# gue-ni/raytracer.glsl

Hardware: AMD Instinct MI355X
Metric: Mpaths/s at 1920x1080, 8 bounces, 10k tris (higher is better)
Workload: dtype f32; 1 GPU; C2: 1920x1080, 8 bounces, 10000 triangles + 5 spheres, cube map 256^2, 1 spp/frame progressive, dof=1; parallelism=1 GPU(s), 8-row strips interleaved, gather to rank 0 every frame, frame_batch=1, kernel=4, wf_rays=4, wf_mode=1, wf_chunk=256, wf_early=0, wf_packed=0, mf_sets=4, mf_group_quads=32, mf_chunk_quads=32

## Files before the change

### raytracer.glsl_amd/csrc/rt_scan.hpp

```cpp
#pragma once
#include <type_traits>
#include "rt_mfma.hpp"

#pragma clang fp contract(off)

namespace rt {

typedef uint32_t u32x4 __attribute__((ext_vector_type(4)));
typedef float f32x6 __attribute__((ext_vector_type(6)));

template <bool kMax> __device__ __forceinline__ float half_reduce(float x)
{
    auto op = [](float a, float b) { return kMax ? __builtin_fmaxf(a, b) : __builtin_fminf(a, b); };
    auto dpp = [](float v, auto ctrl) { return __builtin_bit_cast(float, __builtin_amdgcn_update_dpp(0, __builtin_bit_cast(int, v), decltype(ctrl)::value, 0xf, 0xf, false)); };
    x = op(x, dpp(x, std::integral_constant<int, 0xB1>{}));
    x = op(x, dpp(x, std::integral_constant<int, 0x4E>{}));
    x = op(x, dpp(x, std::integral_constant<int, 0x141>{}));
    x = op(x, dpp(x, std::integral_constant<int, 0x140>{}));
    const float r0 = __builtin_bit_cast(float, __builtin_amdgcn_readlane(__builtin_bit_cast(int, x), 0));
    const float r1 = __builtin_bit_cast(float, __builtin_amdgcn_readlane(__builtin_bit_cast(int, x), 16));
    return op(r0, r1);
}
__device__ __forceinline__ float half_max(float x) { return half_reduce<true>(x); }
__device__ __forceinline__ float half_min(float x) { return half_reduce<false>(x); }
// ... 7 lines not shown
    x = op(x, dpp(x, std::integral_constant<int, 0x140>{}));
    auto rl = [&](int l) { return __builtin_bit_cast(float, __builtin_amdgcn_readlane(__builtin_bit_cast(int, x), l)); };
    return op(op(rl(0), rl(16)), op(rl(32), rl(48)));
}

constexpr uint32_t kCullRowWords = 128;
__device__ __forceinline__ void wave_lds_sync() { __builtin_amdgcn_fence(__ATOMIC_ACQ_REL, "wavefront"); __builtin_amdgcn_wave_barrier(); }
__device__ __forceinline__ bool cull_lane(const MfCull &c, bool have, const MfPacket &pk)
{
    bool skip = false, open = false;
    f3 W = mk(0.0f, 0.0f, 0.0f); float L = 0.0f, nz = 0.0f, Wn = 0.0f;
    if (have && c.Nmin > 0.0f) {
        const f3 gq = pk.O - mk(c.cx, c.cy, c.cz);
        L = __builtin_amdgcn_sqrtf(dot3(gq, gq)) * 1.0001f;
        nz = 9.5367431640625e-07f * __builtin_fmaf(c.lmax, pk.On, c.Pw) * 1.01f;
        W = cross3(pk.D, gq);
        Wn = __builtin_amdgcn_sqrtf(dot3(W, W));
        skip = mf_certified_ka(c, pk, gq, L, nz, Wn);
        open = !skip;
    }
    if (__any(open)) { if (open) skip = mf_certified_b(c, pk, W, L, nz, Wn); }
    return skip;
}

__global__ void __launch_bounds__(256) __attribute__((amdgpu_waves_per_eu(5))) packet_cull_kernel(WaveBuffers wb, const MfCull *__restrict__ cull, uint32_t n_tiles, uint32_t bounce, float ro_add, float sigma_add,
                                                          const MfCull *__restrict__ node, uint32_t node_shift, uint32_t gather)
{
    __shared__ uint32_t s_row[4][kCullRowWords];
    __shared__ uint32_t s_open[4][64];
    const uint32_t n_rays = wb.counts[bounce];
    const RayQueue qin = (bounce & 1u) ? wb.q[1] : wb.q[0];
    const uint32_t lane = threadIdx.x & 63u, n_gran = (n_rays + 127u) / 128u;
    const float inf = __builtin_inff();
    for (uint32_t g = blockIdx.x * 4u + (threadIdx.x >> 6); g < n_gran; g += gridDim.x * 4u) {
        f3 o[2], dh[2]; bool valid[2]; bool usable = true;
        f3 olo = mk(inf, inf, inf), ohi = mk(-inf, -inf, -inf), dlo = olo, dhi = ohi;
#pragma unroll
        for (int k = 0; k < 2; ++k) {
            const uint32_t slot = g * 128u + (uint32_t)k * 64u + lane;
            valid[k] = slot < n_rays;
            o[k] = mk(0.0f, 0.0f, 0.0f); dh[k] = o[k];
            if (valid[k]) {
                float4 a, b;
                const uint32_t from = gather ? wb.sort_src[slot] : n_rays;
                if (from < n_rays) {
                    const float4 *const rec = wb.stage + 4u * from;
                    a = rec[0]; b = rec[1];
                    const float4 c = rec[2];
                    const uint4 r = *reinterpret_cast<const uint4 *>(rec + 3);
                    const uint32_t px = wb.stage_pixel[from];
                    store_through(qin.a + slot, a.x, a.y, a.z, a.w);
                    store_through(qin.b + slot, b.x, b.y, b.z, b.w);
                    store_through(qin.c + slot, c.x, c.y, c.z, c.w);
                    store_through(qin.rng + slot, r.x, r.y, r.z, r.w);
                    store_through(qin.pixel + slot, px);
                } else { a = qin.a[slot]; b = qin.b[slot]; }
                o[k] = mk(a.x, a.y, a.z);
                const f3 d = mk(a.w, b.x, b.y);
                const float dd = dot3(d, d), il = __builtin_amdgcn_rsqf(dd), dl = dd * il;
                dh[k] = mk(d.x * il, d.y * il, d.z * il);
                usable &= (dl > 0.0f) && (dl < inf) && (fabsf(o[k].x) < 1e18f) && (fabsf(o[k].y) < 1e18f) && (fabsf(o[k].z) < 1e18f);
                olo = mk(fminf(olo.x, o[k].x), fminf(olo.y, o[k].y), fminf(olo.z, o[k].z)); ohi = mk(fmaxf(ohi.x, o[k].x), fmaxf(ohi.y, o[k].y), fmaxf(ohi.z, o[k].z));
                dlo = mk(fminf(dlo.x, dh[k].x), fminf(dlo.y, dh[k].y), fminf(dlo.z, dh[k].z)); dhi = mk(fmaxf(dhi.x, dh[k].x), fmaxf(dhi.y, dh[k].y), fmaxf(dhi.z, dh[k].z));
            }
        }
        olo = mk(full_reduce<false>(olo.x), full_reduce<false>(olo.y), full_reduce<false>(olo.z)); ohi = mk(full_reduce<true>(ohi.x), full_reduce<true>(ohi.y), full_reduce<true>(ohi.z));
        dlo = mk(full_reduce<false>(dlo.x), full_reduce<false>(dlo.y), full_reduce<false>(dlo.z)); dhi = mk(full_reduce<true>(dhi.x), full_reduce<true>(dhi.y), full_reduce<true>(dhi.z));
        MfPacket pk;
        pk.O = mk(0.5f * olo.x + 0.5f * ohi.x, 0.5f * olo.y + 0.5f * ohi.y, 0.5f * olo.z + 0.5f * ohi.z);
        f3 D = mk(0.5f * dlo.x + 0.5f * dhi.x, 0.5f * dlo.y + 0.5f * dhi.y, 0.5f * dlo.z + 0.5f * dhi.z);
        const float DD = dot3(D, D), iDl = __builtin_amdgcn_rsqf(DD), Dl = DD * iDl;
        pk.D = mk(D.x * iDl, D.y * iDl, D.z * iDl);
        float ro = 0.0f, sigma = 0.0f;
#pragma unroll
        for (int k = 0; k < 2; ++k)
            if (valid[k]) {
                const f3 eo = o[k] - pk.O, ed = dh[k] - pk.D;
                ro = fmaxf(ro, __builtin_amdgcn_sqrtf(dot3(eo, eo))); sigma = fmaxf(sigma, __builtin_amdgcn_sqrtf(dot3(ed, ed)));
            }
        pk.ro = full_reduce<true>(ro) * 1.0001f + 1e-30f + ro_add; pk.sigma = full_reduce<true>(sigma) * 1.0001f + 2e-6f + sigma_add;
        usable = !__any(!usable) && (Dl > 0.25f);
        pk.On = __builtin_amdgcn_sqrtf(dot3(pk.O, pk.O)) * 1.0001f + pk.ro;
        uint32_t *const row = wb.keep + (size_t)g * wb.keep_words;
        if (node_shift) {
            const uint32_t wv = threadIdx.x >> 6, S = 1u << node_shift, n_nodes = (n_tiles + S - 1u) >> node_shift;
            const uint32_t batch_nodes = (kCullRowWords * 32u) >> node_shift;
            const uint32_t grp = min(S, 32u);
            for (uint32_t b0 = 0; b0 < n_nodes; b0 += batch_nodes) {
                const uint32_t tile0 = b0 << node_shift, w0 = tile0 >> 5;
                s_row[wv][lane] = 0u; s_row[wv][lane + 64u] = 0u;
                wave_lds_sync();
                for (uint32_t n0 = b0; n0 < min(b0 + batch_nodes, n_nodes); n0 += 64u) {
                    const bool have_node = usable && n0 + lane < n_nodes;
                    MfCull c = {};
                    if (have_node) c = node[n0 + lane];
                    const bool closed = cull_lane(c, have_node, pk);
                    const unsigned long long open_nodes = __builtin_amdgcn_ballot_w64(n0 + lane < n_nodes && !closed);
                    if (n0 + lane < n_nodes && !closed)
                        s_open[wv][__builtin_amdgcn_mbcnt_hi((uint32_t)(open_nodes >> 32), __builtin_amdgcn_mbcnt_lo((uint32_t)open_nodes, 0u))] = n0 + lane;
                    wave_lds_sync();
                    const uint32_t n_items = (uint32_t)__builtin_popcountll(open_nodes) << node_shift;
                    for (uint32_t i0 = 0; i0 < n_items; i0 += 64u) {
                        const uint32_t j = i0 + lane;
                        const uint32_t t = j < n_items ? (s_open[wv][j >> node_shift] << node_shift) + (j & (S - 1u)) : n_tiles;
                        const bool have_tile = t < n_tiles;
                        MfCull ct = {};
                        if (usable && have_tile) ct = cull[t];
                        const bool skip = cull_lane(ct, usable && have_tile, pk);
                        const unsigned long long keep = __builtin_amdgcn_ballot_w64(have_tile && !skip);
                        if (j < n_items && (lane & (grp - 1u)) == 0u) {
                            const uint32_t bits = (uint32_t)(keep >> lane) & (uint32_t)((1ull << grp) - 1ull);
                            if (bits) atomicOr(&s_row[wv][(t >> 5) - w0], bits << (t & 31u));
                        }
                    }
                    wave_lds_sync();
                }
                for (uint32_t k = lane; k < kCullRowWords && w0 + k < wb.keep_words; k += 64u)
                    store_through(row + w0 + k, s_row[wv][k]);
                wave_lds_sync();
            }
            continue;
        }
        MfCull c_next = {};
        bool have_next = usable && lane < n_tiles;
        if (have_next) c_next = cull[lane];
        for (uint32_t t0 = 0; t0 < n_tiles; t0 += 64u) {
            const MfCull c = c_next;
            const bool have_this = have_next;
            have_next = usable && t0 + 64u + lane < n_tiles;
            if (have_next) c_next = cull[t0 + 64u + lane];
            const bool skip = cull_lane(c, have_this, pk);
            const unsigned long long have = (n_tiles - t0 >= 64u) ? ~0ull : ((1ull << (n_tiles - t0)) - 1ull);
            const unsigned long long keep = ~(unsigned long long)__builtin_amdgcn_ballot_w64(skip) & have;
            if (lane == 0u) {
                store_through(row + (t0 >> 5), (uint32_t)keep);
                if ((t0 >> 5) + 1u < wb.keep_words) store_through(row + ((t0 >> 5) + 1u), (uint32_t)(keep >> 32));
            }
        }
    }
}

__device__ __forceinline__ void exact_and_merge_at(const MfView &mf, const RayQueue &qin, unsigned long long *best, uint32_t slot, uint32_t pos)
{
    const float4 a = qin.a[slot], b = qin.b[slot];
    const uint32_t v = mf.order[pos];
    TriRay tr; tr.o = mk(a.x, a.y, a.z); tr.d = mk(a.w, b.x, b.y); tr.cv = cross3(tr.d, tr.o); tr.ncv = tr.nd = 0.0f;
    const float t = tri_exact(mf.edges_s[pos], mf.planes_s[pos], tr);
    if (kEps < t && t < kInf) atomicMin(&best[slot], ((unsigned long long)__float_as_uint(t) << 32) | v);
}

constexpr int kDrainFly = 4;
typedef float drain_f4 __attribute__((ext_vector_type(4)));
static_assert(sizeof(TriEdges) == 80 && sizeof(TriPlane) == 32 && alignof(TriEdges) == 16 && alignof(TriPlane) == 16, "drain_region reads these as rows of 16 bytes");
__device__ __forceinline__ void drain_region(const SceneView &sc, const MfView &mf, const RayQueue &qin, unsigned long long *best,
                                             const unsigned long long *recs, uint32_t n_rec, uint32_t lane)
{
    constexpr int K = kDrainFly;
    const uint32_t last_tri = sc.n_tri_visits - 1u;
    for (uint32_t i0 = 0; i0 < n_rec; i0 += 64u * (uint32_t)K) {
        unsigned long long rec[K];
#pragma unroll
        for (int j = 0; j < K; ++j) rec[j] = __hip_atomic_load(recs + min(i0 + (uint32_t)j * 64u + lane, n_rec - 1u), __ATOMIC_RELAXED, __HIP_MEMORY_SCOPE_AGENT);
        uint32_t slot[K], pos5[K], um[K];
#pragma unroll
        for (int j = 0; j < K; ++j) {
            const uint32_t hi = (uint32_t)(rec[j] >> 32);
            slot[j] = (uint32_t)rec[j]; pos5[j] = hi >> 5;
            um[j] = i0 + (uint32_t)j * 64u + lane < n_rec ? hi & 31u : 0u;
        }
        float4 a[K], b[K];
#pragma unroll
        for (int j = 0; j < K; ++j) a[j] = qin.a[slot[j]];
#pragma unroll
        for (int j = 0; j < K; ++j) b[j] = qin.b[slot[j]];
        TriRay tr[K];
#pragma unroll
        for (int j = 0; j < K; ++j) { tr[j].o = mk(a[j].x, a[j].y, a[j].z); tr[j].d = mk(a[j].w, b[j].x, b[j].y); tr[j].cv = cross3(tr[j].d, tr[j].o); tr[j].ncv = tr[j].nd = 0.0f; }
        while ((um[0] | um[1] | um[2] | um[3]) != 0u) {
            static_assert(K == 4, "the loop condition names the masks");
            bool on[K]; uint32_t p[K], v[K]; drain_f4 e[K][5], pl[K][2];
#pragma unroll
            for (int j = 0; j < K; ++j) {
                const uint32_t pos = pos5[j] + (um[j] ? (uint32_t)__builtin_ctz(um[j]) : 0u);
                on[j] = um[j] != 0u && pos < sc.n_tri_visits;
                um[j] &= um[j] - 1u;
                p[j] = min(pos, last_tri);
            }
#pragma unroll
            for (int j = 0; j < K; ++j) {
                const drain_f4 *const ep = reinterpret_cast<const drain_f4 *>(mf.edges_s + p[j]), *const pp = reinterpret_cast<const drain_f4 *>(mf.planes_s + p[j]);
#pragma unroll
                for (int k = 0; k < 5; ++k) e[j][k] = ep[k];
                pl[j][0] = pp[0]; pl[j][1] = pp[1]; v[j] = mf.order[p[j]];
            }
#pragma unroll
            for (int j = 0; j < K; ++j) {
#pragma unroll
                for (int k = 0; k < 5; ++k) asm volatile("" : "+v"(e[j][k]));
                asm volatile("" : "+v"(pl[j][0]), "+v"(pl[j][1]), "+v"(v[j]));
            }
#pragma unroll
            for (int j = 0; j < K; ++j) {
                TriEdges T; TriPlane P;
                T.e0x = e[j][0].x; T.e0y = e[j][0].y; T.e0z = e[j][0].z; T.e1x = e[j][0].w; T.e1y = e[j][1].x; T.e1z = e[j][1].y; T.e2x = e[j][1].z; T.e2y = e[j][1].w; T.e2z = e[j][2].x;
                T.m0x = e[j][2].y; T.m0y = e[j][2].z; T.m0z = e[j][2].w; T.m1x = e[j][3].x; T.m1y = e[j][3].y; T.m1z = e[j][3].z; T.m2x = e[j][3].w; T.m2y = e[j][4].x; T.m2z = e[j][4].y;
                T.bound_e = e[j][4].z; T.bound_m = e[j][4].w;
                P.nx = pl[j][0].x; P.ny = pl[j][0].y; P.nz = pl[j][0].z; P.v0x = pl[j][0].w; P.v0y = pl[j][1].x; P.v0z = pl[j][1].y; P.material = 0; P.pad = 0;
                const float t = tri_exact(T, P, tr[j]);
                if (on[j] && kEps < t && t < kInf) atomicMin(&best[slot[j]], ((unsigned long long)__float_as_uint(t) << 32) | v[j]);
            }
        }
    }
}

constexpr int kSoloSets = 4;
struct SoloCfg {
    static constexpr uint32_t kStepMax = 2u * 64u;
    static constexpr uint32_t kDrain = 192u;
    static constexpr uint32_t kQueue = kStepMax + kDrain + 1u;
    static constexpr uint32_t kRaysPerWave = (uint32_t)kSoloSets * 32u;
};

#define RT_HEAD "s_nop 1\n\t"
#define RT_EXAM(PL, ML, KL, TH) \
    "v_min3_f32 v[" #ML "+0], v[" #PL "+0], v[" #PL "+1], v[" #PL "+2]\n\t" \
    "v_min3_f32 v[" #ML "+1], v[" #PL "+3], v[" #PL "+4], v[" #PL "+5]\n\t" \
    "v_min3_f32 v[" #ML "+2], v[" #PL "+6], v[" #PL "+7], v[" #PL "+8]\n\t" \
    "v_min3_f32 v[" #ML "+3], v[" #PL "+9], v[" #PL "+10], v[" #PL "+11]\n\t" \
    "v_min3_f32 v[" #ML "+4], v[" #PL "+12], v[" #PL "+13], v[" #PL "+14]\n\t" \
    "v_max3_f32 v[" #ML "+5], v[" #ML "+0], v[" #ML "+1], v[" #ML "+2]\n\t" \
    "v_max3_f32 v[" #ML "+5], v[" #ML "+5], v[" #ML "+3], v[" #ML "+4]\n\t" \
    "v_cmp_nle_f32_e64 s[" #KL ":" #KL "+1], v[" #ML "+5], " TH "\n\t"
#define RT_MFMA(NL, AOP, B) "v_mfma_f32_32x32x16_bf16 v[" #NL ":" #NL "+15], " AOP ", " B ", 0\n\t"
#define RT_FOLD(ANY, KL) "s_or_b64 " ANY ", s[" #KL ":" #KL "+1], s[" #KL "+2:" #KL "+3]\n\ts_or_b64 " ANY ", " ANY ", s[" #KL "+4:" #KL "+5]\n\ts_or_b64 " ANY ", " ANY ", s[" #KL "+6:" #KL "+7]\n\t"
#define RT_STAGE_Y_TEXT(AOP) RT_MFMA(192, AOP, "%[b0]") RT_EXAM(128, 96, 36, "%[t0]") RT_MFMA(208, AOP, "%[b1]") RT_EXAM(144, 104, 38, "%[t1]") \
                             RT_MFMA(224, AOP, "%[b2]") RT_EXAM(160, 112, 40, "%[t2]") RT_MFMA(240, AOP, "%[b3]") RT_EXAM(176, 120, 42, "%[t3]")
#define RT_STAGE_X_TEXT(AOP) RT_MFMA(128, AOP, "%[b0]") RT_EXAM(192, 64, 44, "%[t0]") RT_MFMA(144, AOP, "%[b1]") RT_EXAM(208, 72, 46, "%[t1]") \
                             RT_MFMA(160, AOP, "%[b2]") RT_EXAM(224, 80, 48, "%[t2]") RT_MFMA(176, AOP, "%[b3]") RT_EXAM(240, 88, 50, "%[t3]")
#define RT_K_CLOBBERS "s36", "s37", "s38", "s39", "s40", "s41", "s42", "s43", "s44", "s45", "s46", "s47", "s48", "s49", "s50", "s51"
#define RT_TRIP(AY, AX) \
    asm volatile(RT_HEAD RT_STAGE_Y_TEXT("%[ay]") RT_STAGE_X_TEXT("%[ax]") RT_FOLD("%[anya]", 36) RT_FOLD("%[anyb]", 44) \
                 : "+{v[128:143]}"(X0), "+{v[144:159]}"(X1), "+{v[160:175]}"(X2), "+{v[176:191]}"(X3), \
                   "=&{v[192:207]}"(Y0), "=&{v[208:223]}"(Y1), "=&{v[224:239]}"(Y2), "=&{v[240:255]}"(Y3), \
                   "=&{v[96:101]}"(MA0), "=&{v[104:109]}"(MA1), "=&{v[112:117]}"(MA2), "=&{v[120:125]}"(MA3), \
                   "=&{v[64:69]}"(MB0), "=&{v[72:77]}"(MB1), "=&{v[80:85]}"(MB2), "=&{v[88:93]}"(MB3), [anya] "=&s"(any_a), [anyb] "=&s"(any_b) \
                 : [ay] "v"(AY), [ax] "v"(AX), [b0] "v"(B0), [b1] "v"(B1), [b2] "v"(B2), [b3] "v"(B3), [t0] "v"(th0), [t1] "v"(th1), [t2] "v"(th2), [t3] "v"(th3) \
                 : RT_K_CLOBBERS)
#define RT_TRIP_L(AY, AX, NY, NX, ADDR) \
    asm volatile(RT_HEAD RT_MFMA(192, "%[ay]", "%[b0]") "ds_read_b128 %[ny], %[addr]\n\tds_read_b128 %[nx], %[addr] offset:1024\n\tv_add_u32_e32 %[addr], 0x800, %[addr]\n\t" \
                 RT_EXAM(128, 96, 36, "%[t0]") RT_MFMA(208, "%[ay]", "%[b1]") RT_EXAM(144, 104, 38, "%[t1]") \
                 RT_MFMA(224, "%[ay]", "%[b2]") RT_EXAM(160, 112, 40, "%[t2]") RT_MFMA(240, "%[ay]", "%[b3]") RT_EXAM(176, 120, 42, "%[t3]") \
                 RT_STAGE_X_TEXT("%[ax]") "s_waitcnt lgkmcnt(0)\n\t" RT_FOLD("%[anya]", 36) RT_FOLD("%[anyb]", 44) \
                 : "+{v[128:143]}"(X0), "+{v[144:159]}"(X1), "+{v[160:175]}"(X2), "+{v[176:191]}"(X3), \
                   "=&{v[192:207]}"(Y0), "=&{v[208:223]}"(Y1), "=&{v[224:239]}"(Y2), "=&{v[240:255]}"(Y3), \
                   "=&{v[96:101]}"(MA0), "=&{v[104:109]}"(MA1), "=&{v[112:117]}"(MA2), "=&{v[120:125]}"(MA3), \
                   "=&{v[64:69]}"(MB0), "=&{v[72:77]}"(MB1), "=&{v[80:85]}"(MB2), "=&{v[88:93]}"(MB3), [anya] "=&s"(any_a), [anyb] "=&s"(any_b), \
                   [ny] "=&v"(NY), [nx] "=&v"(NX), [addr] "+v"(ADDR) \
                 : [ay] "v"(AY), [ax] "v"(AX), [b0] "v"(B0), [b1] "v"(B1), [b2] "v"(B2), [b3] "v"(B3), [t0] "v"(th0), [t1] "v"(th1), [t2] "v"(th2), [t3] "v"(th3) \
                 : RT_K_CLOBBERS, "memory")
#define RT_TRIP_G(AY, AX, NY, NX, ADDRY, ADDRX) \
    asm volatile(RT_HEAD RT_MFMA(192, "%[ay]", "%[b0]") "ds_read_b128 %[ny], %[addry]\n\tds_read_b128 %[nx], %[addrx]\n\t" \
                 RT_EXAM(128, 96, 36, "%[t0]") RT_MFMA(208, "%[ay]", "%[b1]") RT_EXAM(144, 104, 38, "%[t1]") \
                 RT_MFMA(224, "%[ay]", "%[b2]") RT_EXAM(160, 112, 40, "%[t2]") RT_MFMA(240, "%[ay]", "%[b3]") RT_EXAM(176, 120, 42, "%[t3]") \
                 RT_STAGE_X_TEXT("%[ax]") "s_waitcnt lgkmcnt(0)\n\t" RT_FOLD("%[anya]", 36) RT_FOLD("%[anyb]", 44) \
                 : "+{v[128:143]}"(X0), "+{v[144:159]}"(X1), "+{v[160:175]}"(X2), "+{v[176:191]}"(X3), \
                   "=&{v[192:207]}"(Y0), "=&{v[208:223]}"(Y1), "=&{v[224:239]}"(Y2), "=&{v[240:255]}"(Y3), \
                   "=&{v[96:101]}"(MA0), "=&{v[104:109]}"(MA1), "=&{v[112:117]}"(MA2), "=&{v[120:125]}"(MA3), \
                   "=&{v[64:69]}"(MB0), "=&{v[72:77]}"(MB1), "=&{v[80:85]}"(MB2), "=&{v[88:93]}"(MB3), [anya] "=&s"(any_a), [anyb] "=&s"(any_b), \
                   [ny] "=&v"(NY), [nx] "=&v"(NX) \
                 : [ay] "v"(AY), [ax] "v"(AX), [b0] "v"(B0), [b1] "v"(B1), [b2] "v"(B2), [b3] "v"(B3), [t0] "v"(th0), [t1] "v"(th1), [t2] "v"(th2), [t3] "v"(th3), \
                   [addry] "v"(ADDRY), [addrx] "v"(ADDRX) \
                 : RT_K_CLOBBERS, "memory")
#define RT_STAGE_Y(AY) \
    asm volatile(RT_HEAD RT_STAGE_Y_TEXT("%[ay]") RT_FOLD("%[anya]", 36) \
                 : "=&{v[192:207]}"(Y0), "=&{v[208:223]}"(Y1), "=&{v[224:239]}"(Y2), "=&{v[240:255]}"(Y3), \
                   "=&{v[96:101]}"(MA0), "=&{v[104:109]}"(MA1), "=&{v[112:117]}"(MA2), "=&{v[120:125]}"(MA3), [anya] "=&s"(any_a) \
                 : "{v[128:143]}"(X0), "{v[144:159]}"(X1), "{v[160:175]}"(X2), "{v[176:191]}"(X3), \
                   [ay] "v"(AY), [b0] "v"(B0), [b1] "v"(B1), [b2] "v"(B2), [b3] "v"(B3), [t0] "v"(th0), [t1] "v"(th1), [t2] "v"(th2), [t3] "v"(th3) \
                 : RT_K_CLOBBERS)
#define RT_PRODUCTS_X(AOP) \
    asm volatile(RT_HEAD RT_MFMA(128, "%[a]", "%[b0]") RT_MFMA(144, "%[a]", "%[b1]") RT_MFMA(160, "%[a]", "%[b2]") RT_MFMA(176, "%[a]", "%[b3]") "s_nop 15" \
                 : "=&{v[128:143]}"(X0), "=&{v[144:159]}"(X1), "=&{v[160:175]}"(X2), "=&{v[176:191]}"(X3) \
                 : [a] "v"(AOP), [b0] "v"(B0), [b1] "v"(B1), [b2] "v"(B2), [b3] "v"(B3))
#define RT_EXAMINE_X() \
    asm volatile("s_nop 15\n\t" RT_EXAM(128, 96, 36, "%[t0]") RT_EXAM(144, 104, 38, "%[t1]") RT_EXAM(160, 112, 40, "%[t2]") RT_EXAM(176, 120, 42, "%[t3]") "s_nop 7\n\t" RT_FOLD("%[anya]", 36) \
                 : "=&{v[96:101]}"(MA0), "=&{v[104:109]}"(MA1), "=&{v[112:117]}"(MA2), "=&{v[120:125]}"(MA3), [anya] "=&s"(any_a) \
                 : "{v[128:143]}"(X0), "{v[144:159]}"(X1), "{v[160:175]}"(X2), "{v[176:191]}"(X3), [t0] "v"(th0), [t1] "v"(th1), [t2] "v"(th2), [t3] "v"(th3) \
                 : RT_K_CLOBBERS)
#define RT_EXAMINE_Y() \
    asm volatile("s_nop 15\n\t" RT_EXAM(192, 64, 44, "%[t0]") RT_EXAM(208, 72, 46, "%[t1]") RT_EXAM(224, 80, 48, "%[t2]") RT_EXAM(240, 88, 50, "%[t3]") "s_nop 7\n\t" RT_FOLD("%[anyb]", 44) \
                 : "=&{v[64:69]}"(MB0), "=&{v[72:77]}"(MB1), "=&{v[80:85]}"(MB2), "=&{v[88:93]}"(MB3), [anyb] "=&s"(any_b) \
                 : "{v[192:207]}"(Y0), "{v[208:223]}"(Y1), "{v[224:239]}"(Y2), "{v[240:255]}"(Y3), [t0] "v"(th0), [t1] "v"(th1), [t2] "v"(th2), [t3] "v"(th3) \
                 : RT_K_CLOBBERS)

#define RT_MASK_BIT(ML, U, TH) "v_cmp_nle_f32_e32 vcc, v[" #ML "+" #U "], " TH "\n\tv_addc_co_u32_e32 %[m], vcc, %[m], %[m], vcc\n\t"
#define RT_MASK_SET(ML, TH) RT_MASK_BIT(ML, 4, TH) RT_MASK_BIT(ML, 3, TH) RT_MASK_BIT(ML, 2, TH) RT_MASK_BIT(ML, 1, TH) RT_MASK_BIT(ML, 0, TH)
#define RT_MASK_A(MASK) \
    asm volatile("v_mov_b32_e32 %[m], 0\n\t" RT_MASK_SET(120, "%[t3]") RT_MASK_SET(112, "%[t2]") RT_MASK_SET(104, "%[t1]") RT_MASK_SET(96, "%[t0]") \
                 : [m] "=&v"(MASK) : "{v[96:101]}"(MA0), "{v[104:109]}"(MA1), "{v[112:117]}"(MA2), "{v[120:125]}"(MA3), \
                   [t0] "v"(th0), [t1] "v"(th1), [t2] "v"(th2), [t3] "v"(th3) : "vcc")
#define RT_MASK_B(MASK) \
    asm volatile("v_mov_b32_e32 %[m], 0\n\t" RT_MASK_SET(88, "%[t3]") RT_MASK_SET(80, "%[t2]") RT_MASK_SET(72, "%[t1]") RT_MASK_SET(64, "%[t0]") \
                 : [m] "=&v"(MASK) : "{v[64:69]}"(MB0), "{v[72:77]}"(MB1), "{v[80:85]}"(MB2), "{v[88:93]}"(MB3), \
                   [t0] "v"(th0), [t1] "v"(th1), [t2] "v"(th2), [t3] "v"(th3) : "vcc")

#if defined(RT_SOLO_STAMPS) && RT_SOLO_STAMPS == 3
#define RT_STAMP(var) const unsigned long long var = 0
#define RT_STAMP_ADD(acc, from, to)
#define RT_STAMP_NOW() __builtin_amdgcn_s_memtime()
#elif defined(RT_SOLO_STAMPS) && RT_SOLO_STAMPS == 2
#define RT_STAMP(var) const unsigned long long var = 0
#define RT_STAMP_ADD(acc, from, to)
#define RT_STAMP_NOW() __builtin_amdgcn_s_memrealtime()
#elif defined(RT_SOLO_STAMPS)
#define RT_STAMP(var) const unsigned long long var = __builtin_amdgcn_s_memtime()
#define RT_STAMP_ADD(acc, from, to) acc += (to) - (from)
#define RT_STAMP_NOW() __builtin_amdgcn_s_memtime()
#else
#define RT_STAMP(var)
#define RT_STAMP_ADD(acc, from, to)
#endif

struct Mask128 { unsigned long long lo, hi; };
__device__ __forceinline__ Mask128 m128_shr(Mask128 m, uint32_t s)
{
    Mask128 r;
    if (s >= 128u) { r.lo = 0ull; r.hi = 0ull; }
    else if (s >= 64u) { r.lo = m.hi >> (s - 64u); r.hi = 0ull; }
    else if (s == 0u) r = m;
    else { r.lo = (m.lo >> s) | (m.hi << (64u - s)); r.hi = m.hi >> s; }
    return r;
}
__device__ __forceinline__ Mask128 m128_low(uint32_t n)
{
    Mask128 r;
    r.lo = n >= 64u ? ~0ull : ((1ull << n) - 1ull);
    r.hi = n >= 128u ? ~0ull : (n > 64u ? ((1ull << (n - 64u)) - 1ull) : 0ull);
    return r;
}
__device__ __forceinline__ Mask128 m128_and(Mask128 a, Mask128 b) { Mask128 r; r.lo = a.lo & b.lo; r.hi = a.hi & b.hi; return r; }
__device__ __forceinline__ bool m128_any(Mask128 m) { return (m.lo | m.hi) != 0ull; }
__device__ __forceinline__ uint32_t m128_popc(Mask128 m) { return (uint32_t)__builtin_popcountll(m.lo) + (uint32_t)__builtin_popcountll(m.hi); }
__device__ __forceinline__ uint32_t m128_ctz(Mask128 m)
{
    return m.lo ? (uint32_t)__builtin_ctzll(m.lo) : (m.hi ? 64u + (uint32_t)__builtin_ctzll(m.hi) : 128u);
}
__device__ __forceinline__ uint32_t m128_cto(Mask128 m)
{
    Mask128 n; n.lo = ~m.lo; n.hi = ~m.hi;
    return m128_ctz(n);
}
template <typename Words>
__device__ __forceinline__ Mask128 chunk_keep_bits(Words row, uint32_t tile_begin, uint32_t n_tiles)
{
    const Words w = row + (tile_begin >> 5);
    const uint32_t sh = tile_begin & 31u;
    const unsigned long long w01 = (unsigned long long)w[0] | ((unsigned long long)w[1] << 32), w23 = (unsigned long long)w[2] | ((unsigned long long)w[3] << 32), w4 = w[4];
    Mask128 m;
    m.lo = sh ? (w01 >> sh) | (w23 << (64u - sh)) : w01;
    m.hi = sh ? (w23 >> sh) | (w4 << (64u - sh)) : w23;
    return m128_and(m, m128_low(n_tiles));
}

template <bool kCount>
__global__ void __launch_bounds__(256) cull_items_kernel(WaveBuffers wb, uint32_t bounce, uint32_t chunk_quads, uint32_t n_quads, Counters *__restrict__ counters)
{
    const uint32_t n_rays = wb.counts[bounce], n_gran = (n_rays + 127u) >> 7;
    const uint32_t c = blockIdx.y, q_begin = c * chunk_quads, q_end = min(q_begin + chunk_quads, n_quads);
    const uint32_t lane = threadIdx.x & 63u;
    if (q_begin >= q_end) return;
    const uint32_t n_tiles = (q_end - q_begin) * kMfQuadTiles;
    unsigned long long culled = 0;
    for (uint32_t g0 = blockIdx.x * 256u + (threadIdx.x & ~63u); g0 < n_gran; g0 += gridDim.x * 256u) {
        const uint32_t g = g0 + lane;
        bool any = false;
        if (g < n_gran) {
            const Mask128 bits = chunk_keep_bits(wb.keep + (size_t)g * wb.keep_words, q_begin * kMfQuadTiles, n_tiles);
            any = m128_any(bits);
            if (kCount) culled += (unsigned long long)(n_tiles - m128_popc(bits)) * kMfTileTris * min(128u, n_rays - g * 128u);
        }
        const unsigned long long m = __builtin_amdgcn_ballot_w64(any);
        if (m == 0ull) continue;
        uint32_t at = 0u;
        if (lane == 0u) at = atomicAdd(wb.item_counts + c, (uint32_t)__popcll(m));
        at = __builtin_amdgcn_readfirstlane(at) + __builtin_amdgcn_mbcnt_hi((uint32_t)(m >> 32), __builtin_amdgcn_mbcnt_lo((uint32_t)m, 0u));
        if (any) store_through(wb.items + ((size_t)c * wb.items_stride + at), g);
    }
    if (kCount && culled) atomicAdd(&counters->culled_tests, culled);
}

constexpr uint32_t kPlanItemFixed = 6u;
template <bool kCount>
__global__ void __launch_bounds__(256) scan_plan_kernel(WaveBuffers wb, uint32_t bounce, uint32_t chunk_quads, uint32_t n_quads, Counters *__restrict__ counters)
{
    __shared__ uint32_t wsum[4];
    __shared__ uint32_t carry;
    const uint32_t n_rays = wb.counts[bounce], n_gran = (n_rays + 127u) >> 7;
    const uint32_t c = blockIdx.x, q_begin = c * chunk_quads, q_end = min(q_begin + chunk_quads, n_quads);
    const uint32_t lane = threadIdx.x & 63u, wave = threadIdx.x >> 6;
    const uint32_t n_tiles = q_begin < q_end ? (q_end - q_begin) * kMfQuadTiles : 0u;
    uint32_t *const P = wb.plan_prefix + (size_t)c * wb.plan_stride;
    unsigned long long culled = 0;
    if (threadIdx.x == 0) carry = 0u;
    __syncthreads();
    for (uint32_t g0 = 0; g0 < n_gran; g0 += 256u) {
        const uint32_t g = g0 + threadIdx.x;
        uint32_t cost = 0u;
        if (g < n_gran && n_tiles) {
            const uint32_t kept = m128_popc(chunk_keep_bits(wb.keep + (size_t)g * wb.keep_words, q_begin * kMfQuadTiles, n_tiles));
            cost = kept ? 4u * (kept + kPlanItemFixed) : 1u;
            if (kCount) culled += (unsigned long long)(n_tiles - kept) * kMfTileTris * min(128u, n_rays - g * 128u);
        }
        uint32_t inc = cost;
        for (int off = 1; off < 64; off <<= 1) { const uint32_t t = __shfl_up(inc, off); if (lane >= (uint32_t)off) inc += t; }
        if (lane == 63u) wsum[wave] = inc;
        __syncthreads();
        uint32_t base = carry;
        for (uint32_t w = 0; w < wave; ++w) base += wsum[w];
        if (g < n_gran) store_through(P + g, base + inc);
        __syncthreads();
        if (threadIdx.x == 255u) carry = base + inc;
        __syncthreads();
    }
    if (threadIdx.x == 0) store_through(wb.plan_total + c, carry);
    if (kCount && culled) atomicAdd(&counters->culled_tests, culled);
}
__global__ void __launch_bounds__(64) scan_plan_base_kernel(WaveBuffers wb, uint32_t n_chunks)
{
    const uint32_t lane = threadIdx.x;
    unsigned long long run = 0ull;
    for (uint32_t c0 = 0; c0 < n_chunks; c0 += 64u) {
        const uint32_t c = c0 + lane;
        const unsigned long long t = c < n_chunks ? (unsigned long long)wb.plan_total[c] : 0ull;
        unsigned long long inc = t;
        for (int off = 1; off < 64; off <<= 1) { const unsigned long long u = __shfl_up(inc, off); if (lane >= (uint32_t)off) inc += u; }
        if (c < n_chunks) store_through(wb.plan_base + c, run + inc - t);
        run += __shfl(inc, 63);
    }
    if (lane == 0) store_through(wb.plan_base + n_chunks, run);
}

template <bool kCount, uint32_t kWaves>
__device__ __forceinline__ unsigned long long *solo_cand_words()
{
    if constexpr (kCount) { __shared__ unsigned long long words[kWaves]; return words; }
    else return nullptr;
}
template <bool kCount, int W, int kDist>
__global__ void __launch_bounds__(256 * W) __attribute__((amdgpu_waves_per_eu(W, W)))
scan_solo_kernel(SceneView sc, WaveBuffers wb, MfView mf, uint32_t bounce, uint32_t chunk_quads, uint32_t n_chunks, Counters *__restrict__ counters, int debug_skip_exact, int cull, int narrow_fused)
{
    using Cfg = SoloCfg;
    constexpr bool dynamic = kDist == 1, planned = kDist == 2, hybrid = kDist == 3;
    constexpr int S = kSoloSets;
    constexpr uint32_t kWaves = 4u * (uint32_t)W, kThreads = 256u * (uint32_t)W;
    extern __shared__ uint4 lds_tiles[];
    __shared__ uint2 lds_queue[kWaves * Cfg::kQueue];
    __shared__ uint32_t lds_pick;
    unsigned long long *const lds_cand = solo_cand_words<kCount, kWaves>();
    __shared__ uint32_t lds_ring[kWaves * 16u];
#ifdef RT_SOLO_STAMPS
#if RT_SOLO_STAMPS == 3
    const unsigned long long tr_wave_begin = __builtin_amdgcn_s_memrealtime();
#endif
    const unsigned long long ts_wave_begin = RT_STAMP_NOW();
    unsigned long long tt_stage = 0, tt_rays = 0, tt_group = 0, tt_steady = 0, tt_park = 0, tt_flush = 0, tt_iters = 0, tt_culled = 0, tt_culled_n = 0, tt_tiles = 0;
#endif
    if constexpr (W == 1) asm volatile("" ::: "a255");
    const uint32_t n_rays = wb.counts[bounce], n_gran = (n_rays + 127u) >> 7;
    const RayQueue qin = (bounce & 1u) ? wb.q[1] : wb.q[0];
    unsigned long long *best = (bounce & 1u) ? wb.best[1] : wb.best[0];
    const int lane = threadIdx.x & 63, wave = __builtin_amdgcn_readfirstlane((int)(threadIdx.x >> 6)), col = lane & 31, half = lane >> 5;
    const uint32_t real_quads = min(mf.n_quads, (sc.n_tri_visits + kMfQuadTris - 1u) / kMfQuadTris);
    const uint32_t region = blockIdx.x * kWaves + (uint32_t)wave;
    uint2 *const cand = wb.cand + (size_t)region * wb.cand_region;
    unsigned long long appended = 0;
    uint32_t *const sched = wb.sched + (size_t)bounce * wb.sched_stride;
    uint32_t opaque_zero = 0u;
    asm volatile("" : "+v"(opaque_zero));
    const uint32_t group_shift = (uint32_t)__builtin_ctz(mf.group_quads);
    constexpr uint32_t kQuadBytes = kMfQuadTiles * 1024;
    uint2 *queue = lds_queue + wave * Cfg::kQueue;
    if (kCount && lane == 0) lds_cand[wave] = 0ull;
    unsigned long long c_culled = 0;
    typedef const float __attribute__((address_space(4))) *ConstFloats;
    typedef const uint32_t __attribute__((address_space(4))) *ConstWords;
    typedef float f32x4 __attribute__((ext_vector_type(4)));
    typedef const volatile f32x4 __attribute__((address_space(4))) *ConstGroupHalf;
    const ConstFloats groups_k = (ConstFloats)(uintptr_t)mf.groups;
    const uint32_t l_lane = (uint32_t)half * 32u + (uint32_t)col;

    constexpr bool kSplit = W == 2;
    constexpr int H = kSplit ? S / 2 : S;
    static_assert(S == 4, "a granule is four sets of 32 rays");
    constexpr uint32_t kRayStride = kSplit ? 64u : 32u;
    const uint32_t ray_lane = kSplit ? (uint32_t)lane : (uint32_t)col;
    float4 nxt_a[H], nxt_b[H];
    auto fetch_rays = [&](uint32_t g, float4 (&da)[H], float4 (&db)[H]) {
        if (g * 128u + 128u <= n_rays) {
            const uint32_t slot0 = g * 128u + ray_lane;
#pragma unroll
            for (int j = 0; j < H; ++j) da[j] = qin.a[slot0 + (uint32_t)j * kRayStride];
#pragma unroll
            for (int j = 0; j < H; ++j) db[j] = qin.b[slot0 + (uint32_t)j * kRayStride];
            return;
        }
#pragma unroll
        for (int j = 0; j < H; ++j) {
            const uint32_t slot = g * 128u + (uint32_t)j * kRayStride + ray_lane;
            da[j] = make_float4(0.0f, 0.0f, 0.0f, 0.0f); db[j] = da[j];
            if (slot < n_rays) { da[j] = qin.a[slot]; db[j] = qin.b[slot]; }
        }
    };
    auto prepare_ray = [&](MfRay &r, const float4 &a, const float4 &b, bool valid) {
        r.valid = valid;
        r.o = mk(a.x, a.y, a.z); r.d = mk(a.w, b.x, b.y);
        r.wd = __builtin_amdgcn_sqrtf(dot3(r.d, r.d)) * 1.001f;
        r.wod = (__builtin_amdgcn_sqrtf(dot3(r.o, r.o)) * 1.001f) * r.wd;
        const uint32_t dxy = pack_bf16(r.d.x, r.d.y);
        r.dyz = pack_bf16(r.d.y, r.d.z);
        r.dx_hi = dxy << 16;
        const f3 dl = mk(r.d.x - __uint_as_float(dxy << 16), r.d.y - __uint_as_float(dxy & 0xffff0000u), r.d.z - __uint_as_float(r.dyz & 0xffff0000u));
        if constexpr (kSplit) { r.tail = pack_bf16(1.0f, dl.x); r.tail_hi = pack_bf16(dl.y, dl.z); }
        else { r.tail = half ? pack_bf16(dl.y, dl.z) : pack_bf16(1.0f, dl.x); r.tail_hi = r.tail; }
    };

    constexpr uint32_t kXcds = 8;
    const bool by_xcd = gridDim.x >= kXcds * n_chunks;
    const uint32_t c_first = by_xcd ? (blockIdx.x / kXcds) % n_chunks : blockIdx.x % n_chunks;
    typedef const unsigned long long __attribute__((address_space(4))) *ConstU64;
    const ConstU64 pbase_k = (ConstU64)(uintptr_t)wb.plan_base;
    auto chunk_base = [&](uint32_t cc) -> unsigned long long { return cull ? pbase_k[cc] : (unsigned long long)cc * n_gran; };
    unsigned long long p_lo = 0ull, p_hi = 0ull;
    uint32_t p_next = 0u;
    if constexpr (planned) {
        const unsigned long long total = chunk_base(n_chunks);
        p_lo = (unsigned long long)(((unsigned __int128)total * blockIdx.x) / gridDim.x);
        p_hi = (unsigned long long)(((unsigned __int128)total * (blockIdx.x + 1u)) / gridDim.x);
        uint32_t lo = 0u, hi = n_chunks;
        while (hi - lo > 1u) { const uint32_t mid = (lo + hi) >> 1; if (chunk_base(mid) <= p_lo) lo = mid; else hi = mid; }
        p_next = lo;
    }
    bool first_chunk = true;
    for (uint32_t c_from = c_first;;) {
        RT_STAMP(ts_pick);
        uint32_t c = c_from;
        if constexpr (planned) {
            while (p_next < n_chunks && chunk_base(p_next + 1u) <= p_lo) ++p_next;
            if (p_lo == p_hi || p_next >= n_chunks || chunk_base(p_next) >= p_hi) break;
            c = p_next++;
            if (!first_chunk) __syncthreads();
            first_chunk = false;
        }
        if (dynamic) {
            __syncthreads();
            if (wave == 0) {
                uint32_t dist = 0xFFFFFFFFu;
                for (uint32_t cc = (uint32_t)lane; cc < n_chunks; cc += 64u) {
                    const uint32_t have = cull ? wb.item_counts[cc] : n_gran;
                    if (__hip_atomic_load(sched + cc, __ATOMIC_RELAXED, __HIP_MEMORY_SCOPE_AGENT) < have) dist = min(dist, (cc + n_chunks - c_from) % n_chunks);
                }
                for (int off = 32; off > 0; off >>= 1) dist = min(dist, (uint32_t)__shfl_xor((int)dist, off));
                if (lane == 0) lds_pick = dist == 0xFFFFFFFFu ? 0xFFFFFFFFu : (c_from + dist) % n_chunks;
            }
            __syncthreads();
            c = __builtin_amdgcn_readfirstlane(lds_pick);
            if (c == 0xFFFFFFFFu) break;
        }
        c_from = (c + 1u) % n_chunks;
        const uint32_t q_begin = c * chunk_quads, q_end = min(q_begin + chunk_quads, real_quads);
        const uint32_t v_chunk_begin = q_begin * kMfQuadTris, v_chunk_end = min(q_end * (uint32_t)kMfQuadTris, sc.n_tri_visits);
        const uint32_t n_tiles = (q_end - q_begin) * kMfQuadTiles, tile_begin = q_begin * kMfQuadTiles;
        const Mask128 keep_all = m128_low(n_tiles);
        {
            const uint32_t n16 = (q_end - q_begin) * (kQuadBytes / 16u);
            const uint4 *src = mf.A + (size_t)q_begin * (kQuadBytes / 16u);
            for (uint32_t i0 = threadIdx.x; i0 < n16; i0 += 8u * kThreads) {
                uint4 v[8];
#pragma unroll
                for (int k = 0; k < 8; ++k) { const uint32_t i = i0 + (uint32_t)k * kThreads; v[k] = src[min(i, n16 - 1u)]; }
#pragma unroll
                for (int k = 0; k < 8; ++k) { const uint32_t i = i0 + (uint32_t)k * kThreads; if (i < n16) lds_tiles[i] = v[k]; }
            }
            __syncthreads();
        }
        RT_STAMP(ts_staged);
        RT_STAMP_ADD(tt_stage, ts_pick, ts_staged);

        uint32_t *const counter = sched + c;
        const uint32_t n_items = __builtin_amdgcn_readfirstlane((cull && dynamic) ? wb.item_counts[c] : n_gran);
        const ConstWords items_k = (ConstWords)(uintptr_t)(wb.items + (size_t)c * wb.items_stride);
        uint32_t blocks_here, rank_here;
        if (by_xcd) {
            const uint32_t rest = gridDim.x % (kXcds * n_chunks);
            blocks_here = (gridDim.x / (kXcds * n_chunks)) * kXcds + min(kXcds, rest > kXcds * c ? rest - kXcds * c : 0u);
            rank_here = (blockIdx.x / (kXcds * n_chunks)) * kXcds + blockIdx.x % kXcds;
        } else { blocks_here = (gridDim.x - c + n_chunks - 1u) / n_chunks; rank_here = blockIdx.x / n_chunks; }
        constexpr uint32_t kNone = 0xFFFFFFFFu;
        const uint32_t hdiv = max(wb.hybrid_div, 1u), hturn = max(hdiv - 1u, 1u);
        const uint32_t n_tail = hybrid ? n_gran / hdiv : 0u, n_turns = n_gran - n_tail;
        const uint32_t n_claimable = hybrid ? n_tail : n_items;
        auto claim = [&](uint32_t seen, uint32_t &lo, uint32_t &end) {
            const uint32_t rem = n_claimable > seen ? n_claimable - seen : 0u;
            const uint32_t n = hybrid ? min(max(rem / (2u * max(blocks_here, 1u) * kWaves), 1u), 4u) : min(max(rem / (4u * max(blocks_here, 1u) * kWaves), 1u), 16u);
            uint32_t v = 0u;
            if (lane == 0) v = atomicAdd(counter + opaque_zero, n);
            const uint32_t at = __builtin_amdgcn_readfirstlane(v);
            lo = min(at, n_claimable); end = min(at + n, n_claimable);
        };
        bool tail = false;
        const ConstWords keep_k = (ConstWords)(uintptr_t)wb.keep;
        auto item_of = [&](uint32_t k, uint32_t &g, Mask128 &bits) {
            g = hybrid ? (tail ? hdiv * k + (hdiv - 1u) : (k / hturn) * hdiv + k % hturn) : k; bits = keep_all;
            if (cull) {
                if (dynamic) g = items_k[k];
                bits = chunk_keep_bits(keep_k + (size_t)g * wb.keep_words, tile_begin, n_tiles);
            }
        };
        uint32_t k, hi, step;
        if (dynamic) { step = 1u; claim(0u, k, hi); }
        else if (planned) {
            const unsigned long long cb = chunk_base(c), ce = chunk_base(c + 1u);
            const uint32_t a = (uint32_t)((p_lo > cb ? p_lo : cb) - cb), e = (uint32_t)((p_hi < ce ? p_hi : ce) - cb);
            const uint32_t w_lo = a + (uint32_t)(((unsigned long long)(e - a) * (uint32_t)wave) / kWaves), w_hi = a + (uint32_t)(((unsigned long long)(e - a) * ((uint32_t)wave + 1u)) / kWaves);
            const ConstWords P = (ConstWords)(uintptr_t)(wb.plan_prefix + (size_t)c * wb.plan_stride);
            auto first_above = [&](uint32_t x) -> uint32_t {
                if (!cull) return min(x, n_gran);
                uint32_t lo = 0u, up = n_gran;
                while (lo < up) { const uint32_t mid = (lo + up) >> 1; if (P[mid] > x) up = mid; else lo = mid + 1u; }
                return lo;
            };
            step = 1u; k = first_above(w_lo); hi = first_above(w_hi);
        }
        else {
            step = blocks_here * kWaves; k = rank_here * kWaves + (uint32_t)wave; hi = hybrid ? n_turns : n_items;
            if (hybrid && k >= hi) { tail = true; step = 1u; claim(0u, k, hi); }
        }
        uint32_t rec_k = kNone, rec_g = 0u;
        Mask128 rec_keep = {0ull, 0ull};
        uint32_t ray_k = kNone;
        auto advance = [&]() {
            k += step;
            if (dynamic && k >= hi) claim(hi, k, hi);
            if (hybrid && k >= hi) { if (tail) claim(hi, k, hi); else { tail = true; step = 1u; claim(0u, k, hi); } }
        };
        uint32_t qn = 0, seq = 0, seq_flushed = 0;
        uint32_t *const ring = lds_ring + wave * 16;
        auto flush = [&]() __attribute__((always_inline)) {
            for (uint32_t i0 = 0; i0 < qn; i0 += 64u) {
                const uint32_t i = i0 + (uint32_t)lane;
                const uint2 e = i < qn ? queue[i] : make_uint2(0u, 0u);
                const uint32_t ln = e.x & 63u, pos5 = v_chunk_begin + ((e.x >> 8) & 127u) * kMfTileTris + 5u * (ln >> 5);
                const uint32_t slot0 = ring[(e.x >> 16) & 15u] * 128u;
                if (kCount) {
                    uint32_t pairs = 0u;
#pragma unroll
                    for (int b = 0; b < 5 * S; ++b) pairs += (uint32_t)__popcll(__builtin_amdgcn_ballot_w64(((e.y >> b) & 1u) != 0u));
                    if (lane == 0) lds_cand[wave] += (unsigned long long)pairs;
                }
                const uint32_t bits = (debug_skip_exact == 0 || debug_skip_exact == 3) ? e.y : 0u;
#pragma unroll
                for (int s = 0; s < S; ++s) {
                    uint32_t um = (bits >> (5 * s)) & 31u;
                    const unsigned long long m = __builtin_amdgcn_ballot_w64(um != 0u);
                    const unsigned long long at = appended + __builtin_amdgcn_mbcnt_hi((uint32_t)(m >> 32), __builtin_amdgcn_mbcnt_lo((uint32_t)m, 0u));
                    const uint32_t slot = slot0 + (uint32_t)(s * 32) + (ln & 31u);
                    if (um != 0u) {
                        if (at < (unsigned long long)wb.cand_region) store_through(reinterpret_cast<unsigned long long *>(cand + at), (unsigned long long)slot | ((unsigned long long)((pos5 << 5) | um) << 32));
                        else
                            while (um) {
                                const uint32_t pos = pos5 + (uint32_t)__builtin_ctz(um);
                                um &= um - 1u;
                                if (pos < v_chunk_end) exact_and_merge_at(mf, qin, best, slot, pos);
                            }
                    }
                    appended += (unsigned long long)__popcll(m);
                }
            }
            qn = 0; seq_flushed = seq;
        };
        while (k < hi) {
            RT_STAMP(ts_iter);
            uint32_t g; Mask128 keep;
            if (rec_k == k) { g = rec_g; keep = rec_keep; } else item_of(k, g, keep);
            const uint32_t wave_slot0 = g * 128u;
            const uint32_t succ = k + step < hi ? k + step : kNone;
            if (succ != kNone) { item_of(succ, rec_g, rec_keep); rec_k = succ; }
            if (kCount && cull && !dynamic && !planned)
                c_culled += (unsigned long long)(n_tiles - m128_popc(keep)) * kMfTileTris * min(128u, n_rays - wave_slot0);
            if (!m128_any(keep)) {
                if constexpr (W == 1) { if (succ != kNone && m128_any(rec_keep)) { fetch_rays(rec_g, nxt_a, nxt_b); ray_k = succ; } }
                advance();
                continue;
            }
            if (seq - seq_flushed >= 15u) flush();
            if (lane == 0) ring[seq & 15u] = g;
            const uint32_t item_tag = (seq & 15u) << 16;
            ++seq;
            MfRay ray[H];
            if constexpr (W == 1) {
                if (ray_k != k) fetch_rays(g, nxt_a, nxt_b);
#pragma unroll
                for (int j = 0; j < H; ++j) prepare_ray(ray[j], nxt_a[j], nxt_b[j], wave_slot0 + (uint32_t)j * kRayStride + ray_lane < n_rays);
                if (succ != kNone && m128_any(rec_keep)) { fetch_rays(rec_g, nxt_a, nxt_b); ray_k = succ; }
            }

            u32x4 B0, B1, B2, B3;
            float th0, th1, th2, th3;
            f32x16 X0, X1, X2, X3, Y0, Y1, Y2, Y3;
            f32x6 MA0, MA1, MA2, MA3, MB0, MB1, MB2, MB3;
            unsigned long long any_a, any_b;
            auto append = [&](uint32_t tile, uint32_t mask) __attribute__((always_inline)) {
                const unsigned long long m = __builtin_amdgcn_ballot_w64(mask != 0u);
                uint32_t pre = __builtin_amdgcn_mbcnt_hi((uint32_t)(m >> 32), __builtin_amdgcn_mbcnt_lo((uint32_t)m, 0u));
                asm volatile("" : "+v"(pre));
                queue[mask ? qn + pre : Cfg::kQueue - 1u] = make_uint2((uint32_t)lane | (tile << 8) | item_tag, mask);
                qn += (uint32_t)__popcll(m);
                if (qn >= Cfg::kDrain) flush();
            };
            auto park_a = [&](uint32_t tile) { RT_STAMP(ts_p0); uint32_t mask; RT_MASK_A(mask); append(tile, mask); RT_STAMP(ts_p1); RT_STAMP_ADD(tt_park, ts_p0, ts_p1); };
            auto park_b = [&](uint32_t tile) { RT_STAMP(ts_p0); uint32_t mask; RT_MASK_B(mask); append(tile, mask); RT_STAMP(ts_p1); RT_STAMP_ADD(tt_park, ts_p0, ts_p1); };
            RT_STAMP(ts_rays);
            RT_STAMP_ADD(tt_rays, ts_iter, ts_rays);

            for (uint32_t ts0 = 0; ts0 < n_tiles;) {
                RT_STAMP(ts_g0);
                const uint32_t q = q_begin + ts0 / kMfQuadTiles;
                const uint32_t grp = q >> group_shift;
                const uint32_t ts1 = min(n_tiles, (((grp + 1u) << group_shift) - q_begin) * kMfQuadTiles);
                Mask128 seg = m128_and(m128_shr(keep, ts0), m128_low(ts1 - ts0));
                if (!m128_any(seg)) { ts0 = ts1; continue; }
                const ConstGroupHalf gp = (ConstGroupHalf)(groups_k + (size_t)grp * (sizeof(MfGroup) / 4));
                const f32x4 g_lo = gp[0], g_hi = gp[1];
                MfGroup G;
                G.cx = g_lo.x; G.cy = g_lo.y; G.cz = g_lo.z; G.E = g_lo.w; G.Ml = g_hi.x; G.Pw = g_hi.y; G.P = g_hi.z; G.pad1 = 0.0f;
                if constexpr (W == 2) {
                    fetch_rays(g, nxt_a, nxt_b);
#pragma unroll
                    for (int j = 0; j < H; ++j) prepare_ray(ray[j], nxt_a[j], nxt_b[j], wave_slot0 + (uint32_t)j * kRayStride + ray_lane < n_rays);
                }
                u32x4 Bs[S]; float ths[S];
#pragma unroll
                for (int j = 0; j < H; ++j) {
                    const MfRay &r = ray[j];
                    const f3 ol = r.o - mk(G.cx, G.cy, G.cz);
                    const f3 cvl = cross3(r.d, ol);
                    const float ncv = __builtin_amdgcn_sqrtf(dot3(cvl, cvl)) * 1.001f, no = __builtin_amdgcn_sqrtf(dot3(ol, ol)) * 1.001f;
                    const float margin = mf_margin(G, ncv, no, r);
                    const float th = (!r.valid || debug_skip_exact == 2) ? __builtin_inff() : (margin < 1.0e30f ? -margin : __builtin_nanf(""));
                    const uint32_t bx = pack_bf16(cvl.x, cvl.y), by = (pack_bf16(cvl.z, 0.0f) & 0xffffu) | r.dx_hi;
                    if constexpr (!kSplit) {
                        Bs[j].x = bx; Bs[j].y = by; Bs[j].z = r.dyz; Bs[j].w = r.tail; ths[j] = th;
                    } else {
                        const auto px = __builtin_amdgcn_permlane32_swap(bx, bx, false, false);
                        const auto py = __builtin_amdgcn_permlane32_swap(by, by, false, false);
                        const auto pz = __builtin_amdgcn_permlane32_swap(r.dyz, r.dyz, false, false);
                        const auto pw = __builtin_amdgcn_permlane32_swap(r.tail, r.tail_hi, false, false);
                        const auto pt = __builtin_amdgcn_permlane32_swap(__float_as_uint(th), __float_as_uint(th), false, false);
                        const int s0 = 2 * j, s1 = 2 * j + 1;
                        Bs[s0].x = px[0]; Bs[s0].y = py[0]; Bs[s0].z = pz[0]; Bs[s0].w = pw[0]; ths[s0] = __uint_as_float(pt[0]);
                        Bs[s1].x = px[1]; Bs[s1].y = py[1]; Bs[s1].z = pz[1]; Bs[s1].w = pw[1]; ths[s1] = __uint_as_float(pt[1]);
                    }
                }
                B0 = Bs[0]; B1 = Bs[1]; B2 = Bs[2]; B3 = Bs[3];
                th0 = ths[0]; th1 = ths[1]; th2 = ths[2]; th3 = ths[3];
#if defined(RT_SOLO_STAMPS) && RT_SOLO_STAMPS == 1
                asm volatile("" : "+v"(B0), "+v"(B1), "+v"(B2), "+v"(B3), "+v"(th0), "+v"(th1), "+v"(th2), "+v"(th3));
#endif
                RT_STAMP(ts_g1);
                RT_STAMP_ADD(tt_group, ts_g0, ts_g1);
                typedef const uint4 __attribute__((address_space(3))) *LdsRow;
                const uint32_t n_kept = m128_popc(seg);
                if (n_kept == ts1 - ts0 && debug_skip_exact != 3) {
                    const uint32_t t0 = ts0, t1 = ts1;
                    const uint4 *row = lds_tiles + (size_t)t0 * 64u + l_lane;
                    auto tile_row = [&]() { const uint4 r = *row; row += 64; return u32x4{r.x, r.y, r.z, r.w}; };
                    u32x4 ap = tile_row(), ay = tile_row(), ax = tile_row(), by, bx;
                    uint32_t addr = (uint32_t)(uintptr_t)(LdsRow)row;
                    RT_PRODUCTS_X(ap);
                    uint32_t t = t0 + 1u;
                    for (; t + 3u < t1; t += 4u) {
                        RT_TRIP_L(ay, ax, by, bx, addr);
                        if (__builtin_expect((any_a | any_b) != 0ull, 0)) {
                            if (any_a) park_a(t - 1u);
                            if (any_b) park_b(t);
                        }
                        RT_TRIP_L(by, bx, ay, ax, addr);
                        if (__builtin_expect((any_a | any_b) != 0ull, 0)) {
                            if (any_a) park_a(t + 1u);
                            if (any_b) park_b(t + 2u);
                        }
                    }
                    if (t + 1u < t1) {
                        RT_TRIP_L(ay, ax, by, bx, addr);
                        if ((any_a | any_b) != 0ull) {
                            if (any_a) park_a(t - 1u);
                            if (any_b) park_b(t);
                        }
                        ay = by; t += 2u;
                    }
                    if (t < t1) {
                        RT_STAGE_Y(ay);
                        if (any_a) park_a(t - 1u);
                        RT_EXAMINE_Y();
                        if (any_b) park_b(t);
                    } else {
                        RT_EXAMINE_X();
                        if (any_a) park_a(t - 1u);
                    }
                } else {
                    unsigned long long cur = seg.lo, nxt = seg.hi;
                    uint32_t base = ts0;
                    auto next_tile = [&]() -> uint32_t {
                        if (cur == 0ull) { cur = nxt; nxt = 0ull; base += 64u; }
                        const uint32_t bit = (uint32_t)__builtin_ctzll(cur);
                        cur &= ~(1ull << bit);
                        return base + bit;
                    };
                    const uint32_t lds_lane = (uint32_t)(uintptr_t)(LdsRow)(lds_tiles + l_lane);
                    auto row_addr = [&](uint32_t tile) { return lds_lane + tile * 1024u; };
                    auto load_row = [&](uint32_t tile) { const uint4 r = lds_tiles[(size_t)tile * 64u + l_lane]; return u32x4{r.x, r.y, r.z, r.w}; };
                    uint32_t left = n_kept;
                    uint32_t t_x = next_tile(); --left;
                    u32x4 ap = load_row(t_x), ay, ax, by, bx;
                    uint32_t t_y = t_x, t_n = t_x;
                    if (left > 0u) t_y = next_tile();
                    if (left > 1u) t_n = next_tile();
                    ay = load_row(t_y); ax = load_row(t_n);
                    RT_PRODUCTS_X(ap);
#define RT_LIST_TRIP(AY, AX, NY, NX) do { \
                        left -= 2u; \
                        const uint32_t u_y = left > 0u ? next_tile() : t_x, u_n = left > 1u ? next_tile() : t_x; \
                        const uint32_t a_y = row_addr(u_y), a_n = row_addr(u_n); \
                        RT_TRIP_G(AY, AX, NY, NX, a_y, a_n); \
                        if (__builtin_expect((any_a | any_b) != 0ull, 0)) { \
                            if (any_a) park_a(t_x); \
                            if (any_b) park_b(t_y); \
                        } \
                        t_x = t_n; t_y = u_y; t_n = u_n; \
                    } while (0)
                    while (left >= 4u) { RT_LIST_TRIP(ay, ax, by, bx); RT_LIST_TRIP(by, bx, ay, ax); }
                    if (left >= 2u) { RT_LIST_TRIP(ay, ax, by, bx); ay = by; }
#undef RT_LIST_TRIP
                    if (left == 1u) {
                        RT_STAGE_Y(ay);
                        if (any_a) park_a(t_x);
                        RT_EXAMINE_Y();
                        if (any_b) park_b(t_y);
                    } else {
                        RT_EXAMINE_X();
                        if (any_a) park_a(t_x);
                    }
                }
                ts0 = ts1;
                RT_STAMP(ts_g2);
                RT_STAMP_ADD(tt_steady, ts_g0, ts_g2);
            }
            RT_STAMP(ts_f0);
            advance();
            RT_STAMP(ts_f1);
            RT_STAMP_ADD(tt_flush, ts_f0, ts_f1);
#ifdef RT_SOLO_STAMPS
            tt_iters++; tt_tiles += m128_popc(keep);
#endif
        }
        flush();
        if (!dynamic && !planned) break;
    }
    if (narrow_fused) {
        const uint32_t n_rec = (uint32_t)(appended < (unsigned long long)wb.cand_region ? appended : (unsigned long long)wb.cand_region);
        if (n_rec) {
            asm volatile("s_waitcnt vmcnt(0)" ::: "memory");
            drain_region(sc, mf, qin, best, reinterpret_cast<const unsigned long long *>(cand), n_rec, (uint32_t)lane);
        }
    }
#ifdef RT_SOLO_STAMPS
    if (lane == 0 && mf.dbg_log) {
        unsigned long long *d = reinterpret_cast<unsigned long long *>(mf.dbg_log) + 16ull * bounce;
        const unsigned long long ts_end = RT_STAMP_NOW();
#if RT_SOLO_STAMPS == 3
        const unsigned long long tr_end = __builtin_amdgcn_s_memrealtime();
#endif
        atomicAdd(d + 0, ts_end - ts_wave_begin); atomicAdd(d + 1, tt_stage); atomicAdd(d + 2, tt_rays); atomicAdd(d + 3, tt_group);
        atomicAdd(d + 4, tt_steady); atomicAdd(d + 5, tt_park); atomicAdd(d + 6, tt_flush); atomicAdd(d + 7, tt_iters); atomicAdd(d + 8, 1ull);
        atomicAdd(d + 9, tt_tiles);
        if (blockIdx.x == 0 && wave == 0) d[15] = (unsigned long long)gridDim.x * kWaves;
        atomicMax(d + 10, ts_end - ts_wave_begin);
        if (kDist == 0 && bounce < 16u) {
            unsigned long long *pc = reinterpret_cast<unsigned long long *>(mf.dbg_log) + 2048ull + (16ull * bounce) * 64ull * 2ull + 2ull * (c_first % 512u);
            atomicAdd(pc, ts_end - ts_wave_begin); atomicAdd(pc + 1, 1ull);
        }
        atomicAdd(d + 11, tt_culled); atomicAdd(d + 12, tt_culled_n);
#if RT_SOLO_STAMPS == 3
        atomicAdd(d + 14, tr_end - tr_wave_begin);
#endif
    }
#endif
    if (lane == 0) store_through(wb.cand_counts + region, (uint32_t)(appended < (unsigned long long)wb.cand_region ? appended : (unsigned long long)wb.cand_region));
    if (lane == 0 && appended > (unsigned long long)*wb.cand_peak) atomicMax(wb.cand_peak, (uint32_t)(appended < 0xFFFFFFF0ull ? appended : 0xFFFFFFF0ull));
    if (kCount) {
        if (lane == 0 && lds_cand[wave]) atomicAdd(&counters->candidates, lds_cand[wave]);
        if (lane == 0 && c_culled) atomicAdd(&counters->culled_tests, c_culled);
        if (blockIdx.x == 0 && threadIdx.x == 0) atomicAdd(&counters->tri_tests, (unsigned long long)n_rays * sc.n_tri_visits);
    }
}

constexpr uint32_t kNarrowSplit = 4;
__global__ void __launch_bounds__(256) narrow_phase_kernel(SceneView sc, WaveBuffers wb, MfView mf, uint32_t bounce, uint32_t n_regions)
{
#ifdef RT_SOLO_STAMPS
    if (blockIdx.x == 0 && blockIdx.y == 0 && threadIdx.x == 0 && mf.dbg_log) {
        unsigned long long *d = reinterpret_cast<unsigned long long *>(mf.dbg_log) + 16ull * bounce;
        d[13] += d[10]; d[10] = 0ull;
    }
#endif
    const RayQueue qin = (bounce & 1u) ? wb.q[1] : wb.q[0];
// ... 21 lines not shown
```

### raytracer.glsl_amd/csrc/rtgl_amd.hip

```cpp
#include <hip/hip_runtime.h>
#include <algorithm>
#include <cmath>
#include <cstdio>
#include <cstring>
#include <string>
#include <vector>
#include <map>
#include <mutex>
#include <thread>
#include <condition_variable>
#include <memory>

#include "../../include/rtgl_amd.h"
#include "rt_device.hpp"
#include "rt_wavefront.hpp"
#include "rt_mfma.hpp"
#include "rt_scan.hpp"
#include "rt_denoise.hpp"
#include "rt_temporal.hpp"
#include "rt_temporal_clip.hpp"
#include "rt_tonemap.hpp"
#include "rt_error.hpp"
#include "rt_adaptive.hpp"
#include "rt_adaptive_plan.hpp"
#include "rt_robust.hpp"
#include "rt_robust_plan.hpp"
#include "rt_spread.hpp"
#include "rt_spread_plan.hpp"
#include "rt_node_walk.hpp"
#include "rt_mesh_visits.hpp"
#include "rt_buffers.hpp"
#include "rt_scan_launch.hpp"
#include "rt_shade_launch.hpp"
#include "rt_camera_keep.hpp"

#pragma clang fp contract(off)

using namespace rt;


__global__ void __launch_bounds__(256) prepare_triangles_kernel(const float4 *__restrict__ vertices,
                                                                const uint32_t *__restrict__ visit_tri, uint32_t n_visits,
                                                                TriEdges *__restrict__ edges, TriPlane *__restrict__ planes)
{
    uint32_t k = blockIdx.x * blockDim.x + threadIdx.x;
    if (k >= n_visits) return;
    uint32_t tri = visit_tri[k];
    float4 a = vertices[3 * (size_t)tri + 0], b = vertices[3 * (size_t)tri + 1], c = vertices[3 * (size_t)tri + 2];
    f3 v0 = mk(a.x, a.y, a.z), v1 = mk(b.x, b.y, b.z), v2 = mk(c.x, c.y, c.z);
    f3 e0 = v1 - v0, e1 = v2 - v1, e2 = v0 - v2;
    f3 m0 = cross3(v1, v0), m1 = cross3(v2, v1), m2 = cross3(v0, v2);
    f3 n = normalize3(cross3(v1 - v0, v2 - v0));
    TriEdges E;
    E.e0x = e0.x; E.e0y = e0.y; E.e0z = e0.z; E.e1x = e1.x; E.e1y = e1.y; E.e1z = e1.z; E.e2x = e2.x; E.e2y = e2.y; E.e2z = e2.z;
    E.m0x = m0.x; E.m0y = m0.y; E.m0z = m0.z; E.m1x = m1.x; E.m1y = m1.y; E.m1z = m1.z; E.m2x = m2.x; E.m2y = m2.y; E.m2z = m2.z;
    float be = fmaxf(fmaxf(dot3(e0, e0), dot3(e1, e1)), dot3(e2, e2));
    float bm = fmaxf(fmaxf(dot3(m0, m0), dot3(m1, m1)), dot3(m2, m2));
    E.bound_e = __builtin_sqrtf(be) * 1.0001f;
    E.bound_m = __builtin_sqrtf(bm) * 1.0001f;
    edges[k] = E;
    TriPlane P;
    P.nx = n.x; P.ny = n.y; P.nz = n.z; P.v0x = v0.x; P.v0y = v0.y; P.v0z = v0.z;
    float w = a.w;
    P.material = (w > -2147483648.0f && w < 2147483648.0f) ? (int32_t)w : -1;
    P.pad = 0;
    planes[k] = P;
}

template <bool kCount, bool kAov>
__global__ void __launch_bounds__(256) pathtrace_mega_kernel(SceneView sc, FrameParams P, ImageView im, uint4 *rng_out, Counters *counters, AovView aov)
{
    const int lane = threadIdx.x & 63, wave = threadIdx.x >> 6;
    const int px = (blockIdx.x * 4 + wave) * 8 + (lane & 7);
    const int lrow = blockIdx.y * 8 + (lane >> 3);
    if (px >= im.disp_w || lrow >= im.local_rows) return;
    const int py = local_to_global_row(im, lrow);
    if (py >= im.disp_h) return;

    Rng rng; rng.x = (uint32_t)px; rng.y = (uint32_t)py; rng.z = (uint32_t)P.random;
    rng.w = (uint32_t)px + (uint32_t)py + (uint32_t)P.random;
    float4 *pix = im.pixels + (size_t)lrow * im.width + px;
    f3 prev = mk(0.0f, 0.0f, 0.0f);
    if (!P.reset_flag) { float4 q = *pix; prev = mk(q.x, q.y, q.z); }
    f3 origin, dir;
    camera_ray(P, px, py, im.width, im.height, rng, origin, dir);

    unsigned long long c_seg = 0, c_tests = 0, c_cand = 0, c_env = 0;
    f3 color = mk(0.0f, 0.0f, 0.0f);
    for (uint32_t s = 0; s < P.samples; ++s) {
        f3 o = origin, d = dir;
        f3 radiance = mk(0.0f, 0.0f, 0.0f), thr = mk(1.0f, 1.0f, 1.0f);
        for (uint32_t bounce = 0; bounce < P.max_bounce; ++bounce) {
            if (kCount) c_seg++;
            Hit h1; h1.t = kInf; h1.material = 0; h1.point = h1.normal = mk(0.0f, 0.0f, 0.0f);
            uint32_t sphere_id = kNoSphere;
            bool hit_sphere = kAov ? sphere_pass_id(sc, o, d, h1, sphere_id) : sphere_pass(sc, o, d, h1);
            TriRay tr = make_tri_ray(o, d);
            float best_t = kInf; uint32_t best_v = 0xFFFFFFFFu;
            for (uint32_t v = 0; v < sc.n_tri_visits; ++v) {
                const TriEdges &T = sc.tri_edges[v];
                if (tri_filter(T, tr)) {
                    if (kCount) c_cand++;
                    float t = tri_exact(T, sc.tri_planes[v], tr);
                    if (kEps < t && t < best_t) { best_t = t; best_v = v; }
                }
            }
            if (kCount) c_tests += sc.n_tri_visits;
            bool hit_mesh = best_v != 0xFFFFFFFFu;
            if (!hit_sphere && !hit_mesh) {
                f3 bg;
                if (P.use_envmap) { bg = env_lookup(sc, d); if (kCount) c_env++; }
                else bg = mk(P.background[0], P.background[1], P.background[2]);
                if (kAov && s == 0u && bounce == 0u) aov_write(sc, aov, (uint32_t)(lrow * im.width + px), kAovMiss, h1, 0u, bg);
                radiance = radiance + bg * thr;
                break;
            }
            Hit h = h1;
            if (!(h1.t < best_t)) {
                const TriPlane &pl = sc.tri_planes[best_v];
                h.t = best_t; h.point = o + d * best_t; h.normal = mk(pl.nx, pl.ny, pl.nz); h.material = pl.material;
            }
            if (kAov && s == 0u && bounce == 0u)
                aov_write(sc, aov, (uint32_t)(lrow * im.width + px), !(h1.t < best_t) ? kAovTriangle : kAovSphere, h, !(h1.t < best_t) ? best_v : sphere_id, mk(0.0f, 0.0f, 0.0f));
            if (!shade_hit(sc, h, rng, o, d, thr, radiance)) break;
        }
        color = color + radiance;
    }
    if (kAov && P.max_bounce == 0u) {
        Hit none; none.t = kInf; none.material = 0; none.point = none.normal = mk(0.0f, 0.0f, 0.0f);
        aov_write(sc, aov, (uint32_t)(lrow * im.width + px), kAovMiss, none, 0u, mk(0.0f, 0.0f, 0.0f));
    }
    { const float4 v = accumulate_pixel(P, color, prev); store_through(pix, v.x, v.y, v.z, v.w); }
    if (rng_out) rng_out[(size_t)lrow * im.width + px] = make_uint4(rng.x, rng.y, rng.z, rng.w);
    if (kCount) {
        atomicAdd(&counters->paths, (unsigned long long)P.samples);
        atomicAdd(&counters->segments, c_seg);
        atomicAdd(&counters->tri_tests, c_tests);
        atomicAdd(&counters->candidates, c_cand);
        atomicAdd(&counters->env_lookups, c_env);
    }
}

__global__ void __launch_bounds__(256) image_to_u8_kernel(const float4 *__restrict__ src, uchar4 *__restrict__ dst, int width, int rows, int flip)
{
    int i = blockIdx.x * blockDim.x + threadIdx.x;
    if (i >= width * rows) return;
    int y = i / width, x = i - y * width;
    float4 p = src[i];
    auto q = [](float v) -> unsigned char {
        v = v < 0.0f ? 0.0f : (v > 1.0f ? 1.0f : v);
        if (!(v == v)) v = 0.0f;
        return (unsigned char)__builtin_rintf(v * 255.0f);
    };
    int oy = flip ? rows - 1 - y : y;
    dst[(size_t)oy * width + x] = make_uchar4(q(p.x), q(p.y), q(p.z), q(p.w));
}


static thread_local std::string g_create_error;

struct PartWorker {
    std::thread th;
    std::mutex m;
    std::condition_variable cv;
    enum { kIdle, kJob, kDone, kQuit } state = kIdle;
    int rc = 0;
    rtgl_context *part = nullptr;
};

static int device_alloc(void **p, size_t bytes) { return (int)hipMalloc(p, bytes); }
static int device_free(void *p) { return (int)hipFree(p); }

struct rtgl_context {
    int device = 0;
    int width = 0, height = 0;
    int rank = 0, world = 1, strip_rows = 8, local_rows = 0;
    hipStream_t own_stream = nullptr, stream = nullptr; bool own_stream_shared = false;
    hipEvent_t ev0 = nullptr, ev1 = nullptr;
    bool timed = false;
    std::vector<hipEvent_t> kev;
    uint32_t kev_used = 0;
    std::vector<uint32_t> kev_frame_start;
    std::string error;

    std::vector<uint8_t> h_meshes, h_nodes, h_vertices;
    uint32_t n_meshes = 0, n_nodes = 0, n_vec4 = 0;

    rt_buffers::Ledger buffers{device_alloc, device_free};
    SphereRec *d_spheres = nullptr; uint32_t n_spheres = 0;
    MaterialRec *d_materials = nullptr; uint32_t n_materials = 0;
    float4 *d_vertices = nullptr;
    uint32_t *d_sphere_visits = nullptr; uint32_t n_sphere_visits = 0;
    TriEdges *d_edges = nullptr; TriPlane *d_planes = nullptr; uint32_t n_tri_visits = 0;
    TriEdges *d_edges_s = nullptr; TriPlane *d_planes_s = nullptr;
    uint8_t *d_env = nullptr; int env_w = 0, env_h = 0, env_c = 0, env_faces = 0;
    float4 *d_image_own = nullptr, *d_image = nullptr;
    uint4 *d_rng = nullptr;
    Counters *d_counters = nullptr;
    uchar4 *d_u8 = nullptr;

    float2 *d_group_bounds = nullptr;
    MfGroup *d_mf_groups = nullptr; MfCull *d_mf_cull = nullptr; MfCull *d_mf_cull_node = nullptr; uint32_t cull_node_shift = 0; uint4 *d_mf_A = nullptr; uint32_t *d_mf_order = nullptr; uint32_t n_mf_groups = 0, mf_group_quads = 32; uint32_t *d_dbg_log = nullptr;
    void *d_wave = nullptr; size_t wave_capacity = 0; bool wave_multi = false;
    uint32_t *d_counts = nullptr; uint32_t counts_capacity = 0;
    uint32_t *h_counts = nullptr;
    hipEvent_t counts_ev = nullptr; bool counts_pending = false, counts_valid = false;
    bool timing_this_frame = false; uint32_t timing_frame_counter = 0;
    int kernel_in_use = -1;
    int n_cus = 256;
    uint2 *d_items = nullptr; size_t items_capacity = 0;
    uint32_t *d_sched = nullptr; size_t sched_capacity = 0;
    uint32_t *d_keep = nullptr; size_t keep_capacity = 0;
    uint32_t *d_keep0 = nullptr; size_t keep0_capacity = 0; bool keep0_valid = false; rt_camera_keep::Camera keep0_camera{}; uint32_t keep0_n0 = 0, keep0_words = 0; uint64_t keep0_scene = 0;
    int opt_camera_lean = 1;
    uint32_t camera_lean_frames = 0;
    int opt_shade_pass = 1;
    uint32_t shade_pass_launches = 0;
    uint64_t scene_version = 0;
    void *d_plan = nullptr; size_t plan_capacity = 0;
    void *d_stage = nullptr; size_t stage_capacity = 0;
    uint32_t *d_sort_hist = nullptr; uint32_t sort_bits_alloc = 0;
    int sort_set = 0; uint32_t sort_set_bits = 0; bool sort_sets_clean = false;
    int opt_narrow_fused = 1;
    int opt_sort_move = 1;
    float mesh_lo[3] = {0.0f, 0.0f, 0.0f}, mesh_hi[3] = {0.0f, 0.0f, 0.0f}, mesh_ext = 0.0f;
    uint2 *d_cand = nullptr; uint32_t cand_regions = 0, cand_region_pairs = 0, cand_region_target = 0; bool cand_fixed = false;
    bool solo_attr_set = false;
    bool group_explicit = false;
    bool kernel_explicit = false;
    uint32_t counts_n0 = 0, counts_len = 0;
    std::vector<uint32_t> est_counts;
    WaveBuffers wb{};

    std::vector<rtgl_context *> parts;
    std::vector<hipEvent_t> part_done;
    hipEvent_t gather_done = nullptr;
    std::vector<std::unique_ptr<PartWorker>> workers;
    bool gathered = false, peer_copy = true;

    std::vector<FrameParams> pending;
    float4 *d_batch_rad = nullptr; size_t batch_capacity = 0;
    uint32_t last_batch_frames = 1;
    bool tris_dirty = false, visits_dirty = false;
    float4 *d_aov[3] = {nullptr, nullptr, nullptr}; uint4 *d_aov_ids = nullptr;
    uint32_t aov_n = 0; bool aov_restart = true;
    std::vector<uint32_t> h_visit_mesh, h_visit_tri;
    uint32_t *d_visit_mesh = nullptr, *d_visit_tri = nullptr; bool visit_ids_dirty = true;
    uint32_t *d_visit_scratch = nullptr;
    float4 *d_dn_scratch[2] = {nullptr, nullptr}, *d_denoised = nullptr; bool has_denoised = false;
    float4 *d_dn_variance = nullptr; uint32_t *d_dn_near = nullptr; bool has_dn_variance = false;
    float4 *d_tm_hist[2] = {nullptr, nullptr}, *d_tm_normal[2] = {nullptr, nullptr}, *d_tm_position[2] = {nullptr, nullptr};
    int tm_cur = 0; bool has_temporal = false, tm_valid = false, tm_has_normal = false;
    TemporalCamera tm_camera{};
    float4 *d_tm_moments[2] = {nullptr, nullptr}; int tm_moments = 0;
    uchar4 *d_display = nullptr; uint32_t *d_tone_state = nullptr;
    bool has_display = false, tone_prev = false, tone_auto = false; int tone_set = 0, tone_hist_set = -1; float tone_exposure = 1.0f;
    float *d_err_snapshot = nullptr; uint4 *d_err_tiles = nullptr; uint32_t *d_err_summary = nullptr;
    uint64_t err_epoch = 1, err_snap_epoch = 0; int32_t err_fm = 0, err_first = 0, err_fn = 0; bool err_rendered = false, has_error = false;
    float4 *d_ad_samples = nullptr; float *d_ad_snapshot = nullptr; uint4 *d_ad_records = nullptr; uint32_t *d_ad_counts = nullptr, *d_ad_lists = nullptr;
    bool ad_active = false, has_adaptive = false; rtgl_adaptive_params ad_params{};
    std::vector<uint8_t> ad_mask; std::vector<uint32_t> ad_blocks, ad_tiles;
    float4 *d_rb_buckets = nullptr, *d_rb_out = nullptr;
    uint32_t rb_K = 0, rb_N = 0; bool rb_active = false, rb_resolved = false;
    uint4 *d_rbe_tiles = nullptr; uint32_t *d_rbe_summary = nullptr; bool has_rb_error = false;
    FrameParams params{};
    bool have_params = false;
    int opt_kernel = RTGL_KERNEL_WAVEFRONT_MFMA_SOLO, opt_rng_state = 0, opt_counters = 0, opt_kernel_timing = 0, opt_wf_rays = 4, opt_wf_mode = kLds, opt_wf_chunk = 256, opt_wf_early = 0, opt_wf_packed = 0, opt_mf_chunk_quads = 32, opt_mf_group_quads = 32, opt_cull = 3, opt_sort_min_rays = 131072, opt_scan_waves = 0, opt_scan_dynamic = 0, opt_debug_skip_exact = 0, opt_frame_batch = 1, opt_aov = 0, opt_denoise_source = 0, opt_temporal_moments = 0, opt_denoise_variance = 0;
};

static int fail(rtgl_context *ctx, int code, const std::string &msg)
{
    if (ctx) ctx->error = msg; else g_create_error = msg;
    return code;
}
#define HIPCHK(ctx, expr) do { hipError_t e_ = (expr); if (e_ != hipSuccess) \
    return fail(ctx, RTGL_ERR_DEVICE, std::string(#expr) + ": " + hipGetErrorString(e_)); } while (0)

#define RCCHK(expr) do { const int rc_ = (expr); if (rc_) return rc_; } while (0)

static int buf_rc(rtgl_context *ctx, const char *what, int e) { return e ? fail(ctx, RTGL_ERR_DEVICE, std::string(what) + ": " + hipGetErrorString((hipError_t)e)) : RTGL_OK; }
template <typename T> static int buf_alloc(rtgl_context *ctx, T *&p, size_t bytes) { return buf_rc(ctx, "device allocation", ctx->buffers.allocate((void **)&p, bytes)); }
template <typename T> static int buf_ensure(rtgl_context *ctx, T *&p, size_t bytes) { return buf_rc(ctx, "device allocation", ctx->buffers.ensure((void **)&p, bytes)); }
template <typename T, typename C> static int buf_grow(rtgl_context *ctx, T *&p, C &capacity, size_t need, size_t bytes) { return buf_rc(ctx, "device allocation", ctx->buffers.grow((void **)&p, capacity, (C)need, bytes)); }
template <typename... T> static int buf_release(rtgl_context *ctx, T *&...p)
{
    int e = 0;
    ((e = e ? e : ctx->buffers.release((void **)&p)), ...);
    return buf_rc(ctx, "device free", e);
}

static size_t local_px(const rtgl_context *ctx) { return (size_t)std::max(ctx->local_rows, 1) * ctx->width; }

static int read_rows(rtgl_context *ctx, void *dst, const void *src, size_t px_bytes)
{
    HIPCHK(ctx, hipMemcpyAsync(dst, src, (size_t)ctx->local_rows * ctx->width * px_bytes, hipMemcpyDeviceToHost, ctx->stream));
    HIPCHK(ctx, hipStreamSynchronize(ctx->stream));
    return RTGL_OK;
}

template <typename T>
static int realloc_upload(rtgl_context *ctx, T *&dptr, const void *src, size_t bytes)
{
    if (bytes == 0) return buf_release(ctx, dptr);
    RCCHK(buf_alloc(ctx, dptr, bytes));
    if (src) HIPCHK(ctx, hipMemcpyAsync(dptr, src, bytes, hipMemcpyHostToDevice, ctx->stream));
    HIPCHK(ctx, hipStreamSynchronize(ctx->stream));
    return RTGL_OK;
}

static int local_rows_for(int height, int rank, int world, int strip_rows)
{
    int n_strips = (height + strip_rows - 1) / strip_rows, rows = 0;
    for (int s = rank; s < n_strips; s += world) rows += std::min(strip_rows, height - s * strip_rows);
    return rows;
}

static std::mutex g_stream_mutex;
static std::map<int, std::pair<hipStream_t, int>> g_device_streams;
static hipError_t acquire_device_stream(int device, hipStream_t *out, bool *shared)
{
    const char *priv = getenv("RTGL_AMD_PRIVATE_STREAMS");
    if (priv && atoi(priv) != 0) { *shared = false; return hipStreamCreateWithFlags(out, hipStreamNonBlocking); }
    std::lock_guard<std::mutex> lock(g_stream_mutex);
    auto it = g_device_streams.find(device);
    if (it == g_device_streams.end()) {
        hipStream_t st = nullptr;
        const hipError_t e = hipStreamCreateWithFlags(&st, hipStreamNonBlocking);
        if (e != hipSuccess) return e;
        it = g_device_streams.emplace(device, std::make_pair(st, 0)).first;
    }
    it->second.second++;
    *out = it->second.first; *shared = true;
    return hipSuccess;
}
static std::map<const rtgl_context *, std::pair<int, hipStream_t>> g_ctx_streams;
static void register_ctx_stream(const rtgl_context *ctx, int device, hipStream_t st)
{
    std::lock_guard<std::mutex> lock(g_stream_mutex);
    g_ctx_streams[ctx] = std::make_pair(device, st);
}
static void unregister_ctx_stream(const rtgl_context *ctx)
{
    std::lock_guard<std::mutex> lock(g_stream_mutex);
    g_ctx_streams.erase(ctx);
}
static bool other_stream_in_use(const rtgl_context *ctx, int device, hipStream_t st)
{
    std::lock_guard<std::mutex> lock(g_stream_mutex);
    for (const auto &kv : g_ctx_streams) if (kv.first != ctx && kv.second.first == device && kv.second.second != st) return true;
    return false;
}
static bool concurrent_pipelines_allowed()
{
    const char *a = getenv("RTGL_AMD_ALLOW_CONCURRENT_PIPELINES"), *p = getenv("RTGL_AMD_PRIVATE_STREAMS");
    return (a && atoi(a) != 0) || (p && atoi(p) != 0);
}

static void release_device_stream(int device, hipStream_t st, bool shared)
{
    if (!shared) { (void)hipStreamDestroy(st); return; }
    std::lock_guard<std::mutex> lock(g_stream_mutex);
    auto it = g_device_streams.find(device);
    if (it != g_device_streams.end() && --it->second.second == 0) { (void)hipStreamDestroy(it->second.first); g_device_streams.erase(it); }
}

extern "C" int rtgl_create_tiled(rtgl_context **out, int width, int height, int device, int rank, int world, int strip_rows)
{
    if (!out) return fail(nullptr, RTGL_ERR_INVALID, "out is NULL");
    *out = nullptr;
    if (width <= 0 || height <= 0 || world < 1 || rank < 0 || rank >= world || strip_rows <= 0 || (strip_rows % 8) != 0)
        return fail(nullptr, RTGL_ERR_INVALID, "rtgl_create: bad size / tiling arguments");
    int ndev = 0;
    if (hipGetDeviceCount(&ndev) != hipSuccess || ndev <= 0)
        return fail(nullptr, RTGL_ERR_NO_DEVICE, "no HIP device visible (this library has no CPU path)");
    if (device < 0 || device >= ndev) return fail(nullptr, RTGL_ERR_INVALID, "device ordinal out of range");
    rtgl_context *ctx = new rtgl_context();
    ctx->device = device; ctx->width = width; ctx->height = height;
    ctx->rank = rank; ctx->world = world; ctx->strip_rows = strip_rows;
    ctx->local_rows = local_rows_for(height, rank, world, strip_rows);
    auto bail = [&](int code) { g_create_error = ctx->error; rtgl_destroy(ctx); return code; };
#define CCHK(expr) do { hipError_t e_ = (expr); if (e_ != hipSuccess) { \
    ctx->error = std::string(#expr) + ": " + hipGetErrorString(e_); return bail(RTGL_ERR_DEVICE); } } while (0)
    CCHK(hipSetDevice(device));
    { hipDeviceProp_t prop; if (hipGetDeviceProperties(&prop, device) == hipSuccess && prop.multiProcessorCount > 0) ctx->n_cus = prop.multiProcessorCount; }
    CCHK(acquire_device_stream(device, &ctx->own_stream, &ctx->own_stream_shared));
    ctx->stream = ctx->own_stream;
    register_ctx_stream(ctx, device, ctx->stream);
    CCHK(hipEventCreate(&ctx->ev0));
    CCHK(hipEventCreate(&ctx->ev1));
    size_t img_bytes = local_px(ctx) * sizeof(float4);
    if (buf_alloc(ctx, ctx->d_image_own, img_bytes)) return bail(RTGL_ERR_DEVICE);
    CCHK(hipMemsetAsync(ctx->d_image_own, 0, img_bytes, ctx->stream));
    ctx->d_image = ctx->d_image_own;
    if (buf_alloc(ctx, ctx->d_counters, 64)) return bail(RTGL_ERR_DEVICE);
    CCHK(hipMemsetAsync(ctx->d_counters, 0, 64, ctx->stream));
    CCHK(hipStreamSynchronize(ctx->stream));
#undef CCHK
    if (const char *k = getenv("RTGL_AMD_KERNEL")) { const int v = atoi(k); if (v >= RTGL_KERNEL_MEGA && v <= RTGL_KERNEL_WAVEFRONT_MFMA_SOLO && v != RTGL_KERNEL_REMOVED_3) { ctx->opt_kernel = v; ctx->kernel_explicit = true; } }
    if (const char *k = getenv("RTGL_AMD_SCAN_WAVES")) { const int v = atoi(k); if (v >= 0 && v <= 2) ctx->opt_scan_waves = v; }
    if (const char *k = getenv("RTGL_AMD_FRAME_BATCH")) { const int v = atoi(k); if (v >= 1 && v <= (int)kBatchMax) ctx->opt_frame_batch = v; }
    if (const char *k = getenv("RTGL_AMD_SCAN_DYNAMIC")) { const int v = atoi(k); if (v >= 0 && v <= 4) ctx->opt_scan_dynamic = v; }
    if (const char *k = getenv("RTGL_AMD_NARROW_FUSED")) { const int v = atoi(k); if (v == 0 || v == 1) ctx->opt_narrow_fused = v; }
    if (const char *k = getenv("RTGL_AMD_SORT_MOVE")) { const int v = atoi(k); if (v == 0 || v == 1) ctx->opt_sort_move = v; }
    if (const char *k = getenv("RTGL_AMD_CAMERA_LEAN")) { const int v = atoi(k); if (v == 0 || v == 1) ctx->opt_camera_lean = v; }
    if (const char *k = getenv("RTGL_AMD_SHADE_PASS")) { const int v = atoi(k); if (v == 0 || v == 1) ctx->opt_shade_pass = v; }
    *out = ctx;
    return RTGL_OK;
}

static int flush_pending(rtgl_context *ctx);
extern "C" int rtgl_create(rtgl_context **out, int width, int height, int device)
{
    return rtgl_create_tiled(out, width, height, device, 0, 1, 8);
}

extern "C" void rtgl_destroy(rtgl_context *ctx)
{
    if (!ctx) return;
    if (!ctx->pending.empty() && hipSetDevice(ctx->device) == hipSuccess && flush_pending(ctx) != RTGL_OK)
        fprintf(stderr, "rtgl_destroy: %zu batched frame(s) could not be submitted: %s\n", ctx->pending.size(), ctx->error.c_str());
    unregister_ctx_stream(ctx);
    for (auto &w : ctx->workers) {
        { std::lock_guard<std::mutex> lk(w->m); w->state = PartWorker::kQuit; }
        w->cv.notify_all();
        if (w->th.joinable()) w->th.join();
    }
    ctx->workers.clear();
    for (rtgl_context *part : ctx->parts) rtgl_destroy(part);
    ctx->parts.clear();
    (void)hipSetDevice(ctx->device);
    for (hipEvent_t e : ctx->part_done) (void)hipEventDestroy(e);
    if (ctx->gather_done) (void)hipEventDestroy(ctx->gather_done);
    if (ctx->stream) (void)hipStreamSynchronize(ctx->stream);
#ifdef RT_SOLO_STAMPS
    if (ctx->d_dbg_log) {
        unsigned long long h[16 * 64];
        if (hipMemcpy(h, ctx->d_dbg_log, sizeof h, hipMemcpyDeviceToHost) == hipSuccess)
            for (int b = 0; b < 64 && h[16 * b + 8]; ++b) {
                const unsigned long long *d = h + 16 * b; const double tot = (double)d[0];
                fprintf(stderr, "rtgl stamps bounce %2d: waves %llu iters %llu  cycles/wave %.0f  staging %.1f%% rays %.1f%% segments %.1f%% (of the wave: set-up %.1f%%, park %.1f%%) flush %.1f%%  cycles per tile-stage in steady %.1f  slowest wave of a launch (mean over launches) %.0f  culled items %llu at %.0f cycles\n",
                        b, d[8], d[7], tot / d[8], 100.0 * d[1] / tot, 100.0 * d[2] / tot, 100.0 * d[4] / tot, 100.0 * d[3] / tot, 100.0 * d[5] / tot, 100.0 * d[6] / tot,
                        d[9] ? (double)d[4] / (double)d[9] : 0.0, (double)d[13] * (double)d[15] / (double)d[8], d[12], d[12] ? (double)d[11] / (double)d[12] : 0.0);
            }
#if RT_SOLO_STAMPS == 3
        if (hipMemcpy(h, ctx->d_dbg_log, sizeof h, hipMemcpyDeviceToHost) == hipSuccess) {
            double cyc = 0, ticks = 0;
            for (int b = 0; b < 64 && h[16 * b + 8]; ++b) {
                const unsigned long long *d = h + 16 * b;
                fprintf(stderr, "rtgl clock bounce %2d: %llu waves, %.0f shader cycles per wave over %.0f ticks of 10 ns: %.3f GHz\n", b, d[8], (double)d[0] / d[8], (double)d[14] / d[8], d[14] ? (double)d[0] / (double)d[14] * 0.1 : 0.0);
                cyc += (double)d[0]; ticks += (double)d[14];
            }
            if (ticks > 0) fprintf(stderr, "rtgl clock: in-kernel shader clock of scan_solo_kernel, wave-time weighted over all launches: %.3f GHz\n", cyc / ticks * 0.1);
        }
#endif
        std::vector<unsigned long long> pc(16 * 64 * 2 * 16);
        if (hipMemcpy(pc.data(), reinterpret_cast<unsigned long long *>(ctx->d_dbg_log) + 2048, pc.size() * 8, hipMemcpyDeviceToHost) == hipSuccess)
            for (int b = 0; b < 8; ++b) {
                double tot = 0, cnt = 0; int nch = 0;
                for (int c = 0; c < 64; ++c) { const unsigned long long *e = pc.data() + ((size_t)16 * b * 64 + c) * 2; if (e[1]) { tot += (double)e[0]; cnt += (double)e[1]; nch = c + 1; } }
                if (cnt == 0) continue;
                fprintf(stderr, "rtgl stamps bounce %2d: mean wave time per chunk / bounce mean:", b);
                for (int c = 0; c < nch; ++c) { const unsigned long long *e = pc.data() + ((size_t)16 * b * 64 + c) * 2; fprintf(stderr, " %.2f", e[1] ? ((double)e[0] / (double)e[1]) / (tot / cnt) : 0.0); }
                fprintf(stderr, "\n");
            }
    }
#endif
    ctx->buffers.release_all();
    for (hipEvent_t e : ctx->kev) (void)hipEventDestroy(e);
    if (ctx->h_counts) (void)hipHostFree(ctx->h_counts);
    if (ctx->counts_ev) (void)hipEventDestroy(ctx->counts_ev);
    if (ctx->ev0) (void)hipEventDestroy(ctx->ev0);
    if (ctx->ev1) (void)hipEventDestroy(ctx->ev1);
    if (ctx->own_stream) release_device_stream(ctx->device, ctx->own_stream, ctx->own_stream_shared);
    delete ctx;
}

extern "C" const char *rtgl_last_error(const rtgl_context *ctx) { return ctx ? ctx->error.c_str() : g_create_error.c_str(); }

#define ENTER_NOFLUSH(ctx) do { if (!(ctx)) return RTGL_ERR_INVALID; HIPCHK(ctx, hipSetDevice((ctx)->device)); } while (0)
#define ENTER(ctx) do { ENTER_NOFLUSH(ctx); if (!(ctx)->pending.empty()) { const int rcf_ = flush_pending(ctx); if (rcf_) return rcf_; } } while (0)
#define FANOUT(ctx, call) do { if (!(ctx)->parts.empty()) { (ctx)->gathered = false; \
    for (rtgl_context *part : (ctx)->parts) { const int rc_ = (call); if (rc_) return fail(ctx, rc_, std::string("device ") + std::to_string(part->device) + ": " + part->error); } \
    return RTGL_OK; } } while (0)

extern "C" int rtgl_create_multi(rtgl_context **out, int width, int height, const int *devices, int n_devices, int strip_rows)
{
    if (!out) return fail(nullptr, RTGL_ERR_INVALID, "out is NULL");
    *out = nullptr;
    if (!devices || n_devices < 1 || n_devices > 64) return fail(nullptr, RTGL_ERR_INVALID, "rtgl_create_multi: need 1..64 device ordinals");
    rtgl_context *ctx = nullptr;
    int rc = rtgl_create_tiled(&ctx, width, height, devices[0], 0, 1, strip_rows);
    if (rc) return rc;
    for (int i = 0; i < n_devices; ++i) {
        rtgl_context *part = nullptr;
        rc = rtgl_create_tiled(&part, width, height, devices[i], i, n_devices, strip_rows);
        if (rc) { const std::string msg = g_create_error; rtgl_destroy(ctx); g_create_error = msg; return rc; }
        ctx->parts.push_back(part);
        hipEvent_t ev = nullptr;
        (void)hipSetDevice(devices[i]);
        if (hipEventCreateWithFlags(&ev, hipEventDisableTiming) != hipSuccess) { rtgl_destroy(ctx); return fail(nullptr, RTGL_ERR_DEVICE, "hipEventCreate failed"); }
        ctx->part_done.push_back(ev);
        if (devices[i] != devices[0]) {
            int can = 0;
            (void)hipSetDevice(devices[0]);
            if (hipDeviceCanAccessPeer(&can, devices[0], devices[i]) != hipSuccess || !can) ctx->peer_copy = false;
            else { hipError_t e = hipDeviceEnablePeerAccess(devices[i], 0); if (e != hipSuccess && e != hipErrorPeerAccessAlreadyEnabled) ctx->peer_copy = false; }
            (void)hipGetLastError();
        }
    }
    const char *mt = getenv("RTGL_AMD_MULTI_THREADS");
    if (n_devices > 1 && !(mt && atoi(mt) == 0)) try {
        for (rtgl_context *part : ctx->parts) {
            ctx->workers.emplace_back(new PartWorker);
            PartWorker *w = ctx->workers.back().get();
            w->part = part;
            w->th = std::thread([w] {
                std::unique_lock<std::mutex> lk(w->m);
                for (;;) {
                    w->cv.wait(lk, [w] { return w->state == PartWorker::kJob || w->state == PartWorker::kQuit; });
                    if (w->state == PartWorker::kQuit) return;
                    lk.unlock();
                    const int rc = rtgl_render_frame(w->part);
                    lk.lock();
                    w->rc = rc; w->state = PartWorker::kDone;
                    w->cv.notify_all();
                }
            });
        }
    } catch (const std::exception &) {
        for (auto &w : ctx->workers) {
            { std::lock_guard<std::mutex> lk(w->m); w->state = PartWorker::kQuit; }
            w->cv.notify_all();
            if (w->th.joinable()) w->th.join();
        }
        ctx->workers.clear();
    }
    *out = ctx;
    return RTGL_OK;
}

extern "C" int rtgl_device_count(const rtgl_context *ctx) { return ctx ? (ctx->parts.empty() ? 1 : (int)ctx->parts.size()) : RTGL_ERR_INVALID; }

static int multi_gather(rtgl_context *ctx)
{
    if (ctx->gathered) return RTGL_OK;
    const int world = (int)ctx->parts.size(), sr = ctx->strip_rows;
    const size_t row_bytes = (size_t)ctx->width * 16, strip_bytes = row_bytes * sr;
    std::vector<float> host;
    for (int i = 0; i < world; ++i) {
        rtgl_context *part = ctx->parts[i];
        if (!part->pending.empty()) { HIPCHK(ctx, hipSetDevice(part->device)); const int rc = flush_pending(part); if (rc) return fail(ctx, rc, part->error); }
        const int full = part->local_rows / sr, tail_rows = part->local_rows - full * sr;
        uint8_t *dst = reinterpret_cast<uint8_t *>(ctx->d_image) + (size_t)i * strip_bytes;
        const uint8_t *src = reinterpret_cast<const uint8_t *>(part->d_image);
        if (ctx->peer_copy) {
            HIPCHK(ctx, hipSetDevice(part->device));
            HIPCHK(ctx, hipEventRecord(ctx->part_done[i], part->stream));
            HIPCHK(ctx, hipSetDevice(ctx->device));
            HIPCHK(ctx, hipStreamWaitEvent(ctx->stream, ctx->part_done[i], 0));
            if (full) HIPCHK(ctx, hipMemcpy2DAsync(dst, (size_t)world * strip_bytes, src, strip_bytes, strip_bytes, (size_t)full, hipMemcpyDeviceToDevice, ctx->stream));
            if (tail_rows) HIPCHK(ctx, hipMemcpyAsync(dst + (size_t)full * world * strip_bytes, src + (size_t)full * strip_bytes, row_bytes * tail_rows, hipMemcpyDeviceToDevice, ctx->stream));
        } else {
            host.resize((size_t)part->local_rows * ctx->width * 4);
            int rc = rtgl_read_image_f32(part, host.data());
            if (rc) return fail(ctx, rc, part->error);
            HIPCHK(ctx, hipSetDevice(ctx->device));
            if (full) HIPCHK(ctx, hipMemcpy2DAsync(dst, (size_t)world * strip_bytes, host.data(), strip_bytes, strip_bytes, (size_t)full, hipMemcpyHostToDevice, ctx->stream));
            if (tail_rows) HIPCHK(ctx, hipMemcpyAsync(dst + (size_t)full * world * strip_bytes, reinterpret_cast<const uint8_t *>(host.data()) + (size_t)full * strip_bytes, row_bytes * tail_rows, hipMemcpyHostToDevice, ctx->stream));
            HIPCHK(ctx, hipStreamSynchronize(ctx->stream));
        }
    }
    HIPCHK(ctx, hipSetDevice(ctx->device));
    if (ctx->peer_copy) {
        if (!ctx->gather_done) HIPCHK(ctx, hipEventCreateWithFlags(&ctx->gather_done, hipEventDisableTiming));
        HIPCHK(ctx, hipEventRecord(ctx->gather_done, ctx->stream));
        for (rtgl_context *part : ctx->parts)
            if (part->stream != ctx->stream) {
                HIPCHK(ctx, hipSetDevice(part->device));
                HIPCHK(ctx, hipStreamWaitEvent(part->stream, ctx->gather_done, 0));
            }
        HIPCHK(ctx, hipSetDevice(ctx->device));
    }
    ctx->gathered = true;
    return RTGL_OK;
}

extern "C" int rtgl_gather_tiles(rtgl_context *ctx)
{
    ENTER(ctx);
    if (ctx->parts.empty()) return RTGL_OK;
    return multi_gather(ctx);
}

extern "C" int rtgl_upload_spheres(rtgl_context *ctx, const void *data, uint32_t count)
{
    ENTER(ctx);
    FANOUT(ctx, rtgl_upload_spheres(part, data, count));
    if (count && !data) return fail(ctx, RTGL_ERR_INVALID, "spheres is NULL");
    static_assert(sizeof(SphereRec) == 32, "Sphere stride (shaders/raytracer.glsl:11-15, std140)");
    int rc = realloc_upload(ctx, ctx->d_spheres, data, (size_t)count * 32);
    if (rc) return rc;
    ctx->n_spheres = count; ctx->visits_dirty = true;
    return RTGL_OK;
}

extern "C" int rtgl_upload_materials(rtgl_context *ctx, const void *data, uint32_t count)
{
    ENTER(ctx);
    FANOUT(ctx, rtgl_upload_materials(part, data, count));
    if (count && !data) return fail(ctx, RTGL_ERR_INVALID, "materials is NULL");
    static_assert(sizeof(MaterialRec) == 32, "Material stride (shaders/raytracer.glsl:17-21, std140)");
    int rc = realloc_upload(ctx, ctx->d_materials, data, (size_t)count * 32);
    if (rc) return rc;
    ctx->n_materials = count;
    return RTGL_OK;
}

extern "C" int rtgl_upload_meshes(rtgl_context *ctx, const void *data, uint32_t count)
{
    ENTER(ctx);
    FANOUT(ctx, rtgl_upload_meshes(part, data, count));
    if (count && !data) return fail(ctx, RTGL_ERR_INVALID, "meshes is NULL");
// ... 281 lines not shown
        const size_t px = local_px(ctx), q_bytes = (size_t)n0 * (68 + 8), bytes = 2 * q_bytes + 1024 + (multi_sample ? px * 64 : 0);
        RCCHK(buf_grow(ctx, ctx->d_wave, ctx->wave_capacity, n0, bytes));
        ctx->wave_multi = multi_sample;
        uint8_t *p = (uint8_t *)ctx->d_wave;
        for (int q = 0; q < 2; ++q) {
            ctx->wb.q[q].a = (float4 *)p; p += (size_t)n0 * 16;
            ctx->wb.q[q].b = (float4 *)p; p += (size_t)n0 * 16;
            ctx->wb.q[q].c = (float4 *)p; p += (size_t)n0 * 16;
            ctx->wb.q[q].rng = (uint4 *)p; p += (size_t)n0 * 16;
        }
        for (int q = 0; q < 2; ++q) { ctx->wb.best[q] = (unsigned long long *)p; p += (size_t)n0 * 8; }
        for (int q = 0; q < 2; ++q) { ctx->wb.q[q].pixel = (uint32_t *)p; p += (size_t)n0 * 4; }
        p = (uint8_t *)(((uintptr_t)p + 255) & ~(uintptr_t)255);
        if (multi_sample) {
            ctx->wb.sums = (float4 *)p; p += px * 16;
            ctx->wb.cam_a = (float4 *)p; p += px * 16;
            ctx->wb.cam_b = (float4 *)p; p += px * 16;
            ctx->wb.pix_rng = (uint4 *)p; p += px * 16;
        } else ctx->wb.sums = ctx->wb.cam_a = ctx->wb.cam_b = nullptr, ctx->wb.pix_rng = nullptr;
    }
    ctx->wb.counts = ctx->d_counts;
    ctx->wb.cand_peak = ctx->d_counts + ctx->counts_capacity;
    ctx->wb.group_bounds = ctx->d_group_bounds;
    return RTGL_OK;
}

template <int R, int MODE>
static void launch_bounce(rtgl_context *ctx, const SceneView &sc, const FrameParams &P, const ImageView &im, uint32_t n0, uint32_t bounce, uint4 *rng_out, const AovView *aov)
{
    dim3 grid((n0 + 256u * R - 1) / (256u * R));
    if (aov) {
        if (ctx->opt_counters) hipLaunchKernelGGL((bounce_kernel<R, MODE, true, true>), grid, dim3(256), 0, ctx->stream, sc, P, im, ctx->wb, bounce, rng_out, ctx->d_counters, *aov);
        else hipLaunchKernelGGL((bounce_kernel<R, MODE, false, true>), grid, dim3(256), 0, ctx->stream, sc, P, im, ctx->wb, bounce, rng_out, ctx->d_counters, *aov);
    } else if (ctx->opt_counters)
        hipLaunchKernelGGL((bounce_kernel<R, MODE, true, false>), grid, dim3(256), 0, ctx->stream, sc, P, im, ctx->wb, bounce, rng_out, ctx->d_counters, AovView{});
    else
        hipLaunchKernelGGL((bounce_kernel<R, MODE, false, false>), grid, dim3(256), 0, ctx->stream, sc, P, im, ctx->wb, bounce, rng_out, ctx->d_counters, AovView{});
}

template <bool kSort>
static void launch_shade(rtgl_context *ctx, const rt_shade_launch::Launch &L, const SceneView &sc, const FrameParams &P, const ImageView &im, uint32_t bounce, uint4 *rng_out, const AovView *aov)
{
    using ShadeKernel = decltype(&shade_kernel<false, kSort, false>);
    static const ShadeKernel kKernels[2][2][2] = {
        {{shade_stride_kernel<false, kSort, false>, shade_stride_kernel<false, kSort, true>}, {shade_stride_kernel<true, kSort, false>, shade_stride_kernel<true, kSort, true>}},
        {{shade_kernel<false, kSort, false>, shade_kernel<false, kSort, true>}, {shade_kernel<true, kSort, false>, shade_kernel<true, kSort, true>}}};
    if (L.one_pass) ctx->shade_pass_launches++;
    hipLaunchKernelGGL(kKernels[L.one_pass][ctx->opt_counters != 0][aov != nullptr], dim3(L.blocks), dim3(256), 0, ctx->stream, sc, P, im, ctx->wb, bounce, rng_out, ctx->d_counters, aov ? *aov : AovView{});
}

template <bool kSort>
static void launch_shade_camera(rtgl_context *ctx, uint32_t n0, const SceneView &sc, const FrameParams &P, const ImageView &im, uint4 *rng_out)
{
    const dim3 grid((n0 + 255u) / 256u);
    if (ctx->opt_counters) hipLaunchKernelGGL((shade_camera_kernel<true, kSort>), grid, dim3(256), 0, ctx->stream, sc, P, im, ctx->wb, rng_out, ctx->d_counters);
    else hipLaunchKernelGGL((shade_camera_kernel<false, kSort>), grid, dim3(256), 0, ctx->stream, sc, P, im, ctx->wb, rng_out, ctx->d_counters);
}

static uint32_t estimate_rays(const rtgl_context *ctx, uint32_t n0, uint32_t bounce)
{
    if (bounce == 0 || bounce >= ctx->est_counts.size()) return n0;
    uint64_t e = (uint64_t)ctx->est_counts[bounce] + ctx->est_counts[bounce] / 10 + 2048;
    return (uint32_t)std::min<uint64_t>(e, n0);
}

template <int R, int MODE>
static void launch_intersect(rtgl_context *ctx, const SceneView &sc, uint32_t n0, uint32_t bounce)
{
    const uint32_t chunk = (uint32_t)ctx->opt_wf_chunk;
    const uint32_t est = estimate_rays(ctx, n0, bounce);
    dim3 grid((est + 256u * R - 1) / (256u * R), (sc.n_tri_visits + chunk - 1) / chunk);
    const bool early = bounce < (uint32_t)ctx->opt_wf_early;
#define RTGL_LAUNCH_ISECT(E, P, C) hipLaunchKernelGGL((intersect_kernel<R, MODE, E, P, C>), grid, dim3(256), 0, ctx->stream, sc, ctx->wb, bounce, chunk, ctx->d_counters)
    if (early) { if (ctx->opt_counters) RTGL_LAUNCH_ISECT(true, false, true); else RTGL_LAUNCH_ISECT(true, false, false); }
    else if (ctx->opt_wf_packed) { if (ctx->opt_counters) RTGL_LAUNCH_ISECT(false, true, true); else RTGL_LAUNCH_ISECT(false, true, false); }
    else { if (ctx->opt_counters) RTGL_LAUNCH_ISECT(false, false, true); else RTGL_LAUNCH_ISECT(false, false, false); }
#undef RTGL_LAUNCH_ISECT
}

using CameraKeep = rt_camera_keep::Decision;
static rt_camera_keep::Camera keep_camera(const FrameParams &P)
{
    rt_camera_keep::Camera c{};
    c.use_dof = P.use_dof; c.fov = P.cam_fov; c.aperture = P.cam_aperture; c.focal = P.cam_focal;
    memcpy(c.pos, P.cam_pos, sizeof c.pos); memcpy(c.forward, P.cam_forward, sizeof c.forward); memcpy(c.up, P.cam_up, sizeof c.up); memcpy(c.right, P.cam_right, sizeof c.right);
    return c;
}
static int camera_keep_decide(rtgl_context *ctx, uint32_t n0, const FrameParams *cam, CameraKeep *ck)
{
    const rt_scan_launch::Setup setup = scan_setup(ctx);
    rt_camera_keep::Frame f{};
    f.culled = rt_scan_launch::culls(setup, 0u, false); f.single = cam != nullptr; f.enabled = !getenv("RTGL_AMD_NO_CAMERA_KEEP");
    f.n0 = n0; f.words = ctx->wb.keep_words; f.scene = ctx->scene_version;
    if (cam) f.camera = keep_camera(*cam);
    const size_t need = rt_scan_launch::capacity(setup).keep_count(n0);
    f.room = ctx->keep0_capacity >= need;
    const rt_camera_keep::Key key{ctx->keep0_valid, ctx->keep0_n0, ctx->keep0_words, ctx->keep0_scene, ctx->keep0_camera};
    *ck = rt_camera_keep::decide(key, f);
    if (!ck->cached) return RTGL_OK;
    if (!ck->have_bits) ctx->keep0_valid = false;
    return buf_grow(ctx, ctx->d_keep0, ctx->keep0_capacity, need, need * sizeof(uint32_t));
}

using ScanKernel = decltype(&scan_solo_kernel<false, 1, 0>);
#define RTGL_SCAN_DISTS(C, WW) {scan_solo_kernel<C, WW, 0>, scan_solo_kernel<C, WW, 1>, scan_solo_kernel<C, WW, 2>, scan_solo_kernel<C, WW, 3>}
static const ScanKernel kScanKernels[2][2][4] = {{RTGL_SCAN_DISTS(false, 1), RTGL_SCAN_DISTS(false, 2)}, {RTGL_SCAN_DISTS(true, 1), RTGL_SCAN_DISTS(true, 2)}};
#undef RTGL_SCAN_DISTS

static int launch_intersect_solo(rtgl_context *ctx, const SceneView &sc, uint32_t n0, uint32_t bounce, bool binned, const CameraKeep *ck, const FrameParams *cam)
{
    const rt_scan_launch::Setup setup = scan_setup(ctx);
    const uint64_t items_per_wave = getenv("RTGL_AMD_ITEMS_PER_WAVE") ? (uint64_t)std::max(1, atoi(getenv("RTGL_AMD_ITEMS_PER_WAVE"))) : 3ull;
    const rt_scan_launch::Launch L = rt_scan_launch::launch(setup, items_per_wave, n0, estimate_rays(ctx, n0, bounce), bounce, binned);

#ifdef RT_SOLO_STAMPS
    if (!ctx->d_dbg_log) { RCCHK(buf_alloc(ctx, ctx->d_dbg_log, (size_t)(2 + (2u << 22)) * 4)); HIPCHK(ctx, hipMemsetAsync(ctx->d_dbg_log, 0, 2048 * 8 + 16 * 64 * 2 * 16 * 8, ctx->stream)); }
#endif
    MfView mf{ctx->d_mf_groups, ctx->n_mf_groups, ctx->mf_group_quads, ctx->n_mf_groups * ctx->mf_group_quads, ctx->d_mf_A, ctx->d_dbg_log, ctx->d_mf_cull, ctx->d_edges_s, ctx->d_planes_s, ctx->d_mf_order};
    if (!ctx->solo_attr_set) {
        for (const auto &by_w : kScanKernels) for (const auto &by_dist : by_w) for (const ScanKernel k : by_dist) {
            const void *fn = reinterpret_cast<const void *>(k);
            hipFuncAttributes fattr;
            HIPCHK(ctx, hipFuncGetAttributes(&fattr, fn));
            HIPCHK(ctx, hipFuncSetAttribute(fn, hipFuncAttributeMaxDynamicSharedMemorySize, (int)(160 * 1024 - fattr.sharedSizeBytes)));
        }
        ctx->solo_attr_set = true;
    }
    float ro_add = 0.0f, sigma_add = 0.0f; bool have_bits = false;
    const bool cached = L.cull && bounce == 0 && ck && cam && ck->cached;
    if (L.cull) {
        if (cached) { ctx->wb.keep = ctx->d_keep0; have_bits = ck->have_bits; ro_add = ck->ro_add; sigma_add = ck->sigma_add; }
        else ctx->wb.keep = ctx->d_keep;
        if (L.dist == 2) {
            RCCHK(buf_grow(ctx, ctx->d_plan, ctx->plan_capacity, L.plan_need, L.plan_need));
            ctx->wb.plan_prefix = reinterpret_cast<uint32_t *>(ctx->d_plan); ctx->wb.plan_stride = L.stride;
            ctx->wb.plan_total = reinterpret_cast<uint32_t *>(reinterpret_cast<uint8_t *>(ctx->d_plan) + L.plan_off_tot);
            ctx->wb.plan_base = reinterpret_cast<unsigned long long *>(reinterpret_cast<uint8_t *>(ctx->d_plan) + L.plan_off_base);
        }
        if (L.dist == 1) {
            RCCHK(buf_grow(ctx, ctx->d_items, ctx->items_capacity, L.items_need, L.items_need));
            ctx->wb.item_counts = reinterpret_cast<uint32_t *>(ctx->d_items);
            ctx->wb.items = reinterpret_cast<uint32_t *>(reinterpret_cast<uint8_t *>(ctx->d_items) + L.items_head);
            ctx->wb.items_stride = L.stride;
        }
    }

    if (L.cull) {
        if (!have_bits) {
            hipLaunchKernelGGL(packet_cull_kernel, dim3(L.cull_blocks), dim3(256), 0, ctx->stream, ctx->wb, ctx->d_mf_cull, setup.real_quads * (uint32_t)kMfQuadTiles, bounce, ro_add, sigma_add,
                               ctx->d_mf_cull_node, ctx->d_mf_cull_node ? ctx->cull_node_shift : 0u, (uint32_t)(binned && ctx->opt_sort_move == 1));
            if (cached) {
                HIPCHK(ctx, hipGetLastError());
                ctx->keep0_valid = true; ctx->keep0_n0 = n0; ctx->keep0_words = ctx->wb.keep_words; ctx->keep0_scene = ctx->scene_version; ctx->keep0_camera = keep_camera(*cam);
            }
        }
        if (L.dist == 2) {
            hipLaunchKernelGGL(ctx->opt_counters ? scan_plan_kernel<true> : scan_plan_kernel<false>, dim3(L.chunks), dim3(256), 0, ctx->stream, ctx->wb, bounce, L.chunk_quads, setup.real_quads, ctx->d_counters);
            hipLaunchKernelGGL(scan_plan_base_kernel, dim3(1), dim3(64), 0, ctx->stream, ctx->wb, L.chunks);
        }
        if (L.dist == 1) {
            HIPCHK(ctx, hipMemsetAsync(ctx->wb.item_counts, 0, (size_t)L.chunks * sizeof(uint32_t), ctx->stream));
            hipLaunchKernelGGL(ctx->opt_counters ? cull_items_kernel<true> : cull_items_kernel<false>, dim3(L.items_grid_x, L.items_grid_y), dim3(256), 0, ctx->stream, ctx->wb, bounce, L.chunk_quads, setup.real_quads, ctx->d_counters);
        }
    }
#ifdef RT_SOLO_STAMPS
    const int fused = 0;
#else
    const int fused = ctx->opt_narrow_fused;
#endif
    hipLaunchKernelGGL(kScanKernels[ctx->opt_counters != 0][L.W - 1][L.dist], dim3(L.blocks), dim3(256 * L.W), L.lds, ctx->stream, sc, ctx->wb, mf, bounce, L.chunk_quads, L.chunks, ctx->d_counters, ctx->opt_debug_skip_exact, L.cull, fused);
    HIPCHK(ctx, hipGetLastError());
    if (!fused) hipLaunchKernelGGL(narrow_phase_kernel, dim3(L.blocks * L.waves, kNarrowSplit), dim3(256), 0, ctx->stream, sc, ctx->wb, mf, bounce, L.blocks * L.waves);
    return RTGL_OK;
}

static int launch_wavefront(rtgl_context *ctx, const SceneView &sc, const std::vector<FrameParams> &frames, const ImageView &im, uint32_t n0_frame, uint4 *rng_out,
                            const AovView *aov, const uint32_t *masked = nullptr)
{
    const FrameParams &P = frames[0];
    const uint32_t B = (uint32_t)frames.size(), n0 = n0_frame * B;
    const dim3 gen_grid((n0_frame + 255) / 256);
    if (ctx->counts_pending && hipEventQuery(ctx->counts_ev) == hipSuccess) {
        ctx->counts_pending = false;
        if (ctx->counts_n0 == n0) ctx->est_counts.assign(ctx->h_counts, ctx->h_counts + ctx->counts_len);
        else ctx->est_counts.clear();
        const uint32_t peak = ctx->h_counts[ctx->counts_capacity];
        if (!ctx->cand_fixed && peak > ctx->cand_region_pairs) ctx->cand_region_target = (uint32_t)std::min<uint64_t>((uint64_t)peak + peak / 4, 0xFFFFFFF0u);
    }
    CameraKeep ck{};
    const FrameParams *const cam = (B == 1 && P.samples == 1u && !masked) ? &P : nullptr;
    if (ctx->opt_kernel == RTGL_KERNEL_WAVEFRONT_MFMA_SOLO && sc.n_tri_visits > 0 && P.max_bounce > 0) RCCHK(camera_keep_decide(ctx, n0, cam, &ck));
    const bool lean = rt_camera_keep::lean(ck, ctx->opt_camera_lean, aov != nullptr);
    if (lean) ctx->camera_lean_frames++;
    for (uint32_t s = 0; s < P.samples; ++s) {
        const uint32_t n_counts = ctx->counts_capacity + 1u <= 256u ? ctx->counts_capacity + 1u : 0u;
        if (!n_counts) HIPCHK(ctx, hipMemsetAsync(ctx->d_counts, 0, counts_bytes(ctx->counts_capacity), ctx->stream));
        uint32_t n_sched = 0u;
        if (ctx->opt_kernel == RTGL_KERNEL_WAVEFRONT_MFMA_SOLO && ctx->d_sched && rt_scan_launch::uses_claim_counters(rt_scan_launch::mesh_dist(scan_setup(ctx)))) {
            const size_t words = (size_t)(P.max_bounce + 2) * ctx->wb.sched_stride;
            if (words <= (size_t)gen_grid.x * 256u && !getenv("RTGL_AMD_SCHED_FILL")) n_sched = (uint32_t)words;
            else HIPCHK(ctx, hipMemsetAsync(ctx->d_sched, 0, words * sizeof(uint32_t), ctx->stream));
        }
        if (masked)
            hipLaunchKernelGGL(generate_rays_masked_kernel, gen_grid, dim3(256), 0, ctx->stream, P, im, ctx->wb, masked, n0_frame, ctx->opt_counters ? ctx->d_counters : (Counters *)nullptr, n_counts, n_sched);
        else for (uint32_t f = 0; f < B; ++f)
            hipLaunchKernelGGL(generate_rays_kernel, gen_grid, dim3(256), 0, ctx->stream, frames[f], im, ctx->wb, s, n0_frame,
                               ctx->opt_counters ? ctx->d_counters : (Counters *)nullptr, f == 0 ? n_counts : 0u, f * n0_frame, B > 1 ? f << 28 : 0u, f == 0 ? n0 : 0u, f == 0 ? n_sched : 0u,
                               lean ? 1u : 0u);
        bool binned = false;
        for (uint32_t b = 0; b < P.max_bounce; ++b) {
            const int key = ctx->opt_wf_mode * 10 + ctx->opt_wf_rays;
            const AovView *aov_b = (s == 0u && b == 0u) ? aov : nullptr;
            if (ctx->opt_kernel == RTGL_KERNEL_WAVEFRONT_SPLIT || ctx->opt_kernel == RTGL_KERNEL_WAVEFRONT_MFMA_SOLO) {
                if (sc.n_tri_visits > 0 && ctx->opt_kernel == RTGL_KERNEL_WAVEFRONT_MFMA_SOLO) {
                    kev_mark(ctx);
                    { const int rc = launch_intersect_solo(ctx, sc, n0, b, binned, b == 0u ? &ck : nullptr, cam); if (rc) return rc; }
                    kev_mark(ctx);
                } else if (sc.n_tri_visits > 0) {
                    kev_mark(ctx);
                    switch (key) {
                    case 1: launch_intersect<1, kScalar>(ctx, sc, n0, b); break;
                    case 2: launch_intersect<2, kScalar>(ctx, sc, n0, b); break;
                    case 4: launch_intersect<4, kScalar>(ctx, sc, n0, b); break;
                    case 8: launch_intersect<8, kScalar>(ctx, sc, n0, b); break;
                    case 11: launch_intersect<1, kLds>(ctx, sc, n0, b); break;
                    case 12: launch_intersect<2, kLds>(ctx, sc, n0, b); break;
                    case 14: launch_intersect<4, kLds>(ctx, sc, n0, b); break;
                    case 18: launch_intersect<8, kLds>(ctx, sc, n0, b); break;
                    default: return fail(ctx, RTGL_ERR_STATE, "unsupported wf_mode / wf_rays combination");
                    }
                    kev_mark(ctx);
                }
                const uint32_t est_next = estimate_rays(ctx, n0, b + 1u);
                const bool bin_next = ctx->opt_kernel == RTGL_KERNEL_WAVEFRONT_MFMA_SOLO && ctx->opt_cull == 3 && sc.n_tri_visits > 0 && b + 1u < P.max_bounce
                                      && est_next >= (uint32_t)ctx->opt_sort_min_rays;
                const rt_shade_launch::Launch shade = rt_shade_launch::launch(ctx->opt_shade_pass, n0, estimate_rays(ctx, n0, b), bin_next);
                if (bin_next) {
                    const size_t bins = (size_t)1 << ctx->wb.sort_bits, set_words = bins + bins / kSortSeg;
                    if (!ctx->sort_sets_clean || ctx->sort_set_bits != ctx->wb.sort_bits) {
                        HIPCHK(ctx, hipMemsetAsync(ctx->d_sort_hist, 0, 2 * set_words * sizeof(uint32_t), ctx->stream));
                        ctx->sort_set = 0; ctx->sort_set_bits = ctx->wb.sort_bits;
                    }
                    ctx->sort_sets_clean = false;
                    if (getenv("RTGL_AMD_HIST_FILL")) HIPCHK(ctx, hipMemsetAsync(ctx->d_sort_hist + (size_t)ctx->sort_set * set_words, 0, bins * sizeof(uint32_t), ctx->stream));
                    ctx->wb.sort_hist = ctx->d_sort_hist + (size_t)ctx->sort_set * set_words;
                    ctx->wb.sort_hist_other = ctx->d_sort_hist + (size_t)(ctx->sort_set ^ 1) * set_words;
                    if (lean && b == 0u) launch_shade_camera<true>(ctx, n0, sc, P, im, rng_out);
                    else launch_shade<true>(ctx, shade, sc, P, im, b, rng_out, aov_b);
                    hipLaunchKernelGGL(sort_sums_kernel, dim3((unsigned)(bins / kSortSeg)), dim3(256), 0, ctx->stream, ctx->wb);
                    hipLaunchKernelGGL(sort_prefix_kernel, dim3((unsigned)(bins / kSortSeg)), dim3(256), 0, ctx->stream, ctx->wb);
                    if (ctx->opt_sort_move == 1) hipLaunchKernelGGL(sort_place_kernel, dim3(std::max(1u, std::min((est_next + 255u) / 256u, 16384u))), dim3(256), 0, ctx->stream, ctx->wb, b + 1u);
                    else hipLaunchKernelGGL(sort_scatter_kernel, dim3(std::max(1u, std::min((est_next + 255u) / 256u, 16384u))), dim3(256), 0, ctx->stream, ctx->wb, b + 1u);
                    HIPCHK(ctx, hipGetLastError());
                    ctx->sort_set ^= 1; ctx->sort_sets_clean = true;
                } else if (lean && b == 0u) launch_shade_camera<false>(ctx, n0, sc, P, im, rng_out);
                else launch_shade<false>(ctx, shade, sc, P, im, b, rng_out, aov_b);
                binned = bin_next;
                continue;
            }
            kev_mark(ctx);
            switch (key) {
            case 1: launch_bounce<1, kScalar>(ctx, sc, P, im, n0, b, rng_out, aov_b); break;
            case 2: launch_bounce<2, kScalar>(ctx, sc, P, im, n0, b, rng_out, aov_b); break;
            case 4: launch_bounce<4, kScalar>(ctx, sc, P, im, n0, b, rng_out, aov_b); break;
            case 11: launch_bounce<1, kLds>(ctx, sc, P, im, n0, b, rng_out, aov_b); break;
            case 12: launch_bounce<2, kLds>(ctx, sc, P, im, n0, b, rng_out, aov_b); break;
            case 14: launch_bounce<4, kLds>(ctx, sc, P, im, n0, b, rng_out, aov_b); break;
            default: return fail(ctx, RTGL_ERR_STATE, "unsupported wf_mode / wf_rays combination");
            }
            kev_mark(ctx);
        }
        HIPCHK(ctx, hipGetLastError());
    }
    if (P.samples > 1u) {
        hipLaunchKernelGGL(resolve_kernel, gen_grid, dim3(256), 0, ctx->stream, P, im, ctx->wb);
        HIPCHK(ctx, hipGetLastError());
    }
    if (B > 1) {
        BatchInfo bi{};
        bi.n = B;
        for (uint32_t f = 0; f < B; ++f) { bi.frames[f] = frames[f].frames; bi.reset[f] = frames[f].reset_flag; }
        hipLaunchKernelGGL(resolve_batch_kernel, gen_grid, dim3(256), 0, ctx->stream, im, ctx->wb, bi);
        HIPCHK(ctx, hipGetLastError());
    }
    if (!ctx->counts_pending) {
        ctx->counts_len = P.max_bounce + 1; ctx->counts_n0 = n0;
        HIPCHK(ctx, hipMemcpyAsync(ctx->h_counts, ctx->d_counts, counts_bytes(ctx->counts_capacity), hipMemcpyDeviceToHost, ctx->stream));
        HIPCHK(ctx, hipEventRecord(ctx->counts_ev, ctx->stream));
        ctx->counts_pending = true;
    }
    return RTGL_OK;
}

extern "C" int rtgl_set_frame_params(rtgl_context *ctx, const rtgl_frame_params *p)
{
    ENTER_NOFLUSH(ctx);
    FANOUT(ctx, rtgl_set_frame_params(part, p));
    if (!p) return fail(ctx, RTGL_ERR_INVALID, "params is NULL");
    static_assert(sizeof(FrameParams) == sizeof(rtgl_frame_params), "FrameParams mirrors rtgl_frame_params");
    memcpy(&ctx->params, p, sizeof(FrameParams));
    ctx->have_params = true;
    return RTGL_OK;
}

static int render_batch(rtgl_context *ctx, const std::vector<FrameParams> &batch);

static bool batch_compatible(const FrameParams &a, const FrameParams &b)
{
    return a.samples == b.samples && a.max_bounce == b.max_bounce && a.use_envmap == b.use_envmap && memcmp(a.background, b.background, sizeof a.background) == 0;
}

static int flush_pending(rtgl_context *ctx)
{
    if (ctx->pending.empty()) return RTGL_OK;
    std::vector<FrameParams> batch;
    batch.swap(ctx->pending);
    return render_batch(ctx, batch);
}

extern "C" int rtgl_render_frame(rtgl_context *ctx)
{
    ENTER_NOFLUSH(ctx);
    if (!ctx->workers.empty()) {
        ctx->gathered = false;
        for (auto &w : ctx->workers) { { std::lock_guard<std::mutex> lk(w->m); w->state = PartWorker::kJob; } w->cv.notify_all(); }
        int first = RTGL_OK; const rtgl_context *bad = nullptr;
        for (auto &w : ctx->workers) {
            std::unique_lock<std::mutex> lk(w->m);
            w->cv.wait(lk, [&w] { return w->state == PartWorker::kDone; });
            w->state = PartWorker::kIdle;
            if (w->rc && !first) { first = w->rc; bad = w->part; }
        }
        return first ? fail(ctx, first, std::string("device ") + std::to_string(bad->device) + ": " + bad->error) : RTGL_OK;
    }
    FANOUT(ctx, rtgl_render_frame(part));
    if (!ctx->have_params) return fail(ctx, RTGL_ERR_STATE, "rtgl_set_frame_params has not been called");
    if (ctx->params.samples == 0) return fail(ctx, RTGL_ERR_INVALID, "u_samples == 0 divides by zero in the reference; refused");
    ctx->ad_active = false;
    const bool batchable = ctx->opt_frame_batch > 1 && ctx->params.samples == 1 && ctx->params.max_bounce > 0 && !ctx->opt_counters && !ctx->opt_rng_state
                           && !ctx->opt_kernel_timing && !ctx->opt_aov && (ctx->n_tri_visits > 0 || ctx->tris_dirty || ctx->kernel_explicit) && ctx->opt_kernel != RTGL_KERNEL_MEGA;
    if (!ctx->pending.empty() && (!batchable || !batch_compatible(ctx->pending.front(), ctx->params))) { const int rc = flush_pending(ctx); if (rc) return rc; }
    if (batchable) {
        ctx->pending.push_back(ctx->params);
        return (int)ctx->pending.size() >= ctx->opt_frame_batch ? flush_pending(ctx) : RTGL_OK;
    }
    return render_batch(ctx, std::vector<FrameParams>(1, ctx->params));
}

static SceneView scene_view(const rtgl_context *ctx)
{
    SceneView sc{};
    sc.spheres = ctx->d_spheres; sc.n_spheres = ctx->n_spheres;
    sc.sphere_visits = ctx->d_sphere_visits; sc.n_sphere_visits = ctx->n_sphere_visits;
    sc.materials = ctx->d_materials; sc.n_materials = ctx->n_materials;
    sc.tri_edges = ctx->d_edges; sc.tri_planes = ctx->d_planes; sc.n_tri_visits = ctx->n_tri_visits;
    sc.env = ctx->d_env; sc.env_w = ctx->env_w; sc.env_h = ctx->env_h; sc.env_c = ctx->env_c; sc.env_faces = ctx->env_faces;
    return sc;
}

static int render_batch(rtgl_context *ctx, const std::vector<FrameParams> &batch)
{
    const uint32_t B = (uint32_t)batch.size();
    for (const FrameParams &f : batch) {
        if (f.reset_flag) ++ctx->err_epoch;
        ctx->err_fn = f.frames; ctx->err_rendered = true;
    }
    if (ctx->visits_dirty) { int rc = rebuild_sphere_visits(ctx); if (rc) return rc; }
    if (ctx->tris_dirty) { int rc = rebuild_triangles(ctx); if (rc) return rc; }
    if (ctx->opt_rng_state) RCCHK(buf_ensure(ctx, ctx->d_rng, local_px(ctx) * sizeof(uint4)));
    if ((ctx->opt_aov & RTGL_AOV_IDS) && ctx->visit_ids_dirty) {
        const size_t bytes = ctx->h_visit_tri.size() * sizeof(uint32_t);
        int rc = realloc_upload(ctx, ctx->d_visit_mesh, ctx->h_visit_mesh.data(), bytes);
        if (!rc) rc = realloc_upload(ctx, ctx->d_visit_tri, ctx->h_visit_tri.data(), bytes);
        if (rc) return rc;
        ctx->visit_ids_dirty = false;
    }

    const SceneView sc = scene_view(ctx);
    std::vector<FrameParams> frames(batch);
    for (FrameParams &f : frames) if (!ctx->d_env) f.use_envmap = 0;
    const FrameParams &P = frames[0];
    ImageView im{};
    im.pixels = ctx->d_image; im.width = ctx->width; im.height = ctx->height;
    im.disp_w = ctx->width / 8 * 8; im.disp_h = ctx->height / 8 * 8;
    im.local_rows = ctx->local_rows; im.rank = ctx->rank; im.world = ctx->world; im.strip_rows = ctx->strip_rows;

    if (ctx->opt_counters) HIPCHK(ctx, hipMemsetAsync(ctx->d_counters, 0, sizeof(Counters), ctx->stream));
    int local_disp_rows = 0;
    for (int lr = 0; lr < ctx->local_rows; ++lr) if (rtgl_local_row_to_global(ctx, lr) < im.disp_h) local_disp_rows = lr + 1;
    const uint32_t n0_frame = (uint32_t)im.disp_w * (uint32_t)local_disp_rows;
    if ((uint64_t)n0_frame * B > 0xFFFFFFF0ull || local_px(ctx) > (size_t)kBatchPixelMask) return fail(ctx, RTGL_ERR_INVALID, "frame_batch: the batch does not fit 32-bit ray slots");
    const uint32_t n0 = n0_frame * B;
    uint4 *rng_out = ctx->opt_rng_state ? ctx->d_rng : nullptr;
    AovView aov{};
    if (ctx->opt_aov) {
        ctx->aov_n = (P.reset_flag || ctx->aov_restart) ? 1u : ctx->aov_n + 1u;
        ctx->aov_restart = false;
        aov.albedo = ctx->d_aov[0]; aov.normal = ctx->d_aov[1]; aov.position = ctx->d_aov[2]; aov.ids = ctx->d_aov_ids;
        aov.visit_mesh = ctx->d_visit_mesh; aov.visit_tri = ctx->d_visit_tri; aov.n = ctx->aov_n;
    }
    const int kernel = (ctx->n_tri_visits == 0 && !ctx->kernel_explicit) ? (int)RTGL_KERNEL_MEGA : ctx->opt_kernel;
    const bool use_wavefront = kernel != RTGL_KERNEL_MEGA && P.max_bounce > 0;
    ctx->kernel_in_use = use_wavefront ? kernel : (int)RTGL_KERNEL_MEGA;
    if (B > 1 && !(use_wavefront && n0 > 0)) {
        for (const FrameParams &f : batch) { const int rc = render_batch(ctx, std::vector<FrameParams>(1, f)); if (rc) return rc; }
        return RTGL_OK;
    }
    if (use_wavefront && n0 > 0) { int rc = ensure_wave_buffers(ctx, n0, P.max_bounce, P.samples > 1); if (rc) return rc; }
    ctx->wb.batch_rad = nullptr; ctx->wb.batch_px = 0;
    if (B > 1) {
        const size_t need = local_px(ctx) * B;
        RCCHK(buf_grow(ctx, ctx->d_batch_rad, ctx->batch_capacity, need, need * sizeof(float4)));
        ctx->wb.batch_rad = ctx->d_batch_rad; ctx->wb.batch_px = (uint32_t)local_px(ctx);
    }
    ctx->last_batch_frames = B;
    HIPCHK(ctx, hipEventRecord(ctx->ev0, ctx->stream));
    ctx->timing_this_frame = ctx->opt_kernel_timing > 0 && (ctx->timing_frame_counter++ % (uint32_t)ctx->opt_kernel_timing) == 0u;
    if (ctx->timing_this_frame) {
        if (ctx->kev_frame_start.size() >= 4096) { ctx->kev_used = 0; ctx->kev_frame_start.clear(); }
        ctx->kev_frame_start.push_back(ctx->kev_used);
        kev_mark(ctx);
    }
    if (n0 > 0 && !use_wavefront) {
        dim3 grid((im.disp_w + 31) / 32, (local_disp_rows + 7) / 8);
        kev_mark(ctx);
        if (ctx->opt_aov) {
            if (ctx->opt_counters) hipLaunchKernelGGL((pathtrace_mega_kernel<true, true>), grid, dim3(256), 0, ctx->stream, sc, P, im, rng_out, ctx->d_counters, aov);
            else hipLaunchKernelGGL((pathtrace_mega_kernel<false, true>), grid, dim3(256), 0, ctx->stream, sc, P, im, rng_out, ctx->d_counters, aov);
        } else if (ctx->opt_counters)
            hipLaunchKernelGGL((pathtrace_mega_kernel<true, false>), grid, dim3(256), 0, ctx->stream, sc, P, im, rng_out, ctx->d_counters, AovView{});
        else
            hipLaunchKernelGGL((pathtrace_mega_kernel<false, false>), grid, dim3(256), 0, ctx->stream, sc, P, im, rng_out, ctx->d_counters, AovView{});
        kev_mark(ctx);
        HIPCHK(ctx, hipGetLastError());
    } else if (n0 > 0) {
        int rc = launch_wavefront(ctx, sc, frames, im, n0_frame, rng_out, ctx->opt_aov ? &aov : nullptr);
        if (rc) { ctx->keep0_valid = false; return rc; }
    }
    HIPCHK(ctx, hipEventRecord(ctx->ev1, ctx->stream));
    kev_mark(ctx);
// ... 1135 lines not shown
        HIPCHK(ctx, hipGetLastError());
    }
    if (!to_image) ctx->rb_resolved = true;
    return RTGL_OK;
}

extern "C" int rtgl_robust_end(rtgl_context *ctx)
{
    ENTER(ctx);
    if (!ctx->rb_active) return fail(ctx, RTGL_ERR_STATE, std::string("rtgl_robust_end") + kNoRobustSession);
    HIPCHK(ctx, hipStreamSynchronize(ctx->stream));
    ctx->rb_active = false; ctx->rb_resolved = false; ctx->has_rb_error = false; ctx->rb_K = 0; ctx->rb_N = 0;
    return buf_release(ctx, ctx->d_rb_buckets, ctx->d_rb_out, ctx->d_rbe_tiles, ctx->d_rbe_summary);
}

extern "C" int rtgl_robust_frames(rtgl_context *ctx, uint32_t *frames, uint32_t *buckets)
{
    ENTER_NOFLUSH(ctx);
    if (!frames && !buckets) return fail(ctx, RTGL_ERR_INVALID, "rtgl_robust_frames: both pointers are NULL");
    if (!ctx->rb_active) return fail(ctx, RTGL_ERR_STATE, std::string("rtgl_robust_frames") + kNoRobustSession);
    if (frames) *frames = ctx->rb_N;
    if (buckets) *buckets = ctx->rb_K;
    return RTGL_OK;
}

extern "C" int rtgl_read_robust_f32(rtgl_context *ctx, float *rgba)
{
    ENTER(ctx);
    if (!rgba) return fail(ctx, RTGL_ERR_INVALID, "rgba is NULL");
    if (!ctx->rb_active) return fail(ctx, RTGL_ERR_STATE, std::string("rtgl_read_robust_f32") + kNoRobustSession);
    if (!ctx->rb_resolved) return fail(ctx, RTGL_ERR_STATE, "rtgl_read_robust_f32: no rtgl_robust_resolve with dest RTGL_ROBUST_DEST_BUFFER since rtgl_robust_begin");
    return read_rows(ctx, rgba, ctx->d_rb_out, 16);
}

extern "C" int rtgl_read_robust_bucket_f32(rtgl_context *ctx, uint32_t bucket, float *rgba)
{
    ENTER(ctx);
    if (!rgba) return fail(ctx, RTGL_ERR_INVALID, "rgba is NULL");
    if (!ctx->rb_active) return fail(ctx, RTGL_ERR_STATE, std::string("rtgl_read_robust_bucket_f32") + kNoRobustSession);
    if (bucket >= ctx->rb_K) return fail(ctx, RTGL_ERR_INVALID, "rtgl_read_robust_bucket_f32: bucket >= buckets");
    return read_rows(ctx, rgba, ctx->d_rb_buckets + (size_t)bucket * rt_robust_plan::plane_pixels(ctx->local_rows, ctx->width), 16);
}

static_assert(sizeof(rtgl_robust_error_params) == sizeof(rt_spread_plan::Params) && offsetof(rtgl_robust_error_params, quantile_permille) == offsetof(rt_spread_plan::Params, quantile_permille)
              && rt_spread_plan::kSummaryBytes == kErrSummaryWords * 4 && rt_spread_plan::kRecordBytes == sizeof(uint4) && rt_spread_plan::kTile == (uint32_t)kErrTile, "the layouts of the header");

extern "C" int rtgl_robust_error_defaults(rtgl_robust_error_params *out)
{
    if (!out) return RTGL_ERR_INVALID;
    const rt_spread_plan::Params p = rt_spread_plan::default_params();
    memcpy(out, &p, sizeof p);
    return RTGL_OK;
}

extern "C" int rtgl_robust_error_estimate(rtgl_context *ctx, const rtgl_robust_error_params *params)
{
    ENTER(ctx);
    rt_spread_plan::Params P = rt_spread_plan::default_params();
    if (params) memcpy(&P, params, sizeof P);
    if (const char *why = rt_spread_plan::invalid(P)) return fail(ctx, RTGL_ERR_INVALID, std::string("rtgl_robust_error_estimate: ") + why);
    if (!ctx->parts.empty() || ctx->world > 1)
        return fail(ctx, RTGL_ERR_STATE, "rtgl_robust_error_estimate: a tiled or multi-device context holds strips, and the estimate is of the whole picture (out of scope): render on a single-device context");
    if (const char *why = rt_spread_plan::refused(ctx->rb_active, ctx->rb_N, ctx->rb_K)) return fail(ctx, RTGL_ERR_STATE, std::string("rtgl_robust_error_estimate: ") + why);
    if (!rt_spread_plan::footprint_fits(ctx->width, ctx->height)) return fail(ctx, RTGL_ERR_INVALID, "rtgl_robust_error_estimate: the footprint does not fit 32-bit counts");
    const unsigned tx = rt_spread_plan::tiles_along(ctx->width), ty = rt_spread_plan::tiles_along(ctx->height);
    RCCHK(buf_ensure(ctx, ctx->d_rbe_tiles, rt_spread_plan::record_bytes(ctx->width, ctx->height)));
    RCCHK(buf_ensure(ctx, ctx->d_rbe_summary, rt_spread_plan::kSummaryBytes));
    SpreadTilesArgs a{};
    a.buckets = ctx->d_rb_buckets; a.tiles = ctx->d_rbe_tiles; a.plane = rt_robust_plan::plane_pixels(ctx->local_rows, ctx->width);
    a.width = ctx->width; a.fw = (int32_t)rt_spread_plan::footprint_side(ctx->width); a.fh = (int32_t)rt_spread_plan::footprint_side(ctx->height);
    a.gain = P.gain; a.floor_ = P.floor; a.threshold = P.threshold;
    ErrorSolveArgs s{};
    s.tiles = ctx->d_rbe_tiles; s.summary = ctx->d_rbe_summary; s.n_tiles = tx * ty; s.valid = 1u;
    s.frames_now = (int32_t)ctx->rb_N; s.frames_snapshot = 0;
    s.footprint = (uint32_t)rt_spread_plan::footprint(ctx->width, ctx->height); s.quantile_permille = P.quantile_permille; s.c = 1.0f;
    const dim3 grid(tx, ty);
    if (ctx->rb_K == 4u) hipLaunchKernelGGL(spread_tiles_kernel<4>, grid, dim3(256), 0, ctx->stream, a);
    else if (ctx->rb_K == 8u) hipLaunchKernelGGL(spread_tiles_kernel<8>, grid, dim3(256), 0, ctx->stream, a);
    else hipLaunchKernelGGL(spread_tiles_kernel<16>, grid, dim3(256), 0, ctx->stream, a);
    HIPCHK(ctx, hipGetLastError());
    hipLaunchKernelGGL(error_solve_kernel, dim3(1), dim3(256), 0, ctx->stream, s);
    HIPCHK(ctx, hipGetLastError());
    ctx->has_rb_error = true;
    return RTGL_OK;
}

static const char *const kNoRobustError = ": no rtgl_robust_error_estimate call has succeeded in this session";

extern "C" int rtgl_read_robust_error_summary(rtgl_context *ctx, rtgl_error_summary *out)
{
    ENTER(ctx);
    if (!out) return fail(ctx, RTGL_ERR_INVALID, "out is NULL");
    if (!ctx->rb_active || !ctx->has_rb_error) return fail(ctx, RTGL_ERR_STATE, std::string("rtgl_read_robust_error_summary") + kNoRobustError);
    HIPCHK(ctx, hipMemcpyAsync(out, ctx->d_rbe_summary, sizeof *out, hipMemcpyDeviceToHost, ctx->stream));
    HIPCHK(ctx, hipStreamSynchronize(ctx->stream));
    return RTGL_OK;
}

extern "C" int rtgl_read_robust_error_tiles(rtgl_context *ctx, rtgl_error_tile *tiles, uint32_t *tx, uint32_t *ty)
{
    ENTER(ctx);
    if (!tiles) return fail(ctx, RTGL_ERR_INVALID, "tiles is NULL");
    if (!ctx->rb_active || !ctx->has_rb_error) return fail(ctx, RTGL_ERR_STATE, std::string("rtgl_read_robust_error_tiles") + kNoRobustError);
    const uint32_t nx = rt_spread_plan::tiles_along(ctx->width), ny = rt_spread_plan::tiles_along(ctx->height);
    HIPCHK(ctx, hipMemcpyAsync(tiles, ctx->d_rbe_tiles, (size_t)nx * ny * sizeof(rtgl_error_tile), hipMemcpyDeviceToHost, ctx->stream));
    HIPCHK(ctx, hipStreamSynchronize(ctx->stream));
    if (tx) *tx = nx;
    if (ty) *ty = ny;
    return RTGL_OK;
}

extern "C" void *rtgl_device_robust_error_tiles(rtgl_context *ctx)
{
    if (!ctx) return nullptr;
    if (!ctx->rb_active || !ctx->has_rb_error) { ctx->error = std::string("rtgl_device_robust_error_tiles") + kNoRobustError; return nullptr; }
    return (void *)ctx->d_rbe_tiles;
}

extern "C" int rtgl_set_option(rtgl_context *ctx, const char *key, int value)
{
    ENTER(ctx);
    FANOUT(ctx, rtgl_set_option(part, key, value));
    if (!key) return fail(ctx, RTGL_ERR_INVALID, "key is NULL");
    if (!strcmp(key, "kernel")) {
        if (value == RTGL_KERNEL_REMOVED_3)
            return fail(ctx, RTGL_ERR_INVALID, "kernel variant 3 (three waves per SIMD) was removed: it was not deterministic (DESIGN.md section 5); use 4");
        if (value < RTGL_KERNEL_MEGA || value > RTGL_KERNEL_WAVEFRONT_MFMA_SOLO)
            return fail(ctx, RTGL_ERR_INVALID, "unknown kernel variant");
        ctx->opt_kernel = value; ctx->kernel_explicit = true;
    } else if (!strcmp(key, "wf_rays")) {
        if (value != 1 && value != 2 && value != 4 && value != 8) return fail(ctx, RTGL_ERR_INVALID, "wf_rays must be 1, 2, 4 or 8");
        ctx->opt_wf_rays = value;
    } else if (!strcmp(key, "wf_chunk")) {
        if (value < kBoundGroup || value % kBoundGroup || (uint32_t)value > kMaxChunk) return fail(ctx, RTGL_ERR_INVALID, "wf_chunk must be a multiple of 64 in [64, 4096]");
        ctx->opt_wf_chunk = value;
    } else if (!strcmp(key, "debug_skip_exact")) {
        if (value < 0 || value > 3) return fail(ctx, RTGL_ERR_INVALID, "debug_skip_exact must be 0, 1, 2 or 3");
        ctx->opt_debug_skip_exact = value;
    } else if (!strcmp(key, "mf_chunk_quads")) {
        if (value < 1 || (uint32_t)value > kMfMaxChunkQuads) return fail(ctx, RTGL_ERR_INVALID, "mf_chunk_quads must be in [1, 32]");
        ctx->opt_mf_chunk_quads = value;
    } else if (!strcmp(key, "scan_waves")) {
        if (value < 0 || value > 2) return fail(ctx, RTGL_ERR_INVALID, "scan_waves (waves per SIMD of the kernel-4 scan) must be 0 (default: two), 1 or 2");
        ctx->opt_scan_waves = value;
    } else if (!strcmp(key, "scan_dynamic")) {
        if (value < 0 || value > 4) return fail(ctx, RTGL_ERR_INVALID, "scan_dynamic must be 0 (chosen by the mesh), 1 (static turns), 2 (dynamic claims), 3 (planned: equal-cost intervals) or 4 (hybrid: turns + a claimed tail)");
        ctx->opt_scan_dynamic = value;
    } else if (!strcmp(key, "narrow_fused")) {
        if (value != 0 && value != 1) return fail(ctx, RTGL_ERR_INVALID, "narrow_fused must be 0 (narrow_phase_kernel tests the scan's survivors) or 1 (every scan wave tests its own at its end)");
        ctx->opt_narrow_fused = value;
    } else if (!strcmp(key, "camera_lean")) {
        if (value != 0 && value != 1) return fail(ctx, RTGL_ERR_INVALID, "camera_lean must be 0 (camera rays travel through queue 0 in full) or 1 (shade rebuilds them while the camera's keep bits are reused)");
        ctx->opt_camera_lean = value;
    } else if (!strcmp(key, "shade_pass")) {
        if (value != 0 && value != 1) return fail(ctx, RTGL_ERR_INVALID, "shade_pass must be 0 (every shade launch in grid-stride passes) or 1 (one pass, a block per 256 slots of queue 0, unless the queue is expected to be all but empty)");
        ctx->opt_shade_pass = value;
    } else if (!strcmp(key, "frame_batch")) {
        if (value < 1 || value > (int)kBatchMax) return fail(ctx, RTGL_ERR_INVALID, "frame_batch (consecutive frames traced in one set of launches) must be 1..16");
        ctx->opt_frame_batch = value;
    } else if (!strcmp(key, "cull")) {
        if (value < 0 || value > 3) return fail(ctx, RTGL_ERR_INVALID, "cull must be 0 (off), 1 (camera rays), 2 (every bounce, queues as they come) or 3 (camera rays + binned bounces)");
        ctx->opt_cull = value;
    } else if (!strcmp(key, "sort_min_rays")) {
        if (value < 0) return fail(ctx, RTGL_ERR_INVALID, "sort_min_rays (a bounce's queue is binned when at least this many rays are expected) must be >= 0");
        ctx->opt_sort_min_rays = value;
    } else if (!strcmp(key, "mf_group_quads")) {
        if (value < 1 || value > (int)kMfMaxGroupQuads || (value & (value - 1))) return fail(ctx, RTGL_ERR_INVALID, "mf_group_quads must be a power of two in [1, 64]");
        if (value != (int)ctx->mf_group_quads) ctx->tris_dirty = true;
        ctx->opt_mf_group_quads = value; ctx->group_explicit = true;
    } else if (!strcmp(key, "wf_packed")) {
        ctx->opt_wf_packed = value != 0;
    } else if (!strcmp(key, "wf_early")) {
        if (value < 0) return fail(ctx, RTGL_ERR_INVALID, "wf_early is the number of leading bounces with the wave-level edge short circuit (>= 0)");
        ctx->opt_wf_early = value;
    } else if (!strcmp(key, "wf_mode")) {
        if (value != kScalar && value != kLds) return fail(ctx, RTGL_ERR_INVALID, "wf_mode must be 0 (scalar) or 1 (lds)");
        ctx->opt_wf_mode = value;
    } else if (!strcmp(key, "aov")) {
        if (value < 0 || value > RTGL_AOV_ALL) return fail(ctx, RTGL_ERR_INVALID, "aov must be a mask of RTGL_AOV_ALBEDO | RTGL_AOV_NORMAL | RTGL_AOV_POSITION | RTGL_AOV_IDS (0: off)");
        const int rc = set_aov(ctx, value);
        if (rc) return rc;
    } else if (!strcmp(key, "denoise_source")) {
        if (value != 0 && value != 1) return fail(ctx, RTGL_ERR_INVALID, "denoise_source must be 0 (the accumulation image) or 1 (the latest history buffer of rtgl_temporal_accumulate)");
        ctx->opt_denoise_source = value;
    } else if (!strcmp(key, "temporal_moments")) {
        if (value < 0 || value > 2) return fail(ctx, RTGL_ERR_INVALID, "temporal_moments must be 0 (off), 1 (luminance moments of the radiance) or 2 (of the radiance divided by the albedo)");
        if (value != ctx->opt_temporal_moments) ctx->tm_valid = false;
        ctx->opt_temporal_moments = value;
    } else if (!strcmp(key, "denoise_variance")) {
        if (value != 0 && value != 1) return fail(ctx, RTGL_ERR_INVALID, "denoise_variance must be 0 (the spatial estimate) or 1 (the temporal moments where the history is long enough)");
        ctx->opt_denoise_variance = value;
    } else if (!strcmp(key, "rng_state")) ctx->opt_rng_state = value != 0;
    else if (!strcmp(key, "counters")) ctx->opt_counters = value != 0;
    else if (!strcmp(key, "kernel_timing")) {
        HIPCHK(ctx, hipStreamSynchronize(ctx->stream));
        if (value < 0) return fail(ctx, RTGL_ERR_INVALID, "kernel_timing must be 0 (off) or the sampling period in frames");
        ctx->opt_kernel_timing = value; ctx->kev_used = 0; ctx->kev_frame_start.clear(); ctx->timing_frame_counter = 0; ctx->timing_this_frame = false;
    } else return fail(ctx, RTGL_ERR_INVALID, std::string("unknown option ") + key);
    return RTGL_OK;
}

extern "C" int rtgl_get_option(rtgl_context *ctx, const char *key, int *value)
{
    ENTER(ctx);
    if (!key || !value) return fail(ctx, RTGL_ERR_INVALID, "NULL argument");
    if (!ctx->parts.empty()) { const int rc = rtgl_get_option(ctx->parts[0], key, value); return rc ? fail(ctx, rc, ctx->parts[0]->error) : RTGL_OK; }
    if (!strcmp(key, "kernel")) *value = ctx->opt_kernel;
    else if (!strcmp(key, "kernel_in_use")) *value = ctx->kernel_in_use;
    else if (!strcmp(key, "wf_rays")) *value = ctx->opt_wf_rays;
    else if (!strcmp(key, "wf_mode")) *value = ctx->opt_wf_mode;
    else if (!strcmp(key, "wf_chunk")) *value = ctx->opt_wf_chunk;
    else if (!strcmp(key, "wf_early")) *value = ctx->opt_wf_early;
    else if (!strcmp(key, "wf_packed")) *value = ctx->opt_wf_packed;
    else if (!strcmp(key, "mf_sets")) *value = kSoloSets;
    else if (!strcmp(key, "mf_chunk_quads")) *value = ctx->opt_mf_chunk_quads;
    else if (!strcmp(key, "mf_group_quads")) *value = (int)ctx->mf_group_quads;
    else if (!strcmp(key, "cull")) *value = ctx->opt_cull;
    else if (!strcmp(key, "sort_min_rays")) *value = ctx->opt_sort_min_rays;
    else if (!strcmp(key, "scan_waves")) *value = ctx->opt_scan_waves;
    else if (!strcmp(key, "scan_dynamic")) *value = ctx->opt_scan_dynamic;
    else if (!strcmp(key, "narrow_fused")) *value = ctx->opt_narrow_fused;
    else if (!strcmp(key, "frame_batch")) *value = ctx->opt_frame_batch;
    else if (!strcmp(key, "camera_lean")) *value = ctx->opt_camera_lean;
    else if (!strcmp(key, "camera_lean_frames")) *value = (int)ctx->camera_lean_frames;
    else if (!strcmp(key, "shade_pass")) *value = ctx->opt_shade_pass;
    else if (!strcmp(key, "shade_pass_launches")) *value = (int)ctx->shade_pass_launches;
    else if (!strcmp(key, "rng_state")) *value = ctx->opt_rng_state;
    else if (!strcmp(key, "aov")) *value = ctx->opt_aov;
    else if (!strcmp(key, "denoise_source")) *value = ctx->opt_denoise_source;
    else if (!strcmp(key, "temporal_moments")) *value = ctx->opt_temporal_moments;
    else if (!strcmp(key, "denoise_variance")) *value = ctx->opt_denoise_variance;
    else if (!strcmp(key, "counters")) *value = ctx->opt_counters;
    else if (!strcmp(key, "kernel_timing")) *value = ctx->opt_kernel_timing;
    else if (!strcmp(key, "cand_region_pairs")) *value = (int)ctx->cand_region_pairs;
    else if (!strcmp(key, "device_mbytes")) *value = (int)((ctx->buffers.total_bytes() + (1u << 20) - 1) >> 20);
    else return fail(ctx, RTGL_ERR_INVALID, std::string("unknown option ") + key);
    return RTGL_OK;
}
```

Before: 938.2 Mpaths/s.

## Scan camera-ray bounce granule by granule over sparse cached keep bits

Adds a sparse scan kernel for the camera-ray bounce. Each wave walks a 128-ray granule's cached keep bitmask and runs MFMA tests only on the tiles that are set, rather than scanning every chunk. A count kernel tallies kept bits once per cached keep mask, and the host reads the tally back asynchronously to decide when rows are sparse enough to use the new path. The ray-prep and group-operand code is pulled out into shared helpers, and drain_region is generalized over K. The cost is an extra count kernel, a host readback, and a separate kernel whose load balance may differ from the chunked scan.

```diff
diff --git a/raytracer.glsl_amd/csrc/rt_scan.hpp b/raytracer.glsl_amd/csrc/rt_scan.hpp
--- a/raytracer.glsl_amd/csrc/rt_scan.hpp
+++ b/raytracer.glsl_amd/csrc/rt_scan.hpp
@@ -183,10 +183,10 @@
 constexpr int kDrainFly = 4;
 typedef float drain_f4 __attribute__((ext_vector_type(4)));
 static_assert(sizeof(TriEdges) == 80 && sizeof(TriPlane) == 32 && alignof(TriEdges) == 16 && alignof(TriPlane) == 16, "drain_region reads these as rows of 16 bytes");
+template <int K = kDrainFly>
 __device__ __forceinline__ void drain_region(const SceneView &sc, const MfView &mf, const RayQueue &qin, unsigned long long *best,
                                              const unsigned long long *recs, uint32_t n_rec, uint32_t lane)
 {
-    constexpr int K = kDrainFly;
     const uint32_t last_tri = sc.n_tri_visits - 1u;
     for (uint32_t i0 = 0; i0 < n_rec; i0 += 64u * (uint32_t)K) {
         unsigned long long rec[K];
@@ -207,8 +207,8 @@
         TriRay tr[K];
 #pragma unroll
         for (int j = 0; j < K; ++j) { tr[j].o = mk(a[j].x, a[j].y, a[j].z); tr[j].d = mk(a[j].w, b[j].x, b[j].y); tr[j].cv = cross3(tr[j].d, tr[j].o); tr[j].ncv = tr[j].nd = 0.0f; }
-        while ((um[0] | um[1] | um[2] | um[3]) != 0u) {
-            static_assert(K == 4, "the loop condition names the masks");
+        auto masks_left = [&]() { uint32_t m = um[0]; for (int j = 1; j < K; ++j) m |= um[j]; return m; };
+        while (masks_left() != 0u) {
             bool on[K]; uint32_t p[K], v[K]; drain_f4 e[K][5], pl[K][2];
 #pragma unroll
             for (int j = 0; j < K; ++j) {
@@ -477,6 +477,47 @@
     if constexpr (kCount) { __shared__ unsigned long long words[kWaves]; return words; }
     else return nullptr;
 }
+template <bool kSplit>
+__device__ __forceinline__ void scan_prepare_ray(MfRay &r, const float4 &a, const float4 &b, bool valid, int half)
+{
+    r.valid = valid;
+    r.o = mk(a.x, a.y, a.z); r.d = mk(a.w, b.x, b.y);
+    r.wd = __builtin_amdgcn_sqrtf(dot3(r.d, r.d)) * 1.001f;
+    r.wod = (__builtin_amdgcn_sqrtf(dot3(r.o, r.o)) * 1.001f) * r.wd;
+    const uint32_t dxy = pack_bf16(r.d.x, r.d.y);
+    r.dyz = pack_bf16(r.d.y, r.d.z);
+    r.dx_hi = dxy << 16;
+    const f3 dl = mk(r.d.x - __uint_as_float(dxy << 16), r.d.y - __uint_as_float(dxy & 0xffff0000u), r.d.z - __uint_as_float(r.dyz & 0xffff0000u));
+    if constexpr (kSplit) { r.tail = pack_bf16(1.0f, dl.x); r.tail_hi = pack_bf16(dl.y, dl.z); }
+    else { r.tail = half ? pack_bf16(dl.y, dl.z) : pack_bf16(1.0f, dl.x); r.tail_hi = r.tail; }
+}
+template <bool kSplit, int H>
+__device__ __forceinline__ void scan_group_operands(const MfGroup &G, const MfRay (&ray)[H], int debug_skip_exact, u32x4 (&Bs)[4], float (&ths)[4])
+{
+#pragma unroll
+    for (int j = 0; j < H; ++j) {
+        const MfRay &r = ray[j];
+        const f3 ol = r.o - mk(G.cx, G.cy, G.cz);
+        const f3 cvl = cross3(r.d, ol);
+        const float ncv = __builtin_amdgcn_sqrtf(dot3(cvl, cvl)) * 1.001f, no = __builtin_amdgcn_sqrtf(dot3(ol, ol)) * 1.001f;
+        const float margin = mf_margin(G, ncv, no, r);
+        const float th = (!r.valid || debug_skip_exact == 2) ? __builtin_inff() : (margin < 1.0e30f ? -margin : __builtin_nanf(""));
+        const uint32_t bx = pack_bf16(cvl.x, cvl.y), by = (pack_bf16(cvl.z, 0.0f) & 0xffffu) | r.dx_hi;
+        if constexpr (!kSplit) {
+            Bs[j].x = bx; Bs[j].y = by; Bs[j].z = r.dyz; Bs[j].w = r.tail; ths[j] = th;
+        } else {
+            const auto px = __builtin_amdgcn_permlane32_swap(bx, bx, false, false);
+            const auto py = __builtin_amdgcn_permlane32_swap(by, by, false, false);
+            const auto pz = __builtin_amdgcn_permlane32_swap(r.dyz, r.dyz, false, false);
+            const auto pw = __builtin_amdgcn_permlane32_swap(r.tail, r.tail_hi, false, false);
+            const auto pt = __builtin_amdgcn_permlane32_swap(__float_as_uint(th), __float_as_uint(th), false, false);
+            const int s0 = 2 * j, s1 = 2 * j + 1;
+            Bs[s0].x = px[0]; Bs[s0].y = py[0]; Bs[s0].z = pz[0]; Bs[s0].w = pw[0]; ths[s0] = __uint_as_float(pt[0]);
+            Bs[s1].x = px[1]; Bs[s1].y = py[1]; Bs[s1].z = pz[1]; Bs[s1].w = pw[1]; ths[s1] = __uint_as_float(pt[1]);
+        }
+    }
+}
+
 template <bool kCount, int W, int kDist>
 __global__ void __launch_bounds__(256 * W) __attribute__((amdgpu_waves_per_eu(W, W)))
 scan_solo_kernel(SceneView sc, WaveBuffers wb, MfView mf, uint32_t bounce, uint32_t chunk_quads, uint32_t n_chunks, Counters *__restrict__ counters, int debug_skip_exact, int cull, int narrow_fused)
@@ -543,18 +584,7 @@
             if (slot < n_rays) { da[j] = qin.a[slot]; db[j] = qin.b[slot]; }
         }
     };
-    auto prepare_ray = [&](MfRay &r, const float4 &a, const float4 &b, bool valid) {
-        r.valid = valid;
-        r.o = mk(a.x, a.y, a.z); r.d = mk(a.w, b.x, b.y);
-        r.wd = __builtin_amdgcn_sqrtf(dot3(r.d, r.d)) * 1.001f;
-        r.wod = (__builtin_amdgcn_sqrtf(dot3(r.o, r.o)) * 1.001f) * r.wd;
-        const uint32_t dxy = pack_bf16(r.d.x, r.d.y);
-        r.dyz = pack_bf16(r.d.y, r.d.z);
-        r.dx_hi = dxy << 16;
-        const f3 dl = mk(r.d.x - __uint_as_float(dxy << 16), r.d.y - __uint_as_float(dxy & 0xffff0000u), r.d.z - __uint_as_float(r.dyz & 0xffff0000u));
-        if constexpr (kSplit) { r.tail = pack_bf16(1.0f, dl.x); r.tail_hi = pack_bf16(dl.y, dl.z); }
-        else { r.tail = half ? pack_bf16(dl.y, dl.z) : pack_bf16(1.0f, dl.x); r.tail_hi = r.tail; }
-    };
+    auto prepare_ray = [&](MfRay &r, const float4 &a, const float4 &b, bool valid) { scan_prepare_ray<kSplit>(r, a, b, valid, half); };
 
     constexpr uint32_t kXcds = 8;
     const bool by_xcd = gridDim.x >= kXcds * n_chunks;
@@ -771,28 +801,7 @@
                     for (int j = 0; j < H; ++j) prepare_ray(ray[j], nxt_a[j], nxt_b[j], wave_slot0 + (uint32_t)j * kRayStride + ray_lane < n_rays);
                 }
                 u32x4 Bs[S]; float ths[S];
-#pragma unroll
-                for (int j = 0; j < H; ++j) {
-                    const MfRay &r = ray[j];
-                    const f3 ol = r.o - mk(G.cx, G.cy, G.cz);
-                    const f3 cvl = cross3(r.d, ol);
-                    const float ncv = __builtin_amdgcn_sqrtf(dot3(cvl, cvl)) * 1.001f, no = __builtin_amdgcn_sqrtf(dot3(ol, ol)) * 1.001f;
-                    const float margin = mf_margin(G, ncv, no, r);
-                    const float th = (!r.valid || debug_skip_exact == 2) ? __builtin_inff() : (margin < 1.0e30f ? -margin : __builtin_nanf(""));
-                    const uint32_t bx = pack_bf16(cvl.x, cvl.y), by = (pack_bf16(cvl.z, 0.0f) & 0xffffu) | r.dx_hi;
-                    if constexpr (!kSplit) {
-                        Bs[j].x = bx; Bs[j].y = by; Bs[j].z = r.dyz; Bs[j].w = r.tail; ths[j] = th;
-                    } else {
-                        const auto px = __builtin_amdgcn_permlane32_swap(bx, bx, false, false);
-                        const auto py = __builtin_amdgcn_permlane32_swap(by, by, false, false);
-                        const auto pz = __builtin_amdgcn_permlane32_swap(r.dyz, r.dyz, false, false);
-                        const auto pw = __builtin_amdgcn_permlane32_swap(r.tail, r.tail_hi, false, false);
-                        const auto pt = __builtin_amdgcn_permlane32_swap(__float_as_uint(th), __float_as_uint(th), false, false);
-                        const int s0 = 2 * j, s1 = 2 * j + 1;
-                        Bs[s0].x = px[0]; Bs[s0].y = py[0]; Bs[s0].z = pz[0]; Bs[s0].w = pw[0]; ths[s0] = __uint_as_float(pt[0]);
-                        Bs[s1].x = px[1]; Bs[s1].y = py[1]; Bs[s1].z = pz[1]; Bs[s1].w = pw[1]; ths[s1] = __uint_as_float(pt[1]);
-                    }
-                }
+                scan_group_operands<kSplit, H>(G, ray, debug_skip_exact, Bs, ths);
                 B0 = Bs[0]; B1 = Bs[1]; B2 = Bs[2]; B3 = Bs[3];
                 th0 = ths[0]; th1 = ths[1]; th2 = ths[2]; th3 = ths[3];
 #if defined(RT_SOLO_STAMPS) && RT_SOLO_STAMPS == 1
diff --git a/raytracer.glsl_amd/csrc/rt_scan_sparse.hpp b/raytracer.glsl_amd/csrc/rt_scan_sparse.hpp
--- /dev/null
+++ b/raytracer.glsl_amd/csrc/rt_scan_sparse.hpp
@@ -0,0 +1,217 @@
+#pragma once
+#include "rt_scan.hpp"
+
+#pragma clang fp contract(off)
+
+namespace rt {
+
+struct SparseCfg {
+    static constexpr uint32_t kStepMax = 64u;
+    static constexpr uint32_t kDrain = 192u;
+    static constexpr uint32_t kQueue = kStepMax + kDrain + 1u;
+    static constexpr uint32_t kTileBits = 20u;
+};
+
+#define RT_SPARSE_TILE(AOP) \
+    asm volatile(RT_HEAD RT_MFMA(96, "%[a]", "%[b0]") RT_MFMA(112, "%[a]", "%[b1]") RT_MFMA(128, "%[a]", "%[b2]") RT_MFMA(144, "%[a]", "%[b3]") "s_nop 15\n\ts_nop 15\n\t" \
+                 RT_EXAM(96, 96, 36, "%[t0]") RT_EXAM(112, 112, 38, "%[t1]") RT_EXAM(128, 128, 40, "%[t2]") RT_EXAM(144, 144, 42, "%[t3]") "s_nop 7\n\t" RT_FOLD("%[any]", 36) \
+                 : "=&{v[96:111]}"(X0), "=&{v[112:127]}"(X1), "=&{v[128:143]}"(X2), "=&{v[144:159]}"(X3), [any] "=&s"(any) \
+                 : [a] "v"(AOP), [b0] "v"(B0), [b1] "v"(B1), [b2] "v"(B2), [b3] "v"(B3), [t0] "v"(th0), [t1] "v"(th1), [t2] "v"(th2), [t3] "v"(th3) \
+                 : "s36", "s37", "s38", "s39", "s40", "s41", "s42", "s43")
+#define RT_SPARSE_MASK(MASK) \
+    asm volatile("v_mov_b32_e32 %[m], 0\n\t" RT_MASK_SET(144, "%[t3]") RT_MASK_SET(128, "%[t2]") RT_MASK_SET(112, "%[t1]") RT_MASK_SET(96, "%[t0]") \
+                 : [m] "=&v"(MASK) : "{v[96:111]}"(X0), "{v[112:127]}"(X1), "{v[128:143]}"(X2), "{v[144:159]}"(X3), \
+                   [t0] "v"(th0), [t1] "v"(th1), [t2] "v"(th2), [t3] "v"(th3) : "vcc")
+
+template <bool kCount>
+__global__ void __launch_bounds__(256) __attribute__((amdgpu_waves_per_eu(3)))
+scan_sparse_kernel(SceneView sc, WaveBuffers wb, MfView mf, uint32_t bounce, uint32_t n_tiles, uint32_t stretch, uint32_t peak_num, uint32_t peak_den,
+                   Counters *__restrict__ counters, int debug_skip_exact)
+{
+    using Cfg = SparseCfg;
+    constexpr int S = kSoloSets, H = S / 2;
+    static_assert(S == 4, "a granule is four sets of 32 rays");
+    __shared__ uint2 lds_queue[4u * Cfg::kQueue];
+    __shared__ uint32_t lds_ring[4u * 16u];
+    const uint32_t n_rays = wb.counts[bounce], n_gran = (n_rays + 127u) >> 7;
+    const RayQueue qin = (bounce & 1u) ? wb.q[1] : wb.q[0];
+    unsigned long long *best = (bounce & 1u) ? wb.best[1] : wb.best[0];
+    const int lane = threadIdx.x & 63, wave = __builtin_amdgcn_readfirstlane((int)(threadIdx.x >> 6)), half = lane >> 5;
+    const uint32_t n_waves = gridDim.x * 4u, wave_id = blockIdx.x * 4u + (uint32_t)wave;
+    uint2 *const cand = wb.cand + (size_t)wave_id * stretch;
+    unsigned long long appended = 0;
+    const uint32_t group_shift = (uint32_t)__builtin_ctz(mf.group_quads) + 2u;
+    static_assert(kMfQuadTiles == 4, "group_shift");
+    uint2 *queue = lds_queue + wave * Cfg::kQueue;
+    uint32_t *const ring = lds_ring + wave * 16;
+    unsigned long long *const lds_tally = solo_cand_words<kCount, 12u>();
+    if (kCount && lane < 3) lds_tally[4 * lane + wave] = 0ull;
+    typedef const float __attribute__((address_space(4))) *ConstFloats;
+    typedef float f32x4 __attribute__((ext_vector_type(4)));
+    typedef const volatile f32x4 __attribute__((address_space(4))) *ConstGroupHalf;
+    const ConstFloats groups_k = (ConstFloats)(uintptr_t)mf.groups;
+
+    uint32_t qn = 0, seq = 0, seq_flushed = 0;
+    auto flush = [&]() __attribute__((always_inline)) {
+        for (uint32_t i0 = 0; i0 < qn; i0 += 64u) {
+            const uint32_t i = i0 + (uint32_t)lane;
+            const uint2 e = i < qn ? queue[i] : make_uint2(0u, 0u);
+            const uint32_t ln = e.x & 63u, pos5 = ((e.x >> 8) & ((1u << Cfg::kTileBits) - 1u)) * kMfTileTris + 5u * (ln >> 5);
+            const uint32_t slot0 = ring[e.x >> 28] * 128u;
+            if (kCount) { const uint32_t pairs = (uint32_t)__popc(e.y & ((1u << (5 * S)) - 1u)); if (pairs) atomicAdd(&lds_tally[wave], (unsigned long long)pairs); }
+            const uint32_t bits = (debug_skip_exact == 0 || debug_skip_exact == 3) ? e.y : 0u;
+#pragma unroll
+            for (int s = 0; s < S; ++s) {
+                uint32_t um = (bits >> (5 * s)) & 31u;
+                const unsigned long long m = __builtin_amdgcn_ballot_w64(um != 0u);
+                const unsigned long long at = appended + __builtin_amdgcn_mbcnt_hi((uint32_t)(m >> 32), __builtin_amdgcn_mbcnt_lo((uint32_t)m, 0u));
+                const uint32_t slot = slot0 + (uint32_t)(s * 32) + (ln & 31u);
+                if (um != 0u) {
+                    if (at < (unsigned long long)stretch) store_through(reinterpret_cast<unsigned long long *>(cand + at), (unsigned long long)slot | ((unsigned long long)((pos5 << 5) | um) << 32));
+                    else
+                        while (um) {
+                            const uint32_t pos = pos5 + (uint32_t)__builtin_ctz(um);
+                            um &= um - 1u;
+                            if (pos < sc.n_tri_visits) exact_and_merge_at(mf, qin, best, slot, pos);
+                        }
+                }
+                appended += (unsigned long long)__popcll(m);
+            }
+        }
+        qn = 0; seq_flushed = seq;
+    };
+
+    const uint32_t *const keep = wb.keep;
+    const uint32_t keep_words = wb.keep_words;
+    for (uint32_t g = wave_id; g < n_gran; g += n_waves) {
+        const uint32_t *const row = keep + (size_t)g * keep_words;
+        uint32_t w0 = 0u, word = 0u, bits = 0u, tbase = 0u;
+        unsigned long long nz = 0ull;
+        auto load_words = [&]() {
+            const uint32_t w = w0 + (uint32_t)lane, t0 = w * 32u;
+            word = w < keep_words ? row[w] : 0u;
+            word = t0 >= n_tiles ? 0u : (n_tiles - t0 >= 32u ? word : word & ((1u << (n_tiles - t0)) - 1u));
+            nz = __builtin_amdgcn_ballot_w64(word != 0u);
+        };
+        constexpr uint32_t kNone = 0xFFFFFFFFu;
+        auto next_tile = [&]() -> uint32_t {
+            while (bits == 0u) {
+                while (nz == 0ull) {
+                    if (w0 + 64u >= keep_words) return kNone;
+                    w0 += 64u; load_words();
+                }
+                const uint32_t l = (uint32_t)__builtin_ctzll(nz);
+                nz &= nz - 1ull;
+                bits = (uint32_t)__builtin_amdgcn_readlane((int)word, (int)l);
+                tbase = (w0 + l) * 32u;
+            }
+            const uint32_t b = (uint32_t)__builtin_ctz(bits);
+            bits &= bits - 1u;
+            return tbase + b;
+        };
+        load_words();
+        if (kCount) {
+            const uint32_t rays_g = min(128u, n_rays - g * 128u);
+            for (uint32_t k0 = 0; k0 < keep_words; k0 += 64u) {
+                const uint32_t w = k0 + (uint32_t)lane, t0 = w * 32u;
+                uint32_t x = w < keep_words ? row[w] : 0u;
+                x = t0 >= n_tiles ? 0u : (n_tiles - t0 >= 32u ? x : x & ((1u << (n_tiles - t0)) - 1u));
+                if (x) atomicAdd(&lds_tally[8 + wave], (unsigned long long)((uint32_t)__popc(x) * rays_g));
+            }
+            if (lane == 0) atomicAdd(&lds_tally[4 + wave], (unsigned long long)n_tiles * rays_g);
+        }
+        uint32_t tile = next_tile();
+        if (tile == kNone) continue;
+        const uint4 *const A_lane = mf.A + lane;
+        uint4 a_cur = A_lane[(size_t)tile * 64u];
+
+        const uint32_t slot0 = g * 128u;
+        float4 ra[H], rb[H];
+        if (slot0 + 128u <= n_rays) {
+#pragma unroll
+            for (int j = 0; j < H; ++j) ra[j] = qin.a[slot0 + (uint32_t)lane + (uint32_t)j * 64u];
+#pragma unroll
+            for (int j = 0; j < H; ++j) rb[j] = qin.b[slot0 + (uint32_t)lane + (uint32_t)j * 64u];
+        } else {
+#pragma unroll
+            for (int j = 0; j < H; ++j) {
+                const uint32_t slot = slot0 + (uint32_t)j * 64u + (uint32_t)lane;
+                ra[j] = make_float4(0.0f, 0.0f, 0.0f, 0.0f); rb[j] = ra[j];
+                if (slot < n_rays) { ra[j] = qin.a[slot]; rb[j] = qin.b[slot]; }
+            }
+        }
+        MfRay ray[H];
+#pragma unroll
+        for (int j = 0; j < H; ++j) scan_prepare_ray<true>(ray[j], ra[j], rb[j], slot0 + (uint32_t)j * 64u + (uint32_t)lane < n_rays, half);
+
+        if (seq - seq_flushed >= 15u) flush();
+        if (lane == 0) ring[seq & 15u] = g;
+        const uint32_t item_tag = (seq & 15u) << 28;
+        ++seq;
+
+        u32x4 B0, B1, B2, B3;
+        float th0, th1, th2, th3;
+        f32x16 X0, X1, X2, X3;
+        unsigned long long any;
+        uint32_t grp = kNone;
+        while (tile != kNone) {
+            const uint32_t nxt = next_tile();
+            uint4 a_nxt = a_cur;
+            if (nxt != kNone) a_nxt = A_lane[(size_t)nxt * 64u];
+            if ((tile >> group_shift) != grp) {
+                grp = tile >> group_shift;
+                const ConstGroupHalf gp = (ConstGroupHalf)(groups_k + (size_t)grp * (sizeof(MfGroup) / 4));
+                const f32x4 g_lo = gp[0], g_hi = gp[1];
+                MfGroup G;
+                G.cx = g_lo.x; G.cy = g_lo.y; G.cz = g_lo.z; G.E = g_lo.w; G.Ml = g_hi.x; G.Pw = g_hi.y; G.P = g_hi.z; G.pad1 = 0.0f;
+                u32x4 Bs[S]; float ths[S];
+                scan_group_operands<true, H>(G, ray, debug_skip_exact, Bs, ths);
+                B0 = Bs[0]; B1 = Bs[1]; B2 = Bs[2]; B3 = Bs[3];
+                th0 = ths[0]; th1 = ths[1]; th2 = ths[2]; th3 = ths[3];
+            }
+            const u32x4 ap = {a_cur.x, a_cur.y, a_cur.z, a_cur.w};
+            RT_SPARSE_TILE(ap);
+            if (__builtin_expect(any != 0ull, 0)) {
+                uint32_t mask;
+                RT_SPARSE_MASK(mask);
+                const unsigned long long m = __builtin_amdgcn_ballot_w64(mask != 0u);
+                uint32_t pre = __builtin_amdgcn_mbcnt_hi((uint32_t)(m >> 32), __builtin_amdgcn_mbcnt_lo((uint32_t)m, 0u));
+                asm volatile("" : "+v"(pre));
+                queue[mask ? qn + pre : Cfg::kQueue - 1u] = make_uint2((uint32_t)lane | (tile << 8) | item_tag, mask);
+                qn += (uint32_t)__popcll(m);
+                if (qn >= Cfg::kDrain) flush();
+            }
+            tile = nxt; a_cur = a_nxt;
+        }
+    }
+    flush();
+    const uint32_t n_rec = (uint32_t)(appended < (unsigned long long)stretch ? appended : (unsigned long long)stretch);
+    if (n_rec) {
+        asm volatile("s_waitcnt vmcnt(0)" ::: "memory");
+        drain_region<2>(sc, mf, qin, best, reinterpret_cast<const unsigned long long *>(cand), n_rec, (uint32_t)lane);
+    }
+    if (lane == 0 && appended) {
+        const unsigned __int128 scaled = ((unsigned __int128)appended * peak_num + (peak_den - 1u)) / peak_den;
+        const uint32_t peak = scaled < (unsigned __int128)0xFFFFFFF0ull ? (uint32_t)scaled : 0xFFFFFFF0u;
+        if (peak > *wb.cand_peak) atomicMax(wb.cand_peak, peak);
+    }
+    if (kCount) {
+        wave_lds_sync();
+        if (lane == 0 && lds_tally[wave]) atomicAdd(&counters->candidates, lds_tally[wave]);
+        if (lane == 0 && lds_tally[4 + wave] != lds_tally[8 + wave]) atomicAdd(&counters->culled_tests, (lds_tally[4 + wave] - lds_tally[8 + wave]) * kMfTileTris);
+        if (blockIdx.x == 0 && threadIdx.x == 0) atomicAdd(&counters->tri_tests, (unsigned long long)n_rays * sc.n_tri_visits);
+    }
+}
+
+__global__ void __launch_bounds__(256) keep_count_kernel(const uint32_t *__restrict__ keep, size_t n_words, unsigned long long *__restrict__ total)
+{
+    __shared__ uint32_t part[4];
+    uint32_t c = 0u;
+    for (size_t i = (size_t)blockIdx.x * 256u + threadIdx.x; i < n_words; i += (size_t)gridDim.x * 256u) c += (uint32_t)__popc(keep[i]);
+    for (int off = 32; off > 0; off >>= 1) c += (uint32_t)__shfl_xor((int)c, off);
+    if ((threadIdx.x & 63u) == 0u) part[threadIdx.x >> 6] = c;
+    __syncthreads();
+    if (threadIdx.x == 0) { const uint32_t s = part[0] + part[1] + part[2] + part[3]; if (s) atomicAdd(total, (unsigned long long)s); }
+}
+
+}
diff --git a/raytracer.glsl_amd/csrc/rt_sparse_launch.hpp b/raytracer.glsl_amd/csrc/rt_sparse_launch.hpp
--- /dev/null
+++ b/raytracer.glsl_amd/csrc/rt_sparse_launch.hpp
@@ -0,0 +1,37 @@
+#pragma once
+#include <cstdint>
+#include <cstddef>
+#include <algorithm>
+
+namespace rt_sparse_launch {
+
+constexpr uint32_t kBlockWaves = 4, kWavesPerSimd = 3, kSimdsPerCu = 4, kBlocksPerCu = kWavesPerSimd * kSimdsPerCu / kBlockWaves;
+constexpr uint32_t kRaysPerWave = 128;
+constexpr uint32_t kMaxTiles = 1u << 20;
+
+constexpr uint32_t kMaxKeptPerGranule = 31;
+inline bool sparse_enough(uint64_t kept_tiles, uint32_t granules) { return kept_tiles <= (uint64_t)kMaxKeptPerGranule * std::max(granules, 1u); }
+
+struct Rule {
+    bool cull; uint32_t bounce; int scan_dynamic, mesh_dist, narrow_fused; bool stamps_build; int camera_sparse;
+    uint32_t tiles; bool have_count; uint64_t kept_tiles; uint32_t granules;
+};
+inline bool take(const Rule &r)
+{
+    return r.cull && r.bounce == 0 && r.scan_dynamic == 0 && r.mesh_dist == 3 && r.narrow_fused == 1 && !r.stamps_build && r.camera_sparse == 1
+           && r.tiles > 0 && r.tiles < kMaxTiles && r.have_count && sparse_enough(r.kept_tiles, r.granules);
+}
+
+struct Launch { uint32_t blocks, waves, stretch, peak_num, peak_den; };
+inline Launch launch(uint32_t n_cus, uint32_t n0, uint32_t regions, uint32_t region_pairs)
+{
+    Launch L = {};
+    const uint32_t granules = (uint32_t)(((uint64_t)n0 + kRaysPerWave - 1u) / kRaysPerWave);
+    L.blocks = std::max(1u, std::min(std::max(n_cus, 1u) * kBlocksPerCu, (granules + kBlockWaves - 1u) / kBlockWaves));
+    L.waves = L.blocks * kBlockWaves;
+    L.stretch = (uint32_t)std::min<uint64_t>((uint64_t)regions * region_pairs / L.waves, 0xFFFFFFFFull);
+    L.peak_num = L.waves; L.peak_den = std::max(regions, 1u);
+    return L;
+}
+
+}
diff --git a/raytracer.glsl_amd/csrc/rtgl_amd.hip b/raytracer.glsl_amd/csrc/rtgl_amd.hip
--- a/raytracer.glsl_amd/csrc/rtgl_amd.hip
+++ b/raytracer.glsl_amd/csrc/rtgl_amd.hip
@@ -16,6 +16,7 @@
 #include "rt_wavefront.hpp"
 #include "rt_mfma.hpp"
 #include "rt_scan.hpp"
+#include "rt_scan_sparse.hpp"
 #include "rt_denoise.hpp"
 #include "rt_temporal.hpp"
 #include "rt_temporal_clip.hpp"
@@ -31,6 +32,7 @@
 #include "rt_mesh_visits.hpp"
 #include "rt_buffers.hpp"
 #include "rt_scan_launch.hpp"
+#include "rt_sparse_launch.hpp"
 #include "rt_shade_launch.hpp"
 #include "rt_camera_keep.hpp"
 
@@ -214,6 +216,12 @@
     uint32_t *d_keep0 = nullptr; size_t keep0_capacity = 0; bool keep0_valid = false; rt_camera_keep::Camera keep0_camera{}; uint32_t keep0_n0 = 0, keep0_words = 0; uint64_t keep0_scene = 0;
     int opt_camera_lean = 1;
     uint32_t camera_lean_frames = 0;
+    int opt_camera_sparse = 1;
+    uint32_t camera_sparse_launches = 0;
+    unsigned long long *d_keep0_count = nullptr, *h_keep0_count = nullptr;
+    uint64_t keep0_count_seq = 0, keep0_count_next = 0;
+    uint64_t keep0_count_copy = 0, keep0_count_seen = 0;
+    uint64_t keep0_kept = 0; uint32_t keep0_granules = 0;
     int opt_shade_pass = 1;
     uint32_t shade_pass_launches = 0;
     uint64_t scene_version = 0;
@@ -402,6 +410,7 @@
     if (const char *k = getenv("RTGL_AMD_SCAN_DYNAMIC")) { const int v = atoi(k); if (v >= 0 && v <= 4) ctx->opt_scan_dynamic = v; }
     if (const char *k = getenv("RTGL_AMD_NARROW_FUSED")) { const int v = atoi(k); if (v == 0 || v == 1) ctx->opt_narrow_fused = v; }
     if (const char *k = getenv("RTGL_AMD_SORT_MOVE")) { const int v = atoi(k); if (v == 0 || v == 1) ctx->opt_sort_move = v; }
+    if (const char *k = getenv("RTGL_AMD_CAMERA_SPARSE")) { const int v = atoi(k); if (v == 0 || v == 1) ctx->opt_camera_sparse = v; }
     if (const char *k = getenv("RTGL_AMD_CAMERA_LEAN")) { const int v = atoi(k); if (v == 0 || v == 1) ctx->opt_camera_lean = v; }
     if (const char *k = getenv("RTGL_AMD_SHADE_PASS")) { const int v = atoi(k); if (v == 0 || v == 1) ctx->opt_shade_pass = v; }
     *out = ctx;
@@ -468,6 +477,7 @@
     ctx->buffers.release_all();
     for (hipEvent_t e : ctx->kev) (void)hipEventDestroy(e);
     if (ctx->h_counts) (void)hipHostFree(ctx->h_counts);
+    if (ctx->h_keep0_count) (void)hipHostFree(ctx->h_keep0_count);
     if (ctx->counts_ev) (void)hipEventDestroy(ctx->counts_ev);
     if (ctx->ev0) (void)hipEventDestroy(ctx->ev0);
     if (ctx->ev1) (void)hipEventDestroy(ctx->ev1);
@@ -1055,6 +1065,17 @@
             if (cached) {
                 HIPCHK(ctx, hipGetLastError());
                 ctx->keep0_valid = true; ctx->keep0_n0 = n0; ctx->keep0_words = ctx->wb.keep_words; ctx->keep0_scene = ctx->scene_version; ctx->keep0_camera = keep_camera(*cam);
+                ctx->keep0_count_seq = 0;
+                if (ctx->opt_camera_sparse) {
+                    if (!ctx->d_keep0_count) RCCHK(buf_alloc(ctx, ctx->d_keep0_count, sizeof(unsigned long long)));
+                    if (!ctx->h_keep0_count) HIPCHK(ctx, hipHostMalloc((void **)&ctx->h_keep0_count, sizeof(unsigned long long), hipHostMallocDefault));
+                    const uint32_t granules = (n0 + 127u) / 128u;
+                    const size_t words = (size_t)granules * ctx->wb.keep_words;
+                    HIPCHK(ctx, hipMemsetAsync(ctx->d_keep0_count, 0, sizeof(unsigned long long), ctx->stream));
+                    hipLaunchKernelGGL(keep_count_kernel, dim3((unsigned)std::max<size_t>(1, std::min<size_t>((words + 2047) / 2048, 1024))), dim3(256), 0, ctx->stream, ctx->d_keep0, words, ctx->d_keep0_count);
+                    HIPCHK(ctx, hipGetLastError());
+                    ctx->keep0_count_seq = ++ctx->keep0_count_next; ctx->keep0_granules = granules;
+                }
             }
         }
         if (L.dist == 2) {
@@ -1071,6 +1092,24 @@
 #else
     const int fused = ctx->opt_narrow_fused;
 #endif
+    {
+#ifdef RT_SOLO_STAMPS
+        const bool stamps_build = true;
+#else
+        const bool stamps_build = false;
+#endif
+        const bool have_count = cached && have_bits && ctx->keep0_count_seq != 0 && ctx->keep0_count_seen == ctx->keep0_count_seq;
+        const rt_sparse_launch::Rule rule{L.cull != 0, bounce, ctx->opt_scan_dynamic, rt_scan_launch::mesh_dist(setup), fused, stamps_build, ctx->opt_camera_sparse,
+                                          setup.real_quads * (uint32_t)kMfQuadTiles, have_count, ctx->keep0_kept, ctx->keep0_granules};
+        if (rt_sparse_launch::take(rule)) {
+            const rt_sparse_launch::Launch SL = rt_sparse_launch::launch((uint32_t)ctx->n_cus, n0, ctx->cand_regions, ctx->wb.cand_region);
+            hipLaunchKernelGGL(ctx->opt_counters ? scan_sparse_kernel<true> : scan_sparse_kernel<false>, dim3(SL.blocks), dim3(256), 0, ctx->stream, sc, ctx->wb, mf, bounce, rule.tiles, SL.stretch, SL.peak_num, SL.peak_den,
+                               ctx->d_counters, ctx->opt_debug_skip_exact);
+            HIPCHK(ctx, hipGetLastError());
+            ctx->camera_sparse_launches++;
+            return RTGL_OK;
+        }
+    }
     hipLaunchKernelGGL(kScanKernels[ctx->opt_counters != 0][L.W - 1][L.dist], dim3(L.blocks), dim3(256 * L.W), L.lds, ctx->stream, sc, ctx->wb, mf, bounce, L.chunk_quads, L.chunks, ctx->d_counters, ctx->opt_debug_skip_exact, L.cull, fused);
     HIPCHK(ctx, hipGetLastError());
     if (!fused) hipLaunchKernelGGL(narrow_phase_kernel, dim3(L.blocks * L.waves, kNarrowSplit), dim3(256), 0, ctx->stream, sc, ctx->wb, mf, bounce, L.blocks * L.waves);
@@ -1087,6 +1126,7 @@
         ctx->counts_pending = false;
         if (ctx->counts_n0 == n0) ctx->est_counts.assign(ctx->h_counts, ctx->h_counts + ctx->counts_len);
         else ctx->est_counts.clear();
+        if (ctx->keep0_count_copy) { ctx->keep0_count_seen = ctx->keep0_count_copy; ctx->keep0_kept = *ctx->h_keep0_count; ctx->keep0_count_copy = 0; }
         const uint32_t peak = ctx->h_counts[ctx->counts_capacity];
         if (!ctx->cand_fixed && peak > ctx->cand_region_pairs) ctx->cand_region_target = (uint32_t)std::min<uint64_t>((uint64_t)peak + peak / 4, 0xFFFFFFF0u);
     }
@@ -1189,6 +1229,10 @@
     if (!ctx->counts_pending) {
         ctx->counts_len = P.max_bounce + 1; ctx->counts_n0 = n0;
         HIPCHK(ctx, hipMemcpyAsync(ctx->h_counts, ctx->d_counts, counts_bytes(ctx->counts_capacity), hipMemcpyDeviceToHost, ctx->stream));
+        if (ctx->keep0_count_seq && ctx->keep0_count_seen != ctx->keep0_count_seq) {
+            HIPCHK(ctx, hipMemcpyAsync(ctx->h_keep0_count, ctx->d_keep0_count, sizeof(unsigned long long), hipMemcpyDeviceToHost, ctx->stream));
+            ctx->keep0_count_copy = ctx->keep0_count_seq;
+        }
         HIPCHK(ctx, hipEventRecord(ctx->counts_ev, ctx->stream));
         ctx->counts_pending = true;
     }
@@ -2630,6 +2674,9 @@
     } else if (!strcmp(key, "camera_lean")) {
         if (value != 0 && value != 1) return fail(ctx, RTGL_ERR_INVALID, "camera_lean must be 0 (camera rays travel through queue 0 in full) or 1 (shade rebuilds them while the camera's keep bits are reused)");
         ctx->opt_camera_lean = value;
+    } else if (!strcmp(key, "camera_sparse")) {
+        if (value != 0 && value != 1) return fail(ctx, RTGL_ERR_INVALID, "camera_sparse must be 0 (the camera-ray bounce is always scanned chunk by chunk) or 1 (granule by granule while its kept rows are sparse)");
+        ctx->opt_camera_sparse = value;
     } else if (!strcmp(key, "shade_pass")) {
         if (value != 0 && value != 1) return fail(ctx, RTGL_ERR_INVALID, "shade_pass must be 0 (every shade launch in grid-stride passes) or 1 (one pass, a block per 256 slots of queue 0, unless the queue is expected to be all but empty)");
         ctx->opt_shade_pass = value;
@@ -2702,6 +2749,12 @@
     else if (!strcmp(key, "camera_lean")) *value = ctx->opt_camera_lean;
     else if (!strcmp(key, "camera_lean_frames")) *value = (int)ctx->camera_lean_frames;
     else if (!strcmp(key, "shade_pass")) *value = ctx->opt_shade_pass;
+    else if (!strcmp(key, "camera_sparse")) *value = ctx->opt_camera_sparse;
+    else if (!strcmp(key, "camera_sparse_density")) {
+        const bool have = ctx->keep0_valid && ctx->keep0_count_seq != 0 && ctx->keep0_count_seen == ctx->keep0_count_seq;
+        *value = have ? (int)std::min<uint64_t>(ctx->keep0_kept * 256u / std::max(ctx->keep0_granules, 1u), 0x7FFFFFFFu) : -1;
+    }
+    else if (!strcmp(key, "camera_sparse_launches")) *value = (int)ctx->camera_sparse_launches;
     else if (!strcmp(key, "shade_pass_launches")) *value = (int)ctx->shade_pass_launches;
     else if (!strcmp(key, "rng_state")) *value = ctx->opt_rng_state;
     else if (!strcmp(key, "aov")) *value = ctx->opt_aov;
```

Result: no change. 947.2 Mpaths/s (median of 6 runs) (+1.0%).
